# spcl/gms

Hardware: AMD Instinct MI355X
Metric: edges-intersected/sec + achieved HBM GB/s, RMAT-26 triangle count @1/2/4/8 GPU (higher is better)
Workload: dtype int32 ids / uint64 counts

## Files before the change

gms_amd/capi.py:

```python
import ctypes as C
import os

import numpy as np

_HERE = os.path.dirname(os.path.abspath(__file__))
LIB_PATH = os.environ.get("GMSX_LIB") or os.path.join(_HERE, "lib", "libgmsx.so")

_i64p = np.ctypeslib.ndpointer(np.int64, flags="C_CONTIGUOUS")
_i32p = np.ctypeslib.ndpointer(np.int32, flags="C_CONTIGUOUS")
_u32p = np.ctypeslib.ndpointer(np.uint32, flags="C_CONTIGUOUS")

GEN_KRONECKER, GEN_UNIFORM = 0, 1
RELABEL_NEVER, RELABEL_AUTO, RELABEL_ALWAYS = 0, 1, 2
TC_AUTO, TC_ORIENTED, TC_FULL = 0, 1, 2
UPLOAD_DEFAULT, UPLOAD_TRUSTED, UPLOAD_FOR_TC = 0, 1, 2
PREPARE_TC = 1
SETOP_INTERSECT, SETOP_DIFFERENCE = 0, 1
OK, ERR_INVALID, ERR_NOMEM, ERR_IO, ERR_FORMAT, ERR_DIRECTED, ERR_NO_DEVICE = 0, -1, -2, -3, -4, -5, -6
ERR_DEVICE_MEM, ERR_NOT_CANONICAL, ERR_OVERFLOW, ERR_UNSUPPORTED, ERR_KERNEL, ERR_COMM, ERR_TIMEOUT = -7, -8, -9, -10, -11, -12, -13
COMM_ID_BYTES = 128

SYMBOLS = [
    "gmsx_strerror", "gmsx_version",
    "gmsx_csr_generate", "gmsx_csr_generate_rmat", "gmsx_csr_from_edges", "gmsx_csr_load", "gmsx_csr_save_sg", "gmsx_csr_save_sgx", "gmsx_csr_is_mapped", "gmsx_csr_from_arrays",
# ... 248 lines not shown
    def save_sg(self, path):
        _check(lib().gmsx_csr_save_sg(self._h, os.fsencode(path)), "gmsx_csr_save_sg")

    def save_sgx(self, path):
        _check(lib().gmsx_csr_save_sgx(self._h, os.fsencode(path)), "gmsx_csr_save_sgx")

    @property
    def is_mapped(self):
        return bool(lib().gmsx_csr_is_mapped(self._h))

    def relabel_by_degree(self):
        h = C.c_void_p()
        _check(lib().gmsx_csr_relabel_by_degree(self._h, C.byref(h)), "gmsx_csr_relabel_by_degree")
        return HostCSR(h)

    def worth_relabelling(self):
        return bool(lib().gmsx_csr_worth_relabelling(self._h))

    @property
    def num_nodes(self):
        return lib().gmsx_csr_num_nodes(self._h)

    @property
    def num_edges(self):
        return lib().gmsx_csr_num_edges(self._h)

    @property
    def nnz(self):
        return lib().gmsx_csr_num_edges_directed(self._h)

    def offsets(self):
        return np.ctypeslib.as_array(lib().gmsx_csr_offsets(self._h), shape=(self.num_nodes + 1,))

    def neighbors(self):
        nnz = self.nnz
        if nnz == 0:
            return np.zeros(0, dtype=np.int32)
        return np.ctypeslib.as_array(lib().gmsx_csr_neighbors(self._h), shape=(nnz,))

    def merge_elements(self):
        return int(lib().gmsx_csr_merge_elements(self._h))

    def fingerprint(self):
        return int(lib().gmsx_csr_fingerprint(self._h, 0)), int(lib().gmsx_csr_fingerprint(self._h, 1))

    def __del__(self):
        if getattr(self, "_h", None):
            lib().gmsx_csr_free(self._h)
            self._h = None


def set_host_threads(n=0):
    return int(lib().gmsx_set_host_threads(int(n)))


def set_option(name, value):
    _check(lib().gmsx_set_option(name.encode(), None if value is None else str(value).encode()), f"gmsx_set_option({name})")


def reset_options():
    lib().gmsx_reset_options()


def option_names():
    out, i, p = [], 0, C.c_char_p()
    while lib().gmsx_option_name(i, C.byref(p)) == 0:
        out.append(p.value.decode())
        i += 1
    return out


class options:

    def __init__(self, **kw):
        self.kw = kw

    def __enter__(self):
        for k, v in self.kw.items():
            set_option(k, v)
        return self

    def __exit__(self, *exc):
        for k in self.kw:
            set_option(k, None)
        return False


def init(device=-1):
    _check(lib().gmsx_init(device), "gmsx_init")


def set_stream(stream_ptr):
    _check(lib().gmsx_set_stream(C.c_void_p(stream_ptr)), "gmsx_set_stream")


def hbm_read_probe(nbytes=4 << 30, iterations=20):
    v = C.c_double(0)
    _check(lib().gmsx_hbm_read_probe(int(nbytes), int(iterations), C.byref(v)), "gmsx_hbm_read_probe")
    return v.value


def device_info():
    name = C.create_string_buffer(256)
    cu, mem = C.c_int(0), C.c_int64(0)
    _check(lib().gmsx_device_info(name, 256, C.byref(cu), C.byref(mem)), "gmsx_device_info")
    return {"name": name.value.decode(), "compute_units": cu.value, "hbm_bytes": mem.value}


class DeviceGraph:

    def __init__(self, handle):
        self._h = handle

    @classmethod
    def upload(cls, off, neigh, flags=UPLOAD_DEFAULT):
        off = np.ascontiguousarray(off, dtype=np.int64)
        neigh = np.ascontiguousarray(neigh, dtype=np.int32)
        h = C.c_void_p()
        _check(lib().gmsx_graph_upload(off.size - 1, off, neigh if neigh.size else np.zeros(1, np.int32), flags, C.byref(h)),
               "gmsx_graph_upload")
        return cls(h)

    @classmethod
    def from_csr(cls, csr, flags=UPLOAD_DEFAULT, shard=None):
        h = C.c_void_p()
        if shard is None:
            _check(lib().gmsx_graph_upload_csr(csr._h, flags, C.byref(h)), "gmsx_graph_upload_csr")
        else:
            _check(lib().gmsx_graph_upload_csr_shard(csr._h, flags, int(shard[0]), int(shard[1]), C.byref(h)), "gmsx_graph_upload_csr_shard")
        return cls(h)

    num_nodes = property(lambda self: lib().gmsx_graph_num_nodes(self._h))
    num_edges = property(lambda self: lib().gmsx_graph_num_edges(self._h))
    device_bytes = property(lambda self: lib().gmsx_graph_device_bytes(self._h))
    max_out_degree = property(lambda self: lib().gmsx_graph_max_out_degree(self._h))
    tc_passes = property(lambda self: lib().gmsx_graph_tc_passes(self._h))

    def prepare(self, what=PREPARE_TC):
        _check(lib().gmsx_graph_prepare(self._h, what), "gmsx_graph_prepare")

    def tc_total(self, algo=TC_AUTO, stats=False):
        out, st = C.c_uint64(0), Stats()
        _check(lib().gmsx_tc_total(self._h, algo, C.byref(out), C.byref(st)), "gmsx_tc_total")
        return (int(out.value), st.as_dict()) if stats else int(out.value)

    def tc_partial(self, part, nparts, algo=TC_AUTO, stats=False):
        out, st = C.c_uint64(0), Stats()
        _check(lib().gmsx_tc_partial(self._h, algo, part, nparts, C.byref(out), C.byref(st)), "gmsx_tc_partial")
        return (int(out.value), st.as_dict()) if stats else int(out.value)

    BREAKDOWN = ["hub_rows_list", "hub_rows_bitset", "hub_rows_delta", "tail_rows_list", "tail_rows_delta", "entries", "pivot_containers",
                 "of_which_inline_rows", "light_streamed_hub_rows", "light_streamed_tail_rows", "light_pivot_lists_and_descriptors",
                 "count_entries", "count_inline_entries", "count_work_items", "count_light_streamed_members",
                 "reserved15", "reserved16", "reserved17", "reserved18", "reserved19", "reserved20"]
    BREAKDOWN_BYTES = ("hub_rows_list", "hub_rows_bitset", "hub_rows_delta", "tail_rows_list", "tail_rows_delta", "entries", "pivot_containers",
                       "light_streamed_hub_rows", "light_streamed_tail_rows", "light_pivot_lists_and_descriptors")

    def tc_stream_breakdown(self):
        out = np.zeros(21, dtype=np.uint64)
        _check(lib().gmsx_tc_stream_breakdown(self._h, out), "gmsx_tc_stream_breakdown")
        return dict(zip(self.BREAKDOWN, (int(x) for x in out)))

    def tc_row_histogram(self):
        out = np.zeros(256, dtype=np.uint64)
        _check(lib().gmsx_tc_row_histogram(self._h, out), "gmsx_tc_row_histogram")
        return out[:240].reshape(5, 24, 2).astype(np.int64), out[240:].astype(np.int64)

    def tc_comembership(self, batch):
        out = np.zeros(8, dtype=np.uint64)
        _check(lib().gmsx_tc_comembership(self._h, int(batch), out), "gmsx_tc_comembership")
        return dict(entries=int(out[0]), units=int(out[1]), distinct_rows=int(out[2]), batched_units=int(out[3]), items=int(out[4]))

    def tc_vertex_count2(self, stats=False):
        c, st = np.zeros(self.num_nodes, dtype=np.int64), Stats()
        _check(lib().gmsx_tc_vertex_count2(self._h, c, C.byref(st)), "gmsx_tc_vertex_count2")
        return (c, st.as_dict()) if stats else c

    def intersect_count_batch(self, u, v, stats=False):
        u = np.ascontiguousarray(u, dtype=np.int32)
        v = np.ascontiguousarray(v, dtype=np.int32)
        out, st = np.zeros(max(u.size, 1), dtype=np.uint32), Stats()
        _check(lib().gmsx_intersect_count_batch(self._h, u.size, u if u.size else np.zeros(1, np.int32),
                                                v if v.size else np.zeros(1, np.int32), out, C.byref(st)),
               "gmsx_intersect_count_batch")
        out = out[:u.size]
        return (out, st.as_dict()) if stats else out

    def set_op_batch(self, op, u, v, stats=False):
        code = {"intersect": SETOP_INTERSECT, "difference": SETOP_DIFFERENCE}[op]
        u = np.ascontiguousarray(u, dtype=np.int32)
        v = np.ascontiguousarray(v, dtype=np.int32)
        uu, vv = (u if u.size else np.zeros(1, np.int32)), (v if v.size else np.zeros(1, np.int32))
        off, st = np.zeros(u.size + 1, dtype=np.int64), Stats()
        _check(lib().gmsx_set_op_batch(self._h, code, u.size, uu, vv, off, None, 0, C.byref(st)), "gmsx_set_op_batch (sizing)")
        ids = np.zeros(max(int(off[-1]), 1), dtype=np.int32)
        _check(lib().gmsx_set_op_batch(self._h, code, u.size, uu, vv, off, ids.ctypes.data_as(C.c_void_p), int(off[-1]), C.byref(st)), "gmsx_set_op_batch")
        ids = ids[:int(off[-1])]
        return (off, ids, st.as_dict()) if stats else (off, ids)

    SIM = {"jaccard": 0, "overlap": 1, "adamic_adar": 2, "resource": 3, "common_neighbors": 4, "total_neighbors": 5, "pref_attachment": 6}

    def vertex_similarity_batch(self, metric, u, v, stats=False):
        u = np.ascontiguousarray(u, dtype=np.int32)
        v = np.ascontiguousarray(v, dtype=np.int32)
        out, st = np.zeros(max(u.size, 1), dtype=np.float64), Stats()
        m = self.SIM[metric] if isinstance(metric, str) else int(metric)
        _check(lib().gmsx_vertex_similarity_batch(self._h, m, u.size, u if u.size else np.zeros(1, np.int32),
                                                  v if v.size else np.zeros(1, np.int32), out, C.byref(st)), "gmsx_vertex_similarity_batch")
        out = out[:u.size]
        return (out, st.as_dict()) if stats else out

    def kclique_count(self, k, stats=False):
        ordered, cliques, st = C.c_uint64(0), C.c_uint64(0), Stats()
        _check(lib().gmsx_kclique_count(self._h, k, C.byref(ordered), C.byref(cliques), C.byref(st)), "gmsx_kclique_count")
        r = (int(ordered.value), int(cliques.value))
        return (r + (st.as_dict(),)) if stats else r

    def kclique_star_count(self, k, members=True, stats=False):
        stars, mem, st = C.c_uint64(0), C.c_uint64(0), Stats()
        _check(lib().gmsx_kclique_star_count(self._h, k, C.byref(stars), C.byref(mem) if members else None, C.byref(st)), "gmsx_kclique_star_count")
        r = (int(stars.value), int(mem.value) if members else None)
        return (r + (st.as_dict(),)) if stats else r

    def kclique_star_list_info(self, k, cliques_only=False, part=0, nparts=1):
        info = KcliqueStarListInfo()
        flags = KCSTAR_CLIQUES_ONLY if cliques_only else KCSTAR_DEFAULT
        _check(lib().gmsx_kclique_star_list(self._h, k, flags, part, nparts, None, None, None, 0, 0, C.byref(info), None),
               "gmsx_kclique_star_list (sizing)")
        return info.as_dict()

    def kclique_star_list(self, k, cliques_only=False, part=0, nparts=1, stats=False):
        info, st = KcliqueStarListInfo(), Stats()
        flags = KCSTAR_CLIQUES_ONLY if cliques_only else KCSTAR_DEFAULT
        _check(lib().gmsx_kclique_star_list(self._h, k, flags, part, nparts, None, None, None, 0, 0, C.byref(info), C.byref(st)),
               "gmsx_kclique_star_list (sizing)")
        sizing = st.as_dict()
        nc, nm = int(info.cliques), int(info.star_members)
        cl = np.zeros(max(nc * k, 1), dtype=np.int32)
        soff = mem = None
        if not cliques_only:
            soff = np.zeros(nc + 1, dtype=np.int64)
            mem = np.zeros(max(nm, 1), dtype=np.int32)
        _check(lib().gmsx_kclique_star_list(self._h, k, flags, part, nparts, cl.ctypes.data_as(C.c_void_p),
                                            None if cliques_only else soff.ctypes.data_as(C.c_void_p),
                                            None if cliques_only else mem.ctypes.data_as(C.c_void_p), nc, nm, C.byref(info), C.byref(st)),
               "gmsx_kclique_star_list")
        cl = cl[:nc * k].reshape(nc, k)
        if mem is not None:
            mem = mem[:nm]
        if stats:
            return cl, soff, mem, {"sizing": sizing, "fill": st.as_dict(), "info": info.as_dict()}
        return cl, soff, mem

    def kclique_partial(self, k, part, nparts, stats=False):
        out, st = C.c_uint64(0), Stats()
        _check(lib().gmsx_kclique_partial(self._h, k, part, nparts, C.byref(out), C.byref(st)), "gmsx_kclique_partial")
        return (int(out.value), st.as_dict()) if stats else int(out.value)

    def bk_count(self, rank=None, stats=False):
        out, st = C.c_uint64(0), Stats()
        rp = None
        if rank is not None:
            rank = np.ascontiguousarray(rank, dtype=np.int32)
            rp = rank.ctypes.data_as(C.c_void_p)
        _check(lib().gmsx_bk_count(self._h, rp, C.byref(out), C.byref(st)), "gmsx_bk_count")
        return (int(out.value), st.as_dict()) if stats else int(out.value)

    def bk_partial(self, part, nparts, rank=None, stats=False):
        out, st = C.c_uint64(0), Stats()
        rp = None
        if rank is not None:
            rank = np.ascontiguousarray(rank, dtype=np.int32)
            rp = rank.ctypes.data_as(C.c_void_p)
        _check(lib().gmsx_bk_partial(self._h, rp, part, nparts, C.byref(out), C.byref(st)), "gmsx_bk_partial")
        return (int(out.value), st.as_dict()) if stats else int(out.value)

    def bk_list_info(self, rank=None, part=0, nparts=1):
        info = BkListInfo()
        rp = None
        if rank is not None:
            rank = np.ascontiguousarray(rank, dtype=np.int32)
            rp = rank.ctypes.data_as(C.c_void_p)
        _check(lib().gmsx_bk_list(self._h, rp, part, nparts, None, None, 0, 0, C.byref(info), None), "gmsx_bk_list (sizing)")
        return info.as_dict()

    def bk_list(self, rank=None, part=0, nparts=1, stats=False):
        info, st = BkListInfo(), Stats()
        rp = None
        if rank is not None:
            rank = np.ascontiguousarray(rank, dtype=np.int32)
            rp = rank.ctypes.data_as(C.c_void_p)
        _check(lib().gmsx_bk_list(self._h, rp, part, nparts, None, None, 0, 0, C.byref(info), C.byref(st)), "gmsx_bk_list (sizing)")
        sizing = st.as_dict()
        off = np.zeros(int(info.cliques) + 1, dtype=np.int64)
        mem = np.zeros(max(int(info.members), 1), dtype=np.int32)
        _check(lib().gmsx_bk_list(self._h, rp, part, nparts, off.ctypes.data_as(C.c_void_p), mem.ctypes.data_as(C.c_void_p), off.size,
                                  int(info.members), C.byref(info), C.byref(st)), "gmsx_bk_list")
        mem = mem[:int(info.members)]
        if stats:
            return off, mem, {"sizing": sizing, "fill": st.as_dict(), "info": info.as_dict()}
        return off, mem

    def adg_rank(self, epsilon=0.001, rank_format=True, stats=False):
        out, rounds, st = np.zeros(max(self.num_nodes, 1), dtype=np.int32), C.c_int32(0), Stats()
        _check(lib().gmsx_adg_rank(self._h, float(epsilon), int(bool(rank_format)), out, C.byref(rounds), C.byref(st)), "gmsx_adg_rank")
        r = (out[:self.num_nodes], int(rounds.value))
        return (r + (st.as_dict(),)) if stats else r

    def tc_ordering(self, stats=False):
# ... 143 lines not shown
```

gms_amd/csrc/hip/device_graph.hip:

```cpp
#include "device_graph.hpp"

#include <algorithm>
#include <mutex>
#include <array>
#include <chrono>
#include <cstdio>
#include <cstdlib>
#include <cstring>
#include <memory>
#include <new>
#include <random>

#include <rocprim/device/device_radix_sort.hpp>
#include <rocprim/device/device_scan.hpp>
#include <rocprim/device/device_segmented_radix_sort.hpp>
#include <rocprim/iterator/transform_iterator.hpp>

#include "../host/gmsx_internal.hpp"

namespace gmsx {

Ctx &ctx() {
    static Ctx c;
    return c;
}

int ensure_init() { return ctx().device >= 0 ? GMSX_OK : gmsx_init(-1); }


__device__ __forceinline__ unsigned long long arc_mix(unsigned long long x) {
    x ^= x >> 30;
    x *= 0xbf58476d1ce4e5b9ull;
    x ^= x >> 27;
    x *= 0x94d049bb133111ebull;
    x ^= x >> 31;
    return x;
}
__global__ __launch_bounds__(256) void k_validate(int64_t n, const int64_t *__restrict__ off,
                                                  const int32_t *__restrict__ adj, int check_symmetry, unsigned long long key0,
                                                  unsigned long long key1,
                                                  unsigned long long *__restrict__ acc ) {
    const int lane = threadIdx.x & 63;
    const int64_t wave0 = (int64_t(blockIdx.x) * blockDim.x + threadIdx.x) >> 6;
    const int64_t nwaves = (int64_t(gridDim.x) * blockDim.x) >> 6;
    unsigned flags = 0;
    unsigned long long elems = 0;
    unsigned long long maxdeg = 0;
    unsigned long long f0 = 0, r0 = 0, f1 = 0, r1 = 0;
    for (int64_t u = wave0; u < n; u += nwaves) {
        const int64_t b = off[u], e = off[u + 1];
        const unsigned long long du = (unsigned long long)(e - b);
        if (du > maxdeg) maxdeg = du;
        if (lane == 0) elems += du * du;
        for (int64_t j = b + lane; j < e; j += 64) {
            const int32_t v = adj[j];
            if (v < 0 || v >= n) { flags |= 2; continue; }
            if (v == u) flags |= 4;
            if (j + 1 < e && adj[j + 1] <= v) flags |= 1;
            if (check_symmetry) {
                const unsigned long long uv = ((unsigned long long)uint32_t(u) << 32) | uint32_t(v), vu = ((unsigned long long)uint32_t(v) << 32) | uint32_t(u);
                f0 += arc_mix(uv ^ key0);
                r0 += arc_mix(vu ^ key0);
                f1 += arc_mix(uv * 0x9e3779b97f4a7c15ull + key1);
                r1 += arc_mix(vu * 0x9e3779b97f4a7c15ull + key1);
            }
        }
    }
    for (int s = 32; s > 0; s >>= 1) {
        elems += __shfl_down(elems, s);
        flags |= __shfl_down(flags, s);
        const unsigned long long o = __shfl_down(maxdeg, s);
        maxdeg = o > maxdeg ? o : maxdeg;
        f0 += __shfl_down(f0, s);
        r0 += __shfl_down(r0, s);
        f1 += __shfl_down(f1, s);
        r1 += __shfl_down(r1, s);
    }
    if (lane == 0) {
        if (flags) atomicOr(&acc[0], (unsigned long long)flags);
        if (elems) atomicAdd(&acc[1], elems);
        atomicMax(&acc[2], maxdeg);
        if (check_symmetry) {
            atomicAdd(&acc[3], f0);
            atomicAdd(&acc[4], r0);
            atomicAdd(&acc[5], f1);
            atomicAdd(&acc[6], r1);
        }
    }
}

__global__ void k_rank_keys(int64_t n, const int64_t *__restrict__ off, unsigned long long *__restrict__ keys) {
    const int64_t u = int64_t(blockIdx.x) * blockDim.x + threadIdx.x;
    if (u < n) keys[u] = ((unsigned long long)(off[u + 1] - off[u]) << 32) | (unsigned long long)u;
}
__global__ void k_assign_ids(int64_t n, const unsigned long long *__restrict__ sorted_keys, int32_t *__restrict__ oldid,
                             int32_t *__restrict__ newid) {
    const int64_t i = int64_t(blockIdx.x) * blockDim.x + threadIdx.x;
    if (i < n) {
        const int32_t o = int32_t(sorted_keys[i] & 0xffffffffull);
        oldid[i] = o;
        newid[o] = int32_t(i);
    }
}

__global__ __launch_bounds__(256) void k_count_parts(int64_t n, const int64_t *__restrict__ off, const int32_t *__restrict__ adj,
                                                     const int32_t *__restrict__ newid, int hub_limit, int64_t *__restrict__ hcnt,
                                                     int64_t *__restrict__ tcnt, int32_t *__restrict__ dplus) {
    const int lane = threadIdx.x & 63;
    const int64_t wave0 = (int64_t(blockIdx.x) * blockDim.x + threadIdx.x) >> 6;
    const int64_t nwaves = (int64_t(gridDim.x) * blockDim.x) >> 6;
    for (int64_t u = wave0; u < n; u += nwaves) {
        const int64_t b = off[u], e = off[u + 1];
        const int32_t nu = newid[u];
        int ch = 0, ct = 0;
        for (int64_t j = b + lane; j < e; j += 64) {
            const int32_t nv = newid[adj[j]];
            if (nv < nu) {
                if (nv < hub_limit) ch++; else ct++;
            }
        }
        for (int s = 32; s > 0; s >>= 1) {
            ch += __shfl_down(ch, s);
            ct += __shfl_down(ct, s);
        }
        if (lane == 0) {
            hcnt[nu] = (ch + 1) & ~1;
            tcnt[nu] = ct;
            dplus[nu] = ch + ct;
        }
    }
}

__global__ __launch_bounds__(256) void k_fill_parts(int64_t n, const int64_t *__restrict__ off, const int32_t *__restrict__ adj,
                                                    const int32_t *__restrict__ newid, int hub_limit, const int64_t *__restrict__ hoff,
                                                    const int64_t *__restrict__ toff, uint16_t *__restrict__ hadj,
                                                    int32_t *__restrict__ tadj) {
    const int lane = threadIdx.x & 63;
    const int64_t wave0 = (int64_t(blockIdx.x) * blockDim.x + threadIdx.x) >> 6;
    const int64_t nwaves = (int64_t(gridDim.x) * blockDim.x) >> 6;
    for (int64_t u = wave0; u < n; u += nwaves) {
        const int64_t b = off[u], e = off[u + 1];
        const int32_t nu = newid[u];
        int64_t ho = hoff[nu], to = toff[nu];
        const int64_t hend = hoff[nu + 1];
        for (int64_t base = b; base < e; base += 64) {
            const int64_t j = base + lane;
            bool kh = false, kt = false;
            int32_t nv = 0;
            if (j < e) {
                nv = newid[adj[j]];
                kh = nv < nu && nv < hub_limit;
                kt = nv < nu && nv >= hub_limit;
            }
            const unsigned long long mh = __ballot(kh), mt = __ballot(kt);
            const unsigned long long below = (1ull << lane) - 1ull;
            if (kh) hadj[ho + __popcll(mh & below)] = uint16_t(nv);
            if (kt) tadj[to + __popcll(mt & below)] = nv;
            ho += __popcll(mh);
            to += __popcll(mt);
        }
        if (lane == 0 && ho < hend) hadj[ho] = 0xFFFF;
    }
}

__device__ inline uint32_t delta_encode(const uint16_t *__restrict__ row, int len, uint32_t *__restrict__ emit) {
    uint32_t units = 0;
    int i = 0;
    while (i < len && row[i] != 0xFFFFu) {
        uint32_t w[4] = {row[i], 0u, 0u, 0u};
        uint32_t cur = row[i];
        int slot = 3;
// ... 86 lines not shown
            int rf = kFormList;
            if (rl >= 24 && delta_mode > 0) {
                const uint32_t d = delta_encode(hadj + b + k, rl, nullptr);
                if (d * 100u <= r * uint32_t(delta_pct)) { r = d; rf = kFormDelta; }
            }
            const uint32_t cand = uint32_t(B / 128) + r;
            if (cand < tot && (hybrid_mode == 2 || cand * 100u <= best * 90u)) {
                tot = cand;
                ks = k;
                best2 = r;
                form2 = rf;
            }
        }
        if (ks > 0) {
            best = tot - best2;
            form = kFormBitset;
        }
    }
    ksplit[v] = ks;
    const uint32_t u2[2] = {best, best2};
    const int f2[2] = {form, form2};
    for (int sl = 0; sl < 2; ++sl) {
        const bool big = u2[sl] >= 8u;
        units_out[2 * v + sl] = big ? int64_t((u2[sl] + 7u) & ~7u) : 0;
        small_out[2 * v + sl] = big ? 0 : int64_t(u2[sl]);
        real_out[2 * v + sl] = u2[sl];
        form_out[2 * v + sl] = (unsigned char)f2[sl];
    }
}
__global__ void k_srow_fill(int64_t n, const int64_t *__restrict__ hoff, const uint16_t *__restrict__ hadj, const int64_t *__restrict__ bmoff,
                            const uint32_t *__restrict__ bmpool, const int64_t *__restrict__ uoff, const int64_t *__restrict__ soff,
                            const uint32_t *__restrict__ real, const unsigned char *__restrict__ form, const int32_t *__restrict__ ksplit,
                            unsigned long long *__restrict__ srow, unsigned long long *__restrict__ srow2, uint32_t *__restrict__ spool) {
    const int64_t v = int64_t(blockIdx.x) * blockDim.x + threadIdx.x;
    if (v >= n) return;
    const int64_t b = hoff[v];
    const int len = int(hoff[v + 1] - b);
    const int ks = ksplit[v];
    for (int sl = 0; sl < 2; ++sl) {
        const int64_t units = int64_t(real[2 * v + sl]);
        const int64_t u0 = units >= 8 ? uoff[2 * v + sl] : uoff[2 * n] + soff[2 * v + sl];
        const int fm = form[2 * v + sl];
        const unsigned long long d = units ? ((unsigned long long)u0 << 24) | ((unsigned long long)fm << 22) | (unsigned long long)units : 0ull;
        if (sl == 0) srow[v] = units ? d : ((unsigned long long)u0 << 24) | ((unsigned long long)fm << 22);
        else srow2[v] = d;
        if (units == 0) continue;
        uint32_t *dst = spool + u0 * 4;
        const uint16_t *row = hadj + b + (sl ? ks : 0);
        const int rl = sl ? len - ks : len;
        if (sl == 0 && ks > 0) {
            for (int64_t w = 0; w < units * 4; ++w) dst[w] = 0;
            for (int i = 0; i < ks; ++i) dst[row[i] >> 5] |= 1u << (row[i] & 31u);
        } else if (fm == kFormDelta) {
            delta_encode(row, rl, dst);
        } else if (fm == kFormGap12) {
            gap12_encode(row, rl, dst);
        } else if (fm == kFormBitset) {
            const uint32_t *src = bmpool + bmoff[v];
            for (int64_t w = 0; w < units * 4; ++w) dst[w] = src[w];
        } else {
            for (int64_t w = 0; w < units * 4; ++w) {
                const int i = int(w) * 2;
                const uint32_t lo = i < rl ? row[i] : 0xFFFFu, hi = i + 1 < rl ? row[i + 1] : 0xFFFFu;
                dst[w] = lo | (hi << 16);
            }
        }
    }
}

__device__ inline uint32_t tail_delta_encode(const int32_t *__restrict__ row, int len, uint32_t *__restrict__ emit) {
    uint32_t units = 0;
    int i = 0;
    while (i < len) {
        uint32_t w[4] = {uint32_t(row[i]), 0u, 0u, 0u};
        uint32_t cur = uint32_t(row[i]);
        int slot = 1;
        ++i;
        while (i < len && slot < 6) {
            const uint32_t gap = uint32_t(row[i]) - cur;
            if (gap > 65535u) break;
            w[1 + (slot >> 1)] |= gap << ((slot & 1) * 16);
            ++slot;
            cur = uint32_t(row[i]);
            ++i;
        }
        w[1] |= uint32_t(slot);
        if (emit) {
            emit[units * 4 + 0] = w[0]; emit[units * 4 + 1] = w[1]; emit[units * 4 + 2] = w[2]; emit[units * 4 + 3] = w[3];
        }
        ++units;
    }
    return units;
}
__global__ void k_trow_sizes(int64_t n, const int64_t *__restrict__ toff, const int32_t *__restrict__ tadj, int delta_mode,
                             int64_t *__restrict__ units_out, int64_t *__restrict__ small_out, uint32_t *__restrict__ real_out, unsigned char *__restrict__ form_out) {
    const int64_t v = int64_t(blockIdx.x) * blockDim.x + threadIdx.x;
    if (v > n) return;
    if (v == n) { units_out[n] = 0; small_out[n] = 0; return; }
    const int64_t b = toff[v];
    const int len = int(toff[v + 1] - b);
    uint32_t best = uint32_t((len + 3) / 4);
    int form = kFormList;
    if (len >= 8 && delta_mode > 0) {
        const uint32_t d = tail_delta_encode(tadj + b, len, nullptr);
        if (delta_mode == 2 || d * 100u <= best * 85u) { best = d; form = kFormDelta; }
    }
    const bool big = best >= 8u;
    units_out[v] = big ? int64_t((best + 7u) & ~7u) : 0;
    small_out[v] = big ? 0 : int64_t(best);
    real_out[v] = best;
    form_out[v] = (unsigned char)form;
}
__global__ void k_trow_fill(int64_t n, const int64_t *__restrict__ toff, const int32_t *__restrict__ tadj, const int64_t *__restrict__ uoff,
                            const int64_t *__restrict__ soff, const uint32_t *__restrict__ real, const unsigned char *__restrict__ form,
                            unsigned long long *__restrict__ trow, uint32_t *__restrict__ tpool) {
    const int64_t v = int64_t(blockIdx.x) * blockDim.x + threadIdx.x;
    if (v >= n) return;
    const int64_t units = int64_t(real[v]);
    const int64_t u0 = units >= 8 ? uoff[v] : uoff[n] + soff[v];
    trow[v] = ((unsigned long long)u0 << 24) | ((unsigned long long)form[v] << 22) | (unsigned long long)units;
    if (units == 0) return;
    uint32_t *dst = tpool + u0 * 4;
    const int64_t b = toff[v];
    const int64_t len = toff[v + 1] - b;
    if (form[v] == kFormDelta) tail_delta_encode(tadj + b, int(len), dst);
    else
        for (int64_t w = 0; w < units * 4; ++w) dst[w] = w < len ? uint32_t(tadj[b + w]) : 0xfffffffeu;
}

__global__ void k_dense_sizes(int32_t limit, const int32_t *__restrict__ dplus, int64_t *__restrict__ sizes) {
    const int32_t v = int32_t(blockIdx.x * blockDim.x + threadIdx.x);
    if (v < limit) sizes[v] = bitset_words(v);
    if (v == limit) sizes[v] = 0;
}
__global__ __launch_bounds__(256) void k_dense_fill(int32_t limit, const int64_t *__restrict__ hoff, const uint16_t *__restrict__ hadj,
                                                    const int64_t *__restrict__ toff, const int32_t *__restrict__ tadj,
                                                    const int64_t *__restrict__ bmoff, uint32_t *__restrict__ pool) {
    const int lane = threadIdx.x & 63;
    const int32_t wave0 = int32_t((int64_t(blockIdx.x) * blockDim.x + threadIdx.x) >> 6);
    const int32_t nwaves = int32_t((int64_t(gridDim.x) * blockDim.x) >> 6);
    for (int32_t v = wave0; v < limit; v += nwaves) {
        const int64_t b = bmoff[v];
        if (bmoff[v + 1] == b) continue;
        for (int64_t j = hoff[v] + lane; j < hoff[v + 1]; j += 64) {
            const uint32_t id = hadj[j];
            if (id != 0xFFFFu) atomicOr(&pool[b + (id >> 5)], 1u << (id & 31u));
        }
        for (int64_t j = toff[v] + lane; j < toff[v + 1]; j += 64) {
            const uint32_t id = uint32_t(tadj[j]);
            atomicOr(&pool[b + (id >> 5)], 1u << (id & 31u));
        }
    }
}
__global__ __launch_bounds__(256) void k_tail_split(int64_t n, const int64_t *__restrict__ toff, const int32_t *__restrict__ tadj, int32_t limit,
                                                    int32_t *__restrict__ tsplit) {
    const int lane = threadIdx.x & 63;
    const int64_t wave0 = (int64_t(blockIdx.x) * blockDim.x + threadIdx.x) >> 6;
    const int64_t nwaves = (int64_t(gridDim.x) * blockDim.x) >> 6;
    for (int64_t u = wave0; u < n; u += nwaves) {
        int c = 0;
        for (int64_t j = toff[u] + lane; j < toff[u + 1]; j += 64) c += tadj[j] < limit;
        for (int s = 32; s > 0; s >>= 1) c += __shfl_down(c, s);
        if (lane == 0) tsplit[u] = c;
    }
}

__global__ void k_order_keys(int64_t n, const int32_t *__restrict__ dplus, int32_t *__restrict__ keys, int32_t *__restrict__ vals) {
    const int64_t i = int64_t(blockIdx.x) * blockDim.x + threadIdx.x;
    if (i < n) {
        keys[i] = dplus[i];
        vals[i] = int32_t(i);
    }
}

__global__ void k_warm(unsigned long long *p) {
    if (p) p[0] = 0;
}
__global__ void k_count_ge(int64_t n, const int32_t *__restrict__ order, const int32_t *__restrict__ dplus, int32_t thr, int64_t *__restrict__ out) {
    int64_t lo = 0, hi = n;
    while (lo < hi) {
        const int64_t mid = (lo + hi) >> 1;
        if (dplus[order[mid]] >= thr) lo = mid + 1; else hi = mid;
    }
    out[0] = lo;
}
__global__ void k_task_limits(int64_t n, const unsigned long long *__restrict__ srow, const unsigned long long *__restrict__ srow2,
                              const unsigned long long *__restrict__ trow, uint32_t hub_max, uint32_t tail_max, unsigned long long *__restrict__ out) {
    const int64_t v = int64_t(blockIdx.x) * blockDim.x + threadIdx.x;
    if (v >= n) return;
    if ((srow[v] & 0x3fffffull) > hub_max || (srow2[v] & 0x3fffffull) > hub_max || (trow[v] & 0x3fffffull) > tail_max) atomicOr(out, 1ull);
}

static constexpr int kInlineChunk = 64;
static constexpr int kDefaultInlineFirst = 28;
static constexpr int kInlineFirstMax = 64;
__device__ __forceinline__ bool takes_inline(int32_t v, int32_t inline_limit, const int32_t *__restrict__ dplus) {
    return v < inline_limit || dplus[v] >= kHeavy;
}
template <bool FILL>
__global__ __launch_bounds__(256) void k_inline_rows(int64_t first, int64_t end, const int32_t *__restrict__ order, const int64_t *__restrict__ hoff,
                                                     const uint16_t *__restrict__ hadj, const int64_t *__restrict__ toff, const int32_t *__restrict__ tadj,
                                                     const int32_t *__restrict__ dplus, int32_t inline_limit, int inline_first, const int32_t *__restrict__ opos, int nparts, int part,
                                                     unsigned long long *__restrict__ cnt_h,
                                                     unsigned long long *__restrict__ cnt_t, const int64_t *__restrict__ ihoff,
                                                     const int64_t *__restrict__ itoff, int64_t base_h, uint16_t *__restrict__ pool_h, int64_t base_t,
                                                     int32_t *__restrict__ pool_t) {
    const int lane = threadIdx.x & 63;
    const int64_t wave0 = (int64_t(blockIdx.x) * blockDim.x + threadIdx.x) >> 6;
    const int64_t nwaves = (int64_t(gridDim.x) * blockDim.x) >> 6;
    for (int64_t pos = first + wave0; pos < end; pos += nwaves) {
        const int32_t u = order[pos];
        const int64_t hb = hoff[u], tb = toff[u];
        const int first_u = dplus[u] >= kHeavy ? inline_first : kInlineFirstMax;
        const int hl = min(int(hoff[u + 1] - hb), first_u), tl = min(int(toff[u + 1] - tb), first_u - hl);
        int32_t mv = 0x7fffffff;
        if (lane < hl) {
            const uint32_t x = hadj[hb + lane];
            if (x != 0xFFFFu) mv = int32_t(x);
        } else if (lane - hl < tl) {
            mv = tadj[tb + (lane - hl)];
        }
        const bool valid = mv != 0x7fffffff, is_tail = valid && lane >= hl;
        const unsigned long long vmask = __ballot(valid);
        const int nhub = __popcll(__ballot(valid && lane < hl));
        const int below = __popcll(vmask & ((1ull << lane) - 1ull));
        const bool give = valid && below > 0 && takes_inline(mv, inline_limit, dplus);
        const bool mine = give && (nparts <= 1 || shard_of(opos[mv], nparts) == part);
        const int nh = mine ? (is_tail ? nhub : below) : 0;
        const int nt = mine && is_tail ? lane - hl : 0;
        if (!FILL) {
            if (nh) atomicAdd(&cnt_h[mv], (unsigned long long)nh);
            if (nt) atomicAdd(&cnt_t[mv], (unsigned long long)nt);
        } else {
            int64_t at_h = 0, at_t = 0;
            if (nh) at_h = (base_h + ihoff[mv]) * 8 + int64_t(atomicAdd(&cnt_h[mv], (unsigned long long)nh));
            if (nt) at_t = (base_t + itoff[mv]) * 4 + int64_t(atomicAdd(&cnt_t[mv], (unsigned long long)nt));
            for (int k = 0; k < nhub; ++k) {
                const int32_t x = __shfl(mv, k);
                if (k < nh) pool_h[at_h + k] = uint16_t(x);
            }
            for (int k = 0; k < tl; ++k) {
                const int32_t x = __shfl(mv, hl + k);
                if (k < nt) pool_t[at_t + k] = x;
            }
        }
    }
}
__global__ void k_inline_units(int64_t n, const unsigned long long *__restrict__ ids_h, const unsigned long long *__restrict__ ids_t,
                               int64_t *__restrict__ units_h, int64_t *__restrict__ units_t) {
    const int64_t v = int64_t(blockIdx.x) * blockDim.x + threadIdx.x;
    if (v > n) return;
    units_h[v] = v < n ? int64_t((ids_h[v] + 7) / 8) : 0;
    units_t[v] = v < n ? int64_t((ids_t[v] + 3) / 4) : 0;
}
static constexpr int kDefaultHotWindows = 0, kDefaultHotKB = 2048, kDefaultHotMin = 16;
__device__ __forceinline__ int64_t receiver_of(int32_t w, const int32_t *__restrict__ dplus, const int32_t *__restrict__ opos, const int64_t *__restrict__ lidx,
                                               int64_t n_heavy) {
    return dplus[w] >= kHeavy ? int64_t(opos[w]) : n_heavy + lidx[w];
}
__global__ void k_opos(int64_t n, const int32_t *__restrict__ order, int32_t *__restrict__ opos) {
    const int64_t p = int64_t(blockIdx.x) * blockDim.x + threadIdx.x;
    if (p < n) opos[order[p]] = int32_t(p);
}
__global__ void k_light_flags(int64_t limit, const int32_t *__restrict__ dplus, int64_t *__restrict__ flags) {
    const int64_t w = int64_t(blockIdx.x) * blockDim.x + threadIdx.x;
    if (w <= limit) flags[w] = (w < limit && dplus[w] < kHeavy) ? 1 : 0;
}
__global__ void k_recv_vertices(int64_t n_heavy, int64_t limit, const int32_t *__restrict__ order, const int32_t *__restrict__ dplus, const int64_t *__restrict__ lidx,
                                int32_t *__restrict__ recv_v) {
    const int64_t i = int64_t(blockIdx.x) * blockDim.x + threadIdx.x;
    if (i < n_heavy) recv_v[i] = order[i];
    if (i < limit && dplus[i] < kHeavy) recv_v[n_heavy + lidx[i]] = int32_t(i);
}
template <bool FILL>
__global__ void k_inline_entries(int64_t n, const int32_t *__restrict__ dplus, const int32_t *__restrict__ opos, const int64_t *__restrict__ lidx, int64_t n_heavy,
                                 int32_t inline_limit, const int64_t *__restrict__ ihoff, const int64_t *__restrict__ itoff, int64_t base_h, int64_t base_t,
                                 uint32_t *__restrict__ cnt, uint32_t *__restrict__ cur, const int64_t *__restrict__ hbeg, const int64_t *__restrict__ tbeg,
                                 TaskList htask, TaskList ttask, unsigned long long *__restrict__ totals, TcClasses cc) {
    const int kClasses = cc.count();
    const int64_t v = int64_t(blockIdx.x) * blockDim.x + threadIdx.x;
    if (v >= n) return;
    const int64_t uh = ihoff[v + 1] - ihoff[v], ut = itoff[v + 1] - itoff[v];
    if (uh == 0 && ut == 0) return;
    if (dplus[v] < kHeavy && v >= inline_limit) return;
    const int64_t p = receiver_of(int32_t(v), dplus, opos, lidx, n_heavy);
    uint32_t *c = cnt + p * kClasses;
    for (int64_t o = 0; o < uh; o += kInlineChunk) {
        const unsigned long long units = (unsigned long long)min(int64_t(kInlineChunk), uh - o);
        const unsigned long long d = ((unsigned long long)(base_h + ihoff[v] + o) << 24) | ((unsigned long long)kFormList << 22) | units;
        const int cls = hub_class(cc, d);
        if (!FILL) atomicAdd(&c[cls], 1u);
        else htask.put(hbeg[p] + c[cls] + atomicAdd(&cur[p * kClasses + cls], 1u), d);
    }
    for (int64_t o = 0; o < ut; o += kInlineChunk) {
        const unsigned long long units = (unsigned long long)min(int64_t(kInlineChunk), ut - o);
        const unsigned long long d = ((unsigned long long)(base_t + itoff[v] + o) << 24) | ((unsigned long long)kFormList << 22) | units;
        const int cls = tail_class(cc, d);
        if (!FILL) atomicAdd(&c[cls], 1u);
        else ttask.put(tbeg[p] + c[cls] + atomicAdd(&cur[p * kClasses + cls], 1u), d);
    }
    if (!FILL) {
        atomicAdd(&totals[0], (unsigned long long)((uh + kInlineChunk - 1) / kInlineChunk));
        atomicAdd(&totals[1], (unsigned long long)((ut + kInlineChunk - 1) / kInlineChunk));
    }
}
__global__ void k_list_sizes(int64_t n_recv, uint32_t *__restrict__ cnt, int64_t *__restrict__ hcnt, int64_t *__restrict__ tcnt, TcClasses cc) {
    const int kClasses = cc.count(), hub_end = cc.tail_base();
    const int64_t p = int64_t(blockIdx.x) * blockDim.x + threadIdx.x;
    if (p > n_recv) return;
    if (p == n_recv) { hcnt[p] = 0; tcnt[p] = 0; return; }
    uint32_t *c = cnt + p * kClasses;
    uint32_t run = 0;
    for (int k = 0; k < hub_end; ++k) { const uint32_t x = c[k]; c[k] = run; run += x; }
    hcnt[p] = run;
    run = 0;
    for (int k = hub_end; k < kClasses; ++k) { const uint32_t x = c[k]; c[k] = run; run += x; }
    tcnt[p] = run;
}

__global__ void k_ledge_count(int64_t first, int64_t end, const int32_t *__restrict__ order, const int64_t *__restrict__ toff, const int32_t *__restrict__ tadj,
                              const int32_t *__restrict__ tsplit, const int32_t *__restrict__ dplus, int64_t *__restrict__ cnt) {
    const int64_t pos = first + int64_t(blockIdx.x) * blockDim.x + threadIdx.x;
    if (pos > end) return;
    int64_t c = 0;
    if (pos < end) {
        const int32_t u = order[pos];
        const int64_t tb = toff[u];
        const int tl = int(toff[u + 1] - tb);
        for (int i = tsplit[u]; i < tl; ++i) c += dplus[tadj[tb + i]] < kHeavy ? 1 : 0;
    }
    cnt[pos - first] = c;
}
__global__ void k_ledge_fill(int64_t first, int64_t end, const int32_t *__restrict__ order, const int64_t *__restrict__ hoff, const int64_t *__restrict__ toff,
                             const int32_t *__restrict__ tadj, const int32_t *__restrict__ tsplit, const int32_t *__restrict__ dplus,
                             const int64_t *__restrict__ ebeg, int nparts, int part, uint4 *__restrict__ ledge) {
    const int64_t pos = first + int64_t(blockIdx.x) * blockDim.x + threadIdx.x;
    if (pos >= end) return;
    const int32_t u = order[pos];
    const int64_t hb = hoff[u], tb = toff[u];
    const int tl = int(toff[u + 1] - tb);
    const unsigned long long hu = (unsigned long long)hb | ((unsigned long long)(hoff[u + 1] - hb) << 40);
    int64_t e = ebeg[pos - first];
    for (int i = tsplit[u]; i < tl; ++i) {
        const int32_t v = tadj[tb + i];
        if (dplus[v] >= kHeavy) continue;
        if (nparts <= 1 || shard_of(e, nparts) == part) {
            const unsigned long long tu = (unsigned long long)tb | ((unsigned long long)i << 40);
            const unsigned long long hv = (unsigned long long)hoff[v] | ((unsigned long long)(hoff[v + 1] - hoff[v]) << 40);
            const unsigned long long tv = (unsigned long long)toff[v] | ((unsigned long long)(toff[v + 1] - toff[v]) << 40);
            const int64_t slot = nparts <= 1 ? e : e / nparts;
            ledge[2 * slot] = make_uint4(uint32_t(hu), uint32_t(hu >> 32), uint32_t(tu), uint32_t(tu >> 32));
            ledge[2 * slot + 1] = make_uint4(uint32_t(hv), uint32_t(hv >> 32), uint32_t(tv), uint32_t(tv >> 32));
        }
        ++e;
    }
}

__device__ __forceinline__ uint32_t cut_hub_units(const uint32_t *__restrict__ spool, unsigned long long d, int below, int32_t v) {
    const uint32_t units = uint32_t(d) & 0x3fffffu, form = (uint32_t(d) >> 22) & 3u;
    if (form == kFormList) return min(units, uint32_t(below + 7) / 8u);
    if (form == kFormBitset) return min(units, uint32_t(v + 127) / 128u);
    const uint4 *row = reinterpret_cast<const uint4 *>(spool) + (d >> 24);
    uint32_t lo = 0, hi = units;
    while (lo < hi) {
        const uint32_t mid = (lo + hi) >> 1;
        if (int32_t(row[mid].x & 0xffffu) < v) lo = mid + 1; else hi = mid;
    }
    return lo;
}
__device__ __forceinline__ uint32_t cut_tail_units(const uint32_t *__restrict__ tpool, unsigned long long d, int below, int32_t v) {
    const uint32_t units = uint32_t(d) & 0x3fffffu, form = (uint32_t(d) >> 22) & 3u;
    if (form != kFormDelta) return min(units, uint32_t(below + 3) / 4u);
    const uint4 *row = reinterpret_cast<const uint4 *>(tpool) + (d >> 24);
    uint32_t lo = 0, hi = units;
    while (lo < hi) {
        const uint32_t mid = (lo + hi) >> 1;
        if (int32_t(row[mid].x) < v) lo = mid + 1; else hi = mid;
    }
    return lo;
}
__device__ __forceinline__ uint32_t claim_by_class(uint32_t *ctr, int cls, bool active, int lane) {
    uint32_t mine = 0;
    unsigned long long todo = __ballot(active);
    while (todo) {
        const int leader = __ffsll((long long)todo) - 1;
        const int c = __builtin_amdgcn_readlane(cls, leader);
        const unsigned long long same = __ballot(active && cls == c);
        uint32_t base = 0;
        if (lane == leader) base = atomicAdd(&ctr[c], uint32_t(__popcll(same)));
        base = uint32_t(__builtin_amdgcn_readlane(int(base), leader));
        if (active && cls == c) mine = base + uint32_t(__popcll(same & ((1ull << lane) - 1ull)));
        todo &= ~same;
    }
    return mine;
}
template <bool FILL>
__global__ __launch_bounds__(256) void k_task_lists(int64_t n_heavy, const int32_t *__restrict__ order, const int64_t *__restrict__ hoff,
                                                    const uint16_t *__restrict__ hadj, const int64_t *__restrict__ toff, const int32_t *__restrict__ tadj,
                                                    const int32_t *__restrict__ dplus, const unsigned long long *__restrict__ srow,
                                                    const unsigned long long *__restrict__ srow2, const int32_t *__restrict__ ksplit,
                                                    const unsigned long long *__restrict__ trow, int two_sided, const int32_t *__restrict__ opos,
                                                    uint32_t *__restrict__ cnt, uint32_t *__restrict__ cur, const int64_t *__restrict__ hbeg,
                                                    const int64_t *__restrict__ tbeg, TaskList htask, TaskList ttask,
                                                    int32_t *__restrict__ tunits, unsigned long long *__restrict__ reversed, const uint32_t *__restrict__ spool,
                                                    const uint32_t *__restrict__ tpool, int32_t inline_limit, int inline_first, int nparts, int part, TcClasses cc) {
    const int kClasses = cc.count();
    const int lane = threadIdx.x & 63;
    const int64_t wave0 = (int64_t(blockIdx.x) * blockDim.x + threadIdx.x) >> 6;
    const int64_t nwaves = (int64_t(gridDim.x) * blockDim.x) >> 6;
    unsigned long long rev = 0;
    for (int64_t pos = wave0; pos < n_heavy; pos += nwaves) {
        const int32_t u = order[pos];
        const int64_t hb = hoff[u], tb = toff[u];
        const int hl = int(hoff[u + 1] - hb), tl = int(toff[u + 1] - tb);
        const unsigned long long du_s = srow[u], du_s2 = srow2[u], du_t = trow[u];
        const int ks_u = ksplit[u];
        uint32_t *cu = cnt + pos * kClasses, *ru = cur + pos * kClasses;
        const bool own_u = nparts <= 1 || shard_of(pos, nparts) == part;
        int kept = 0;
        for (int base = 0; base < hl + tl; base += 64) {
            const int i = base + lane;
            int32_t v = -1;
            if (i < hl) {
                const uint32_t x = hadj[hb + i];
                if (x != 0xFFFFu) v = int32_t(x);
            } else if (i < hl + tl) v = tadj[tb + i - hl];
            if (v >= 0 && i > 0 && i < inline_first && takes_inline(v, inline_limit, dplus)) v = -1;
            bool reverse = false;
            uint32_t ch = 0, ch2 = 0, ct = 0;
            if (v >= 0 && i > 0 && two_sided && dplus[v] >= kHeavy) {
                if (i < hl) {
                    ch = cut_hub_units(spool, du_s, i, v);
                    if (du_s2 && i > ks_u) ch2 = cut_hub_units(spool, du_s2, i - ks_u, v);
                } else {
                    ch = uint32_t(du_s) & 0x3fffffu;
                    ch2 = uint32_t(du_s2) & 0x3fffffu;
                }
                ct = (i < hl || toff[v + 1] == toff[v]) ? 0u : cut_tail_units(tpool, du_t, i - hl, v);
                const uint32_t keep = uint32_t(srow[v] & 0x3fffffull) + uint32_t(srow2[v] & 0x3fffffull) + (i > hl ? uint32_t(trow[v] & 0x3fffffull) : 0u);
                reverse = ch + ch2 + ct < keep;
            }
            const bool fwd = v >= 0 && !reverse && own_u;
            if (reverse && nparts > 1 && shard_of(opos[v], nparts) != part) v = -1;
            const unsigned long long fh = (fwd && i > 0) ? srow[v] : 0ull, fh2 = (fwd && i > 0) ? srow2[v] : 0ull, ft = (fwd && i > hl) ? trow[v] : 0ull;
            const bool fh_on = (fh & 0x3fffffull) != 0, fh2_on = (fh2 & 0x3fffffull) != 0, ft_on = (ft & 0x3fffffull) != 0;
            const uint32_t sh = claim_by_class(FILL ? ru : cu, hub_class(cc, fh), fh_on, lane);
            const uint32_t sh2 = claim_by_class(FILL ? ru : cu, hub_class(cc, fh2), fh2_on, lane);
            const uint32_t st = claim_by_class(FILL ? ru : cu, tail_class(cc, ft), ft_on, lane);
            if (FILL) {
                if (fh_on) htask.put(hbeg[pos] + cu[hub_class(cc, fh)] + sh, fh);
                if (fh2_on) htask.put(hbeg[pos] + cu[hub_class(cc, fh2)] + sh2, fh2);
                if (ft_on) ttask.put(tbeg[pos] + cu[tail_class(cc, ft)] + st, ft);
            }
            kept += __popcll(__ballot(fwd));
            if (v >= 0 && reverse) {
                const int64_t pv = opos[v];
                const unsigned long long rh = ch ? (du_s & ~0x3fffffull) | ch : 0ull, rh2 = ch2 ? (du_s2 & ~0x3fffffull) | ch2 : 0ull,
                                         rt = ct ? (du_t & ~0x3fffffull) | ct : 0ull;
                uint32_t *cv = cnt + pv * kClasses;
                if (!FILL) {
                    if (rh) atomicAdd(&cv[hub_class(cc, rh)], 1u);
                    if (rh2) atomicAdd(&cv[hub_class(cc, rh2)], 1u);
                    if (rt) atomicAdd(&cv[tail_class(cc, rt)], 1u);
                    atomicAdd(&tunits[pv], 1);
                    ++rev;
                } else {
                    uint32_t *rv = cur + pv * kClasses;
                    if (rh) htask.put(hbeg[pv] + cv[hub_class(cc, rh)] + atomicAdd(&rv[hub_class(cc, rh)], 1u), rh);
                    if (rh2) htask.put(hbeg[pv] + cv[hub_class(cc, rh2)] + atomicAdd(&rv[hub_class(cc, rh2)], 1u), rh2);
                    if (rt) ttask.put(tbeg[pv] + cv[tail_class(cc, rt)] + atomicAdd(&rv[tail_class(cc, rt)], 1u), rt);
                }
            }
        }
        if (!FILL && lane == 0 && kept) atomicAdd(&tunits[pos], kept);
    }
    if (!FILL) {
        for (int s = 32; s > 0; s >>= 1) rev += __shfl_down(rev, s);
        if (lane == 0 && rev) atomicAdd(reversed, rev);
    }
}
__global__ void k_item_counts(int64_t n_recv, const int64_t *__restrict__ lbeg, const uint32_t *__restrict__ cnt, TcClasses cc, int phases, int64_t *__restrict__ items) {
    const int64_t p = int64_t(blockIdx.x) * blockDim.x + threadIdx.x;
    if (p > n_recv) return;
    if (p == n_recv) { items[int64_t(phases) * n_recv] = 0; return; }
    for (int ph = 0; ph < phases; ++ph) {
        int64_t b = 0, e = lbeg[p + 1] - lbeg[p];
        if (phases > 1) hub_phase_range(cc, cnt + p * cc.count(), e, ph, &b, &e);
        items[int64_t(ph) * n_recv + p] = (e - b + kTaskChunk - 1) / kTaskChunk;
    }
}
__global__ void k_item_fill(int64_t n_recv, const int32_t *__restrict__ recv_v, const int32_t *__restrict__ opos, const int64_t *__restrict__ lbeg,
                            const int64_t *__restrict__ ioff, TaskList task, const int64_t *__restrict__ coff, int kind,
                            const uint32_t *__restrict__ cnt, TcClasses cc, int phases, gmsx_tc_item *__restrict__ items) {
    const int64_t p = int64_t(blockIdx.x) * blockDim.x + threadIdx.x;
    if (p >= n_recv) return;
    const int32_t w = recv_v[p];
    const uint64_t cont = uint64_t(coff[w]) | (uint64_t(coff[w + 1] - coff[w]) << 40);
    for (int ph = 0; ph < phases; ++ph) {
    int64_t b = 0, e = lbeg[p + 1] - lbeg[p];
    if (phases > 1) hub_phase_range(cc, cnt + p * cc.count(), e, ph, &b, &e);
    b += lbeg[p];
    e += lbeg[p];
    int64_t k = ioff[int64_t(ph) * n_recv + p];
    for (int64_t x = b; x < e; x += kTaskChunk, ++k) {
        const int ne = int(min(int64_t(kTaskChunk), e - x));
        gmsx_tc_item it{};
        it.bc = uint64_t(x) | (uint64_t(ne) << 40);
        it.cont = cont;
        it.pivot = w;
        it.pos = opos[w];
        it.kind = uint32_t(kind);
        for (int f = 0; f < 4; ++f) {
            int lo = 0, hi = ne;
            while (lo < hi) {
                const int mid = (lo + hi) >> 1;
                if (int((uint32_t(task.get(x + mid)) >> 22) & 3u) < f) lo = mid + 1; else hi = mid;
            }
            it.fbeg[f] = uint16_t(lo);
        }
        items[k] = it;
    }
    }
}

static int grid_for_waves(int64_t rows) {
    const int64_t want = (rows + 3) / 4;
    const int64_t cap = int64_t(ctx().compute_units > 0 ? ctx().compute_units : 256) * 32;
    return int(want < 1 ? 1 : (want > cap ? cap : want));
}

template <class T>
static int dmalloc(T **p, int64_t count, gmsx_graph *g, int line = __builtin_LINE()) {
    const size_t bytes = size_t(count > 0 ? count : 1) * sizeof(T);
    const bool trace = opt("MEM_TRACE") != nullptr;
    if (trace && g && bytes >= (1u << 20)) std::fprintf(stderr, "gmsx mem: device_graph.hip:%d %.3f GB (elements of %zu B)\n", line, double(bytes) * 1e-9, sizeof(T));
    if (g && g->tc_building && g->tc_limit_bytes > 0 && g->device_bytes + int64_t(bytes) - g->tc_base_bytes > g->tc_limit_bytes) {
        *p = nullptr;
        return GMSX_ERR_DEVICE_MEM;
    }
    if (hipMalloc(reinterpret_cast<void **>(p), bytes) != hipSuccess) {
        (void)hipGetLastError();
        *p = nullptr;
        return GMSX_ERR_DEVICE_MEM;
    }
    if (g) g->device_bytes += int64_t(bytes);
    return GMSX_OK;
}

struct DevGuard {
    void *p;
    ~DevGuard() { (void)hipFree(p); }
};

static void free_tc(gmsx_graph *g) {
    auto drop = [](auto *&p) {
        (void)hipFree(p);
        p = nullptr;
    };
    drop(g->tsplit); drop(g->srow); drop(g->srow2); drop(g->ksplit); drop(g->spool); drop(g->trow); drop(g->htask.lo); drop(g->htask.hi); drop(g->ttask.lo); drop(g->ttask.hi); drop(g->hitem); drop(g->titem); drop(g->tunits);
    drop(g->ledge); drop(g->tpool); drop(g->shard_hitem); drop(g->shard_titem);
    g->shard_idx_part = g->shard_idx_nparts = -1;
    g->device_bytes -= g->tc_bytes;
    g->tc_bytes = 0;
    g->tc_ready = false;
    g->htask_entries = g->ttask_entries = g->hitems = g->titems = g->inline_hentries = g->inline_tentries = 0;
    g->n_ledge = g->ledge_total = 0;
    g->task_reverse = g->inline_units = g->spool_units = g->tpool_units = 0;
    g->stats_part = g->stats_nparts = -1;
}

static void free_graph(gmsx_graph *g) {
    if (!g) return;
    (void)hipFree(g->off);
    (void)hipFree(g->adj);
    (void)hipFree(g->newid);
    (void)hipFree(g->oldid);
    (void)hipFree(g->hoff);
    (void)hipFree(g->hadj);
    (void)hipFree(g->toff);
    (void)hipFree(g->tadj);
    (void)hipFree(g->bmoff);
    (void)hipFree(g->bmpool);
    (void)hipFree(g->tsplit);
    (void)hipFree(g->srow);
    (void)hipFree(g->srow2);
    (void)hipFree(g->ksplit);
    (void)hipFree(g->spool);
    (void)hipFree(g->trow);
    (void)hipFree(g->htask.lo);
    (void)hipFree(g->htask.hi);
    (void)hipFree(g->ttask.lo);
    (void)hipFree(g->ttask.hi);
    (void)hipFree(g->hitem);
    (void)hipFree(g->titem);
    (void)hipFree(g->tunits);
    (void)hipFree(g->shard_hitem);
    (void)hipFree(g->shard_titem);
    (void)hipFree(g->ledge);
    (void)hipFree(g->tpool);
    (void)hipFree(g->dplus);
    (void)hipFree(g->order);
    (void)hipFree(g->kc_rel);
    (void)hipFree(g->kc_aoff);
    (void)hipFree(g->kc_arena);
    (void)hipFree(g->kc_rec);
    (void)hipFree(g->kc_item);
    (void)hipFree(g->kc_relt);
    (void)hipFree(g->kc_rect);
    (void)hipFree(g->kc_itemt);
    (void)hipFree(g->scratch);
    (void)hipFree(g->acc);
    delete g;
}

int exclusive_scan_i64(const int64_t *in, int64_t *out, int64_t count, hipStream_t s) {
    size_t tmp_bytes = 0;
    GMSX_HIP(rocprim::exclusive_scan(nullptr, tmp_bytes, in, out, int64_t(0), size_t(count), rocprim::plus<int64_t>(), s));
    void *tmp = nullptr;
    GMSX_HIP(hipMalloc(&tmp, tmp_bytes ? tmp_bytes : 8));
    DevGuard g_tmp{tmp};
    GMSX_HIP(rocprim::exclusive_scan(tmp, tmp_bytes, in, out, int64_t(0), size_t(count), rocprim::plus<int64_t>(), s));
    GMSX_HIP(hipStreamSynchronize(s));
    return GMSX_OK;
}

struct OffsetMinus {
    int64_t base;
    __host__ __device__ int64_t operator()(int64_t x) const { return x - base; }
};
__global__ void k_lower_bound_i64(int64_t count, const int64_t *__restrict__ a, int64_t target, int64_t *__restrict__ out) {
    int64_t lo = 0, hi = count;
    while (lo < hi) {
        const int64_t mid = (lo + hi) >> 1;
        if (a[mid] < target) lo = mid + 1; else hi = mid;
    }
    out[0] = lo;
}
template <class K>
static int sort_rows(K *keys, int64_t entries, int64_t n, const int64_t *d_off, int end_bit, hipStream_t s) {
    if (n <= 0 || entries <= 0) return GMSX_OK;
    int64_t chunk = int64_t(1) << 31;
    if (const char *e = opt("SORT_CHUNK")) {
        const long long v = std::atoll(e);
        if (v > 0) chunk = v;
    }
    int64_t *d_v = nullptr;
    GMSX_HIP(hipMalloc(reinterpret_cast<void **>(&d_v), sizeof(int64_t)));
    DevGuard g_v{d_v};
    GMSX_HIP(hipStreamSynchronize(s));
    int64_t v0 = 0, base = 0;
    while (v0 < n) {
        int64_t v1 = n;
        if (entries - base > chunk) {
            hipLaunchKernelGGL(k_lower_bound_i64, dim3(1), dim3(1), 0, s, n + 1, d_off, base + chunk + 1, d_v);
            GMSX_HIP(hipStreamSynchronize(s));
            GMSX_HIP(hipMemcpy(&v1, d_v, sizeof(int64_t), hipMemcpyDeviceToHost));
            v1 = std::max(v0 + 1, std::min(n, v1 - 1));
        }
        int64_t end = 0;
        GMSX_HIP(hipMemcpy(&end, d_off + v1, sizeof(int64_t), hipMemcpyDeviceToHost));
        const int64_t cnt = end - base;
        if (cnt >= (int64_t(1) << 32)) return GMSX_ERR_UNSUPPORTED;
        if (cnt > 0) {
            K *sorted = nullptr;
            GMSX_HIP(hipMalloc(reinterpret_cast<void **>(&sorted), size_t(cnt) * sizeof(K)));
            DevGuard g_sorted{sorted};
            auto begin = rocprim::make_transform_iterator(d_off + v0, OffsetMinus{base});
            auto endit = rocprim::make_transform_iterator(d_off + v0 + 1, OffsetMinus{base});
            size_t tmp_bytes = 0;
            GMSX_HIP(rocprim::segmented_radix_sort_keys(nullptr, tmp_bytes, keys + base, sorted, unsigned(cnt), unsigned(v1 - v0), begin, endit, 0, end_bit, s));
            void *tmp = nullptr;
            GMSX_HIP(hipMalloc(&tmp, tmp_bytes ? tmp_bytes : 8));
            DevGuard g_tmp{tmp};
            GMSX_HIP(rocprim::segmented_radix_sort_keys(tmp, tmp_bytes, keys + base, sorted, unsigned(cnt), unsigned(v1 - v0), begin, endit, 0, end_bit, s));
            GMSX_HIP(hipMemcpyAsync(keys + base, sorted, size_t(cnt) * sizeof(K), hipMemcpyDeviceToDevice, s));
            GMSX_HIP(hipStreamSynchronize(s));
        }
        v0 = v1;
        base = end;
    }
    return GMSX_OK;
}

template <class K, class V>
static int sort_segment_pairs(K *keys, V *vals, int64_t entries, int64_t n, const int64_t *d_off, int end_bit, hipStream_t s) {
    if (n <= 0 || entries <= 0) return GMSX_OK;
    int64_t chunk = int64_t(1) << 31;
    if (const char *e = opt("SORT_CHUNK")) {
        const long long v = std::atoll(e);
        if (v > 0) chunk = v;
    }
    int64_t *d_v = nullptr;
    GMSX_HIP(hipMalloc(reinterpret_cast<void **>(&d_v), sizeof(int64_t)));
    DevGuard g_v{d_v};
    GMSX_HIP(hipStreamSynchronize(s));
    int64_t v0 = 0, base = 0;
    while (v0 < n) {
        int64_t v1 = n;
        if (entries - base > chunk) {
            hipLaunchKernelGGL(k_lower_bound_i64, dim3(1), dim3(1), 0, s, n + 1, d_off, base + chunk + 1, d_v);
            GMSX_HIP(hipStreamSynchronize(s));
            GMSX_HIP(hipMemcpy(&v1, d_v, sizeof(int64_t), hipMemcpyDeviceToHost));
            v1 = std::max(v0 + 1, std::min(n, v1 - 1));
        }
        int64_t end = 0;
        GMSX_HIP(hipMemcpy(&end, d_off + v1, sizeof(int64_t), hipMemcpyDeviceToHost));
        const int64_t cnt = end - base;
        if (cnt >= (int64_t(1) << 32)) return GMSX_ERR_UNSUPPORTED;
        if (cnt > 0) {
            K *k_out = nullptr;
            V *v_out = nullptr;
            GMSX_HIP(hipMalloc(reinterpret_cast<void **>(&k_out), size_t(cnt) * sizeof(K)));
            DevGuard g_ko{k_out};
            GMSX_HIP(hipMalloc(reinterpret_cast<void **>(&v_out), size_t(cnt) * sizeof(V)));
            DevGuard g_vo{v_out};
            auto begin = rocprim::make_transform_iterator(d_off + v0, OffsetMinus{base});
            auto endit = rocprim::make_transform_iterator(d_off + v0 + 1, OffsetMinus{base});
            size_t tmp_bytes = 0;
            GMSX_HIP(rocprim::segmented_radix_sort_pairs(nullptr, tmp_bytes, keys + base, k_out, vals + base, v_out, unsigned(cnt), unsigned(v1 - v0), begin, endit, 0,
                                                         end_bit, s));
            void *tmp = nullptr;
            GMSX_HIP(hipMalloc(&tmp, tmp_bytes ? tmp_bytes : 8));
            DevGuard g_tmp{tmp};
            GMSX_HIP(rocprim::segmented_radix_sort_pairs(tmp, tmp_bytes, keys + base, k_out, vals + base, v_out, unsigned(cnt), unsigned(v1 - v0), begin, endit, 0,
                                                         end_bit, s));
            GMSX_HIP(hipMemcpyAsync(vals + base, v_out, size_t(cnt) * sizeof(V), hipMemcpyDeviceToDevice, s));
            GMSX_HIP(hipStreamSynchronize(s));
        }
        v0 = v1;
        base = end;
    }
    return GMSX_OK;
}

struct PhaseTimer {
    hipStream_t s;
    bool on;
    std::chrono::steady_clock::time_point t0;
    const char *what;
    PhaseTimer(hipStream_t st, const char *w) : s(st), on(opt("TIMING") != nullptr), t0(std::chrono::steady_clock::now()), what(w) {}
    void mark(const char *phase) {
        if (!on) return;
        (void)hipStreamSynchronize(s);
        const auto t1 = std::chrono::steady_clock::now();
        std::fprintf(stderr, "[gmsx %s] %-28s %8.1f ms\n", what, phase, std::chrono::duration<double, std::milli>(t1 - t0).count());
        t0 = t1;
    }
};

static constexpr size_t kH2dChunk = size_t(64) << 20;
struct H2dStage {
// ... 41 lines not shown
        parallel_memcpy(to, static_cast<const char *>(src) + at, n);
        GMSX_HIP(hipMemcpyAsync(static_cast<char *>(dst) + at, to, n, hipMemcpyHostToDevice, s));
        GMSX_HIP(hipEventRecord(st.ev[b], s));
        used[b] = true;
    }
    return GMSX_OK;
}

static int build_device_sets(gmsx_graph *g, uint32_t flags) {
    hipStream_t s = ctx().stream;
    PhaseTimer pt(s, "base build");
    const int64_t n = g->n;
    if (int rc = dmalloc(&g->scratch, 16, g)) return rc;
    if (int rc = dmalloc(&g->acc, kAccWords, g)) return rc;
    GMSX_HIP(hipMemsetAsync(g->scratch, 0, 16 * sizeof(unsigned long long), s));

    const int check_sym = (flags & GMSX_UPLOAD_TRUSTED) ? 0 : 1;
    static const std::array<unsigned long long, 2> sym_keys = []() noexcept {
        try {
            std::random_device rd;
            return std::array<unsigned long long, 2>{((unsigned long long)rd() << 32) | rd(), ((unsigned long long)rd() << 32) | rd()};
        } catch (...) {
            const unsigned long long t = (unsigned long long)std::chrono::steady_clock::now().time_since_epoch().count();
            const unsigned long long a = (unsigned long long)reinterpret_cast<uintptr_t>(&t);
            return std::array<unsigned long long, 2>{t * 0x9E3779B97F4A7C15ull ^ a, (a * 0xC2B2AE3D27D4EB4Full) ^ (t << 17)};
        }
    }();
    if (n > 0)
        hipLaunchKernelGGL(k_validate, dim3(grid_for_waves(n)), dim3(256), 0, s, n, g->off, g->adj, check_sym, sym_keys[0], sym_keys[1], g->scratch);
    unsigned long long acc[7] = {0, 0, 0, 0, 0, 0, 0};
    GMSX_HIP(hipMemcpyAsync(acc, g->scratch, sizeof(acc), hipMemcpyDeviceToHost, s));
    GMSX_HIP(hipStreamSynchronize(s));
    if (check_sym && (acc[3] != acc[4] || acc[5] != acc[6])) acc[0] |= 8;
    if (!(flags & GMSX_UPLOAD_TRUSTED) && acc[0] != 0) return GMSX_ERR_NOT_CANONICAL;
    if ((flags & GMSX_UPLOAD_TRUSTED) && (acc[0] & 2)) return GMSX_ERR_NOT_CANONICAL;
    if (!(flags & GMSX_UPLOAD_TRUSTED) && (g->nnz & 1)) return GMSX_ERR_NOT_CANONICAL;
    g->alg_elements = acc[1];
    g->max_deg = int32_t(acc[2]);
    g->m = g->nnz / 2;

    pt.mark("validate");
    const unsigned tb = unsigned((n + 255) / 256);
    if (int rc = dmalloc(&g->newid, n, g)) return rc;
    if (int rc = dmalloc(&g->oldid, n, g)) return rc;
    if (n > 0) {
        unsigned long long *k_in = nullptr, *k_out = nullptr;
        if (int rc = dmalloc(&k_in, n, nullptr)) return rc;
        DevGuard g1{k_in};
        if (int rc = dmalloc(&k_out, n, nullptr)) return rc;
        DevGuard g2{k_out};
        hipLaunchKernelGGL(k_rank_keys, dim3(tb), dim3(256), 0, s, n, g->off, k_in);
        size_t tmp_bytes = 0;
        GMSX_HIP(rocprim::radix_sort_keys_desc(nullptr, tmp_bytes, k_in, k_out, size_t(n), 0, 64, s));
        void *tmp = nullptr;
        GMSX_HIP(hipMalloc(&tmp, tmp_bytes ? tmp_bytes : 8));
        DevGuard g3{tmp};
        GMSX_HIP(rocprim::radix_sort_keys_desc(tmp, tmp_bytes, k_in, k_out, size_t(n), 0, 64, s));
        hipLaunchKernelGGL(k_assign_ids, dim3(tb), dim3(256), 0, s, n, k_out, g->oldid, g->newid);
        GMSX_HIP(hipStreamSynchronize(s));
    }

    pt.mark("rank ids");
    int hub_limit = int((flags >> 8) & 0xffffu);
    if (hub_limit == 0 || hub_limit > kHub) hub_limit = kHub;
    int64_t *hcnt = nullptr, *tcnt = nullptr;
    if (int rc = dmalloc(&hcnt, n + 1, nullptr)) return rc;
    DevGuard g_h{hcnt};
    if (int rc = dmalloc(&tcnt, n + 1, nullptr)) return rc;
    DevGuard g_t{tcnt};
    GMSX_HIP(hipMemsetAsync(hcnt, 0, size_t(n + 1) * sizeof(int64_t), s));
    GMSX_HIP(hipMemsetAsync(tcnt, 0, size_t(n + 1) * sizeof(int64_t), s));
    if (int rc = dmalloc(&g->dplus, n, g)) return rc;
    if (n > 0)
        hipLaunchKernelGGL(k_count_parts, dim3(grid_for_waves(n)), dim3(256), 0, s, n, g->off, g->adj, g->newid, hub_limit, hcnt, tcnt, g->dplus);
    if (int rc = dmalloc(&g->hoff, n + 1, g)) return rc;
    if (int rc = dmalloc(&g->toff, n + 1, g)) return rc;
    if (int rc = exclusive_scan_i64(hcnt, g->hoff, n + 1, s)) return rc;
    if (int rc = exclusive_scan_i64(tcnt, g->toff, n + 1, s)) return rc;
    GMSX_HIP(hipMemcpy(&g->hub_entries, g->hoff + n, sizeof(int64_t), hipMemcpyDeviceToHost));
    GMSX_HIP(hipMemcpy(&g->tail_entries, g->toff + n, sizeof(int64_t), hipMemcpyDeviceToHost));

    if (int rc = dmalloc(&g->hadj, g->hub_entries + 8, g)) return rc;
    if (int rc = dmalloc(&g->tadj, g->tail_entries + 4, g)) return rc;
    GMSX_HIP(hipMemsetAsync(g->hadj + g->hub_entries, 0xff, 8 * sizeof(uint16_t), s));
    GMSX_HIP(hipMemsetAsync(g->tadj + g->tail_entries, 0xff, 4 * sizeof(int32_t), s));
    if (n > 0)
        hipLaunchKernelGGL(k_fill_parts, dim3(grid_for_waves(n)), dim3(256), 0, s, n, g->off, g->adj, g->newid, hub_limit, g->hoff, g->toff,
                           g->hadj, g->tadj);

    pt.mark("containers count+fill");
    if (int rc = sort_rows(g->hadj, g->hub_entries, n, g->hoff, 16, s)) return rc;
    if (int rc = sort_rows(g->tadj, g->tail_entries, n, g->toff, 32, s)) return rc;
    g->rows_sorted = true;

    pt.mark("row sorts");
    g->dense_limit = int32_t(std::min<int64_t>(n, hub_limit));
    g->bitset_limit = g->dense_limit;
    {
        const int32_t K = g->bitset_limit;
        int64_t *sizes = nullptr;
        if (int rc = dmalloc(&sizes, int64_t(K) + 1, nullptr)) return rc;
        DevGuard g_sz{sizes};
        if (int rc = dmalloc(&g->bmoff, int64_t(K) + 1, g)) return rc;
        hipLaunchKernelGGL(k_dense_sizes, dim3(unsigned(K / 256 + 1)), dim3(256), 0, s, K, g->dplus, sizes);
        if (int rc = exclusive_scan_i64(sizes, g->bmoff, int64_t(K) + 1, s)) return rc;
        GMSX_HIP(hipMemcpy(&g->bmpool_words, g->bmoff + K, sizeof(int64_t), hipMemcpyDeviceToHost));
        if (int rc = dmalloc(&g->bmpool, g->bmpool_words + 4, g)) return rc;
        GMSX_HIP(hipMemsetAsync(g->bmpool, 0, size_t(g->bmpool_words + 4) * sizeof(uint32_t), s));
        if (K > 0 && g->bmpool_words > 0)
            hipLaunchKernelGGL(k_dense_fill, dim3(grid_for_waves(K)), dim3(256), 0, s, K, g->hoff, g->hadj, g->toff, g->tadj, g->bmoff, g->bmpool);
    }
    pt.mark("bitsets");
    if (int rc = dmalloc(&g->order, n, g)) return rc;
    if (n > 0) {
        int32_t *keys_in = nullptr, *vals_in = nullptr, *keys_out = nullptr;
        if (int rc = dmalloc(&keys_out, n, nullptr)) return rc;
        DevGuard g_ko{keys_out};
        if (int rc = dmalloc(&keys_in, n, nullptr)) return rc;
        DevGuard g_ki{keys_in};
        if (int rc = dmalloc(&vals_in, n, nullptr)) return rc;
        DevGuard g_vi{vals_in};
        hipLaunchKernelGGL(k_order_keys, dim3(tb), dim3(256), 0, s, n, g->dplus, keys_in, vals_in);
        size_t tmp_bytes = 0;
        GMSX_HIP(rocprim::radix_sort_pairs_desc(nullptr, tmp_bytes, keys_in, keys_out, vals_in, g->order, size_t(n), 0, 32, s));
        void *tmp = nullptr;
        GMSX_HIP(hipMalloc(&tmp, tmp_bytes ? tmp_bytes : 8));
        DevGuard g_tmp{tmp};
        GMSX_HIP(rocprim::radix_sort_pairs_desc(tmp, tmp_bytes, keys_in, keys_out, vals_in, g->order, size_t(n), 0, 32, s));
        int32_t top = 0;
        GMSX_HIP(hipMemcpyAsync(&top, keys_out, sizeof(int32_t), hipMemcpyDeviceToHost, s));
        GMSX_HIP(hipStreamSynchronize(s));
        g->max_dplus = top;
    }

    pt.mark("d+ order");
    GMSX_HIP(hipStreamSynchronize(s));
    GMSX_HIP(hipGetLastError());
    g->hub_limit = hub_limit;
    g->upload_flags = flags;
    return GMSX_OK;
}

static int build_tc_sets(gmsx_graph *g) {
    hipStream_t s = ctx().stream;
    PhaseTimer pt(s, "tc build");
    const int64_t n = g->n;
    const uint32_t flags = g->upload_flags;
    const int hub_limit = g->hub_limit;
    const unsigned tb = unsigned((n + 255) / 256);
    int32_t *opos = nullptr;
    if (int rc = dmalloc(&opos, n + 1, nullptr)) return rc;
    DevGuard g_opos{opos};
    if (n > 0) hipLaunchKernelGGL(k_opos, dim3(tb), dim3(256), 0, s, n, g->order, opos);
    {
        int64_t want = std::min<int64_t>(524288, n / 256);
        bool forced = false;
        if (const char *e = opt("INLINE_LIMIT")) {
            const long long v = std::atoll(e);
            if (v >= 0 && v <= (1ll << 31) - 1) { want = v; forced = true; }
        }
        if (!forced && ((flags >> 8) & 0xffffu)) want = int64_t(4) * hub_limit;
        g->inline_limit = int32_t(std::min<int64_t>(n, std::max<int64_t>(want, g->dense_limit)));
        g->inline_first = kDefaultInlineFirst;
        if (const char *e = opt("TC_INLINE_FIRST")) g->inline_first = std::max(1, std::min(kInlineFirstMax, std::atoi(e)));
        if (int rc = dmalloc(&g->tsplit, n, g)) return rc;
        if (n > 0) hipLaunchKernelGGL(k_tail_split, dim3(grid_for_waves(n)), dim3(256), 0, s, n, g->toff, g->tadj, g->inline_limit, g->tsplit);
    }

    pt.mark("tail split");
    int64_t n_heavy = 0, n_work = 0;
    unsigned long long *inl_h = nullptr, *inl_t = nullptr;
    int64_t *ihoff = nullptr, *itoff = nullptr;
    if (int rc = dmalloc(&inl_h, n + 1, nullptr)) return rc;
    DevGuard g_inl_h{inl_h};
    if (int rc = dmalloc(&inl_t, n + 1, nullptr)) return rc;
    DevGuard g_inl_t{inl_t};
    if (int rc = dmalloc(&ihoff, n + 1, nullptr)) return rc;
    DevGuard g_ihoff{ihoff};
    if (int rc = dmalloc(&itoff, n + 1, nullptr)) return rc;
    DevGuard g_itoff{itoff};
    int64_t inline_h_units = 0, inline_t_units = 0;
    {
        if (n > 0) {
            int64_t *d_cnt = nullptr;
            if (int rc = dmalloc(&d_cnt, 2, nullptr)) return rc;
            DevGuard g_c{d_cnt};
            hipLaunchKernelGGL(k_count_ge, dim3(1), dim3(1), 0, s, n, g->order, g->dplus, int32_t(kHeavy), d_cnt);
            hipLaunchKernelGGL(k_count_ge, dim3(1), dim3(1), 0, s, n, g->order, g->dplus, int32_t(2), d_cnt + 1);
            GMSX_HIP(hipStreamSynchronize(s));
            int64_t h[2] = {0, 0};
            GMSX_HIP(hipMemcpy(h, d_cnt, sizeof(h), hipMemcpyDeviceToHost));
            n_heavy = h[0];
            n_work = h[1];
        }
        GMSX_HIP(hipMemsetAsync(inl_h, 0, size_t(n + 1) * sizeof(unsigned long long), s));
        GMSX_HIP(hipMemsetAsync(inl_t, 0, size_t(n + 1) * sizeof(unsigned long long), s));
        if (n_work > 0)
            hipLaunchKernelGGL(k_inline_rows<false>, dim3(grid_for_waves(n_work)), dim3(256), 0, s, int64_t(0), n_work, g->order, g->hoff, g->hadj,
                               g->toff, g->tadj, g->dplus, g->inline_limit, g->inline_first, opos, g->shard_nparts, g->shard_part, inl_h, inl_t, ihoff, itoff, int64_t(0), static_cast<uint16_t *>(nullptr),
                               int64_t(0), static_cast<int32_t *>(nullptr));
        int64_t *uh = nullptr, *ut = nullptr;
        if (int rc = dmalloc(&uh, n + 1, nullptr)) return rc;
        DevGuard g_uh{uh};
        if (int rc = dmalloc(&ut, n + 1, nullptr)) return rc;
        DevGuard g_ut{ut};
        hipLaunchKernelGGL(k_inline_units, dim3(unsigned(n / 256 + 1)), dim3(256), 0, s, n, inl_h, inl_t, uh, ut);
        if (int rc = exclusive_scan_i64(uh, ihoff, n + 1, s)) return rc;
        if (int rc = exclusive_scan_i64(ut, itoff, n + 1, s)) return rc;
        GMSX_HIP(hipMemcpy(&inline_h_units, ihoff + n, sizeof(int64_t), hipMemcpyDeviceToHost));
        GMSX_HIP(hipMemcpy(&inline_t_units, itoff + n, sizeof(int64_t), hipMemcpyDeviceToHost));
        g->inline_units = inline_h_units + inline_t_units;
    }

    pt.mark("inline row sizes");
    int64_t inline_h_base = 0, inline_t_base = 0;
    {
        int delta_mode = g->rows_sorted ? 1 : 0;
        if (const char *e = opt("TC_DELTA")) {
            const int v = std::atoi(e);
            if (v >= 0 && v <= 2 && g->rows_sorted) delta_mode = v;
        }
        int delta_pct = 85;
        if (const char *e = opt("TC_DELTA_PCT")) {
            const int v = std::atoi(e);
            if (v >= 10 && v <= 100) delta_pct = v;
        }
        int gap12_mode = 0;
        if (const char *e = opt("TC_GAP12")) {
            const int v = std::atoi(e);
            if (v >= 0 && v <= 2 && g->rows_sorted) gap12_mode = v;
        }
        int hybrid_mode = 0;
        if (const char *e = opt("TC_HYBRID")) {
            const int v = std::atoi(e);
            if (v >= 0 && v <= 2 && g->rows_sorted) hybrid_mode = v;
        }
        int64_t *units = nullptr, *uoff = nullptr, *small = nullptr, *soff = nullptr;
        uint32_t *real = nullptr;
        unsigned char *form = nullptr;
        const int64_t n2 = 2 * n;
        if (int rc = dmalloc(&units, n2 + 1, nullptr)) return rc;
        DevGuard g_u{units};
        if (int rc = dmalloc(&uoff, n2 + 1, nullptr)) return rc;
        DevGuard g_o{uoff};
        if (int rc = dmalloc(&small, n2 + 1, nullptr)) return rc;
        DevGuard g_s{small};
        if (int rc = dmalloc(&soff, n2 + 1, nullptr)) return rc;
        DevGuard g_so{soff};
        if (int rc = dmalloc(&real, n2 + 1, nullptr)) return rc;
        DevGuard g_r{real};
        if (int rc = dmalloc(&form, n2 + 1, nullptr)) return rc;
        DevGuard g_f{form};
        if (int rc = dmalloc(&g->ksplit, n + 1, g)) return rc;
        hipLaunchKernelGGL(k_srow_sizes, dim3(unsigned(n / 256 + 1)), dim3(256), 0, s, n, g->hoff, g->hadj, g->dplus, g->dense_limit, delta_mode, delta_pct, gap12_mode,
                           hybrid_mode, units, small, real, form, g->ksplit);
        if (int rc = exclusive_scan_i64(units, uoff, n2 + 1, s)) return rc;
        if (int rc = exclusive_scan_i64(small, soff, n2 + 1, s)) return rc;
        int64_t big_units = 0, small_units = 0;
        GMSX_HIP(hipMemcpy(&big_units, uoff + n2, sizeof(int64_t), hipMemcpyDeviceToHost));
        GMSX_HIP(hipMemcpy(&small_units, soff + n2, sizeof(int64_t), hipMemcpyDeviceToHost));
        g->spool_units = big_units + small_units + inline_h_units;
        inline_h_base = big_units + small_units;
        if (g->spool_units >= (int64_t(1) << 40)) return GMSX_ERR_DEVICE_MEM;
        if (int rc = dmalloc(&g->srow, n, g)) return rc;
        if (int rc = dmalloc(&g->srow2, n, g)) return rc;
        if (int rc = dmalloc(&g->spool, (g->spool_units + kPoolSlack) * 4, g)) return rc;
        GMSX_HIP(hipMemsetAsync(g->spool, 0, size_t((g->spool_units + kPoolSlack) * 4) * sizeof(uint32_t), s));
        if (inline_h_units > 0) GMSX_HIP(hipMemsetAsync(g->spool + inline_h_base * 4, 0xff, size_t(inline_h_units) * 16, s));
        if (n > 0)
            hipLaunchKernelGGL(k_srow_fill, dim3(unsigned((n + 255) / 256)), dim3(256), 0, s, n, g->hoff, g->hadj, g->bmoff, g->bmpool, uoff, soff, real, form,
                               g->ksplit, g->srow, g->srow2, g->spool);
        GMSX_HIP(hipStreamSynchronize(s));
    }
    {
        int delta_mode = g->rows_sorted ? 1 : 0;
        if (const char *e = opt("TC_TAIL_DELTA")) {
            const int v = std::atoi(e);
            if (v >= 0 && v <= 2 && g->rows_sorted) delta_mode = v;
        }
        int64_t *units = nullptr, *uoff = nullptr, *small = nullptr, *soff = nullptr;
        uint32_t *real = nullptr;
        unsigned char *form = nullptr;
        if (int rc = dmalloc(&units, n + 1, nullptr)) return rc;
        DevGuard g_u{units};
        if (int rc = dmalloc(&uoff, n + 1, nullptr)) return rc;
        DevGuard g_o{uoff};
        if (int rc = dmalloc(&small, n + 1, nullptr)) return rc;
        DevGuard g_s{small};
        if (int rc = dmalloc(&soff, n + 1, nullptr)) return rc;
        DevGuard g_so{soff};
        if (int rc = dmalloc(&real, n + 1, nullptr)) return rc;
        DevGuard g_r{real};
        if (int rc = dmalloc(&form, n + 1, nullptr)) return rc;
        DevGuard g_f{form};
        hipLaunchKernelGGL(k_trow_sizes, dim3(unsigned(n / 256 + 1)), dim3(256), 0, s, n, g->toff, g->tadj, delta_mode, units, small, real, form);
        if (int rc = exclusive_scan_i64(units, uoff, n + 1, s)) return rc;
        if (int rc = exclusive_scan_i64(small, soff, n + 1, s)) return rc;
        int64_t big_units = 0, small_units = 0;
        GMSX_HIP(hipMemcpy(&big_units, uoff + n, sizeof(int64_t), hipMemcpyDeviceToHost));
        GMSX_HIP(hipMemcpy(&small_units, soff + n, sizeof(int64_t), hipMemcpyDeviceToHost));
        inline_t_base = big_units + small_units;
        g->tpool_units = inline_t_base + inline_t_units;
        if (g->tpool_units >= (int64_t(1) << 40)) return GMSX_ERR_DEVICE_MEM;
        if (int rc = dmalloc(&g->trow, n, g)) return rc;
        if (int rc = dmalloc(&g->tpool, (g->tpool_units + kPoolSlack) * 4, g)) return rc;
        GMSX_HIP(hipMemsetD32Async(reinterpret_cast<hipDeviceptr_t>(g->tpool), int(0xFFFFFFFEu), size_t(g->tpool_units + kPoolSlack) * 4, s));
        if (n > 0)
            hipLaunchKernelGGL(k_trow_fill, dim3(unsigned((n + 255) / 256)), dim3(256), 0, s, n, g->toff, g->tadj, uoff, soff, real, form, g->trow, g->tpool);
        GMSX_HIP(hipStreamSynchronize(s));
    }

    pt.mark("tail stream rows");
    if (n_work > 0) {
        GMSX_HIP(hipMemsetAsync(inl_h, 0, size_t(n + 1) * sizeof(unsigned long long), s));
        GMSX_HIP(hipMemsetAsync(inl_t, 0, size_t(n + 1) * sizeof(unsigned long long), s));
        hipLaunchKernelGGL(k_inline_rows<true>, dim3(grid_for_waves(n_work)), dim3(256), 0, s, int64_t(0), n_work, g->order, g->hoff, g->hadj, g->toff,
                           g->tadj, g->dplus, g->inline_limit, g->inline_first, opos, g->shard_nparts, g->shard_part, inl_h, inl_t, ihoff, itoff, inline_h_base, reinterpret_cast<uint16_t *>(g->spool),
                           inline_t_base, reinterpret_cast<int32_t *>(g->tpool));
    }
    pt.mark("inline rows fill");
    {
        const int64_t nl = n_work - n_heavy;
        g->n_ledge = g->ledge_total = 0;
        if (nl > 0) {
            int64_t *ecnt = nullptr, *ebeg = nullptr;
            if (int rc = dmalloc(&ecnt, nl + 1, nullptr)) return rc;
            DevGuard g_ec{ecnt};
            if (int rc = dmalloc(&ebeg, nl + 1, nullptr)) return rc;
            DevGuard g_eb{ebeg};
            hipLaunchKernelGGL(k_ledge_count, dim3(unsigned(nl / 256 + 1)), dim3(256), 0, s, n_heavy, n_work, g->order, g->toff, g->tadj, g->tsplit, g->dplus, ecnt);
            if (int rc = exclusive_scan_i64(ecnt, ebeg, nl + 1, s)) return rc;
            GMSX_HIP(hipMemcpy(&g->ledge_total, ebeg + nl, sizeof(int64_t), hipMemcpyDeviceToHost));
            const int np = g->shard_nparts > 1 ? g->shard_nparts : 1, pp = g->shard_nparts > 1 ? g->shard_part : 0;
            {
                const int64_t full = g->ledge_total / np, rem = g->ledge_total % np;
                g->n_ledge = np <= 1 ? g->ledge_total : full + (((full & 1) ? np - 1 - pp : pp) < rem ? 1 : 0);
            }
            if (int rc = dmalloc(&g->ledge, 2 * g->n_ledge + 2, g)) return rc;
            hipLaunchKernelGGL(k_ledge_fill, dim3(unsigned(nl / 256 + 1)), dim3(256), 0, s, n_heavy, n_work, g->order, g->hoff, g->toff, g->tadj, g->tsplit, g->dplus, ebeg,
                               np, pp, g->ledge);
            GMSX_HIP(hipStreamSynchronize(s));
        }
    }
    pt.mark("light pivot list");
    {
        int two_sided = 1;
        if (const char *e = opt("TC_TWO_SIDED")) two_sided = std::atoi(e) != 0;
        const unsigned vb = unsigned(n / 256 + 1);
        const int64_t L = g->inline_limit;
        int64_t *lflag = nullptr, *lidx = nullptr;
        if (int rc = dmalloc(&lflag, L + 1, nullptr)) return rc;
        DevGuard g_lf{lflag};
        if (int rc = dmalloc(&lidx, L + 1, nullptr)) return rc;
        DevGuard g_li{lidx};
        hipLaunchKernelGGL(k_light_flags, dim3(unsigned(L / 256 + 1)), dim3(256), 0, s, L, g->dplus, lflag);
        if (int rc = exclusive_scan_i64(lflag, lidx, L + 1, s)) return rc;
        int64_t n_light_recv = 0;
        GMSX_HIP(hipMemcpy(&n_light_recv, lidx + L, sizeof(int64_t), hipMemcpyDeviceToHost));
        const int64_t n_recv = n_heavy + n_light_recv;
        int32_t *recv_v = nullptr;
        if (int rc = dmalloc(&recv_v, n_recv + 1, nullptr)) return rc;
        DevGuard g_rv{recv_v};
        if (std::max<int64_t>(n_heavy, L) > 0)
            hipLaunchKernelGGL(k_recv_vertices, dim3(unsigned(std::max<int64_t>(n_heavy, L) / 256 + 1)), dim3(256), 0, s, n_heavy, L, g->order, g->dplus, lidx, recv_v);
        {
            auto env_int = [](const char *name, int dflt) { return int(opt_int(name, dflt)); };
            g->tc_hot_windows = std::max(0, std::min(kMaxHotWindows, env_int("TC_HOT_WINDOWS", kDefaultHotWindows)));
            g->tc_window_units = uint32_t(std::max(1, env_int("TC_HOT_KB", kDefaultHotKB))) * 64u;
            g->tc_hot_min = std::max(1, env_int("TC_HOT_MIN", kDefaultHotMin));
        }
        const TcClasses cc{g->tc_hot_windows, g->tc_window_units, g->tc_hot_min};
        const int kClasses = cc.count();
        uint32_t *cnt = nullptr, *cur = nullptr;
        if (int rc = dmalloc(&cnt, n_recv * kClasses + 1, nullptr)) return rc;
        DevGuard g_cnt{cnt};
        if (int rc = dmalloc(&cur, n_recv * kClasses + 1, nullptr)) return rc;
        DevGuard g_cur{cur};
        GMSX_HIP(hipMemsetAsync(cnt, 0, size_t(n_recv * kClasses + 1) * sizeof(uint32_t), s));
        GMSX_HIP(hipMemsetAsync(cur, 0, size_t(n_recv * kClasses + 1) * sizeof(uint32_t), s));
        if (int rc = dmalloc(&g->tunits, n_heavy + 1, g)) return rc;
        GMSX_HIP(hipMemsetAsync(g->tunits, 0, size_t(n_heavy + 1) * sizeof(int32_t), s));
        unsigned long long *totals = nullptr;
        if (int rc = dmalloc(&totals, 4, nullptr)) return rc;
        DevGuard g_tot{totals};
        GMSX_HIP(hipMemsetAsync(totals, 0, 4 * sizeof(unsigned long long), s));
        int64_t *hcnt = nullptr, *tcnt = nullptr, *hbeg = nullptr, *tbeg = nullptr;
        if (int rc = dmalloc(&hcnt, n_recv + 1, nullptr)) return rc;
        DevGuard g_hc{hcnt};
        if (int rc = dmalloc(&tcnt, n_recv + 1, nullptr)) return rc;
        DevGuard g_tc{tcnt};
        if (int rc = dmalloc(&hbeg, n_recv + 1, nullptr)) return rc;
        DevGuard g_hb{hbeg};
        if (int rc = dmalloc(&tbeg, n_recv + 1, nullptr)) return rc;
        DevGuard g_tb{tbeg};
        const int grid = grid_for_waves(n_heavy);
        if (g->spool_units + kPoolSlack >= (int64_t(1) << 32) || g->tpool_units + kPoolSlack >= (int64_t(1) << 32)) return GMSX_ERR_DEVICE_MEM;
        {
            uint32_t hub_max = kTaskHubUnitsMax, tail_max = kTaskTailUnitsMax;
            if (const char *e = opt("TC_TEST_MAX_UNITS")) hub_max = tail_max = uint32_t(std::max(1, std::atoi(e)));
            if (n > 0) hipLaunchKernelGGL(k_task_limits, dim3(vb), dim3(256), 0, s, n, g->srow, g->srow2, g->trow, hub_max, tail_max, totals + 3);
        }
        if (n > 0)
            hipLaunchKernelGGL(k_inline_entries<false>, dim3(vb), dim3(256), 0, s, n, g->dplus, opos, lidx, n_heavy, g->inline_limit, ihoff, itoff, inline_h_base,
                               inline_t_base, cnt, cur, hbeg, tbeg, TaskList{}, TaskList{}, totals, cc);
        if (n_heavy > 0)
            hipLaunchKernelGGL(k_task_lists<false>, dim3(grid), dim3(256), 0, s, n_heavy, g->order, g->hoff, g->hadj, g->toff, g->tadj, g->dplus, g->srow, g->srow2, g->ksplit, g->trow,
                               two_sided, opos, cnt, cur, hbeg, tbeg, TaskList{}, TaskList{}, g->tunits,
                               totals + 2, g->spool, g->tpool, g->inline_limit, g->inline_first, g->shard_nparts, g->shard_part, cc);
        pt.mark("task lists count");
        hipLaunchKernelGGL(k_list_sizes, dim3(unsigned(n_recv / 256 + 1)), dim3(256), 0, s, n_recv, cnt, hcnt, tcnt, cc);
        if (int rc = exclusive_scan_i64(hcnt, hbeg, n_recv + 1, s)) return rc;
        if (int rc = exclusive_scan_i64(tcnt, tbeg, n_recv + 1, s)) return rc;
        unsigned long long tot[4] = {0, 0, 0, 0};
        GMSX_HIP(hipMemcpy(&g->htask_entries, hbeg + n_recv, sizeof(int64_t), hipMemcpyDeviceToHost));
        GMSX_HIP(hipMemcpy(&g->ttask_entries, tbeg + n_recv, sizeof(int64_t), hipMemcpyDeviceToHost));
        GMSX_HIP(hipMemcpy(tot, totals, sizeof(tot), hipMemcpyDeviceToHost));
        if (tot[3]) return GMSX_ERR_UNSUPPORTED;
        g->inline_hentries = int64_t(tot[0]);
        g->inline_tentries = int64_t(tot[1]);
        g->task_reverse = int64_t(tot[2]);
        if (g->htask_entries >= (int64_t(1) << 40) || g->ttask_entries >= (int64_t(1) << 40)) return GMSX_ERR_DEVICE_MEM;
        if (int rc = dmalloc(&g->htask.lo, g->htask_entries + 2, g)) return rc;
        if (int rc = dmalloc(&g->htask.hi, g->htask_entries + 2, g)) return rc;
        if (int rc = dmalloc(&g->ttask.lo, g->ttask_entries + 2, g)) return rc;
        if (int rc = dmalloc(&g->ttask.hi, g->ttask_entries + 2, g)) return rc;
        if (n > 0)
            hipLaunchKernelGGL(k_inline_entries<true>, dim3(vb), dim3(256), 0, s, n, g->dplus, opos, lidx, n_heavy, g->inline_limit, ihoff, itoff, inline_h_base,
                               inline_t_base, cnt, cur, hbeg, tbeg, g->htask, g->ttask, totals, cc);
        if (n_heavy > 0)
            hipLaunchKernelGGL(k_task_lists<true>, dim3(grid), dim3(256), 0, s, n_heavy, g->order, g->hoff, g->hadj, g->toff, g->tadj, g->dplus, g->srow, g->srow2, g->ksplit, g->trow,
                               two_sided, opos, cnt, cur, hbeg, tbeg, g->htask, g->ttask, g->tunits, totals + 2, g->spool, g->tpool, g->inline_limit, g->inline_first, g->shard_nparts, g->shard_part, cc);
        pt.mark("task lists fill");
        const int hub_phases = cc.hub_phases();
        const int64_t slots = int64_t(hub_phases) * n_recv;
        int64_t *icnt = nullptr, *ioff = nullptr;
        if (int rc = dmalloc(&icnt, slots + 1, nullptr)) return rc;
        DevGuard g_ic{icnt};
        if (int rc = dmalloc(&ioff, slots + 1, nullptr)) return rc;
        DevGuard g_io{ioff};
        const unsigned rb = unsigned(n_recv / 256 + 1);
        hipLaunchKernelGGL(k_item_counts, dim3(rb), dim3(256), 0, s, n_recv, hbeg, cnt, cc, hub_phases, icnt);
        if (int rc = exclusive_scan_i64(icnt, ioff, slots + 1, s)) return rc;
        GMSX_HIP(hipMemcpy(&g->hitems, ioff + slots, sizeof(int64_t), hipMemcpyDeviceToHost));
        if (int rc = dmalloc(&g->hitem, g->hitems + 1, g)) return rc;
        if (n_recv > 0) hipLaunchKernelGGL(k_item_fill, dim3(rb), dim3(256), 0, s, n_recv, recv_v, opos, hbeg, ioff, g->htask, g->hoff, 0, cnt, cc, hub_phases, g->hitem);
        hipLaunchKernelGGL(k_item_counts, dim3(rb), dim3(256), 0, s, n_recv, tbeg, cnt, cc, 1, icnt);
        if (int rc = exclusive_scan_i64(icnt, ioff, n_recv + 1, s)) return rc;
        GMSX_HIP(hipMemcpy(&g->titems, ioff + n_recv, sizeof(int64_t), hipMemcpyDeviceToHost));
        if (int rc = dmalloc(&g->titem, g->titems + 1, g)) return rc;
        if (n_recv > 0) hipLaunchKernelGGL(k_item_fill, dim3(rb), dim3(256), 0, s, n_recv, recv_v, opos, tbeg, ioff, g->ttask, g->toff, 1, cnt, cc, 1, g->titem);
        if (g->hitems >= (int64_t(1) << 31) || g->titems >= (int64_t(1) << 31)) return GMSX_ERR_DEVICE_MEM;
        GMSX_HIP(hipStreamSynchronize(s));
    }
    pt.mark("work items");
    GMSX_HIP(hipStreamSynchronize(s));
    GMSX_HIP(hipGetLastError());
    {
        auto drop = [&](auto *&p, size_t bytes) {
            if (!p) return;
            (void)hipFree(p);
            p = nullptr;
            g->device_bytes -= int64_t(bytes);
        };
        const size_t nn = size_t(n > 0 ? n : 1);
        drop(g->tsplit, nn * sizeof(int32_t));
        drop(g->srow2, nn * sizeof(unsigned long long));
        const char *keep = opt("TC_KEEP_ROWS");
        if (!(keep && std::atoi(keep) != 0)) {
            drop(g->srow, nn * sizeof(unsigned long long));
            drop(g->trow, nn * sizeof(unsigned long long));
        }
        drop(g->ksplit, size_t(n + 1) * sizeof(int32_t));
    }
    return GMSX_OK;
}

static int build_tc_once(gmsx_graph *g) {
    g->tc_base_bytes = g->device_bytes;
    g->tc_building = true;
    const int rc = build_tc_sets(g);
    g->tc_building = false;
    g->tc_bytes = g->device_bytes - g->tc_base_bytes;
    if (rc) {
        free_tc(g);
        return rc;
    }
    g->tc_ready = true;
    return GMSX_OK;
}

int ensure_tc(const gmsx_graph *cg) {
    gmsx_graph *g = const_cast<gmsx_graph *>(cg);
    if (g->tc_ready) return GMSX_OK;
    if (const char *e = opt("TC_MEM_LIMIT_MB")) {
        const long long v = std::atoll(e);
        g->tc_limit_bytes = v > 0 ? int64_t(v) << 20 : 0;
    }
    int rc = build_tc_once(g);
    if (rc == GMSX_ERR_DEVICE_MEM && g->shard_nparts == 1) {
        (void)hipGetLastError();
        for (int k = 2; k <= 4096 && rc == GMSX_ERR_DEVICE_MEM; k *= 2) {
            g->shard_part = 0;
            g->shard_nparts = k;
            rc = build_tc_once(g);
            if (rc == GMSX_OK) g->tc_passes = k;
        }
        if (rc) {
            g->shard_part = 0;
            g->shard_nparts = 1;
        }
    }
    return rc;
}

__global__ void k_shard_flags(int64_t n_items, const gmsx_tc_item *__restrict__ items, int nparts, int part, int64_t *__restrict__ flags) {
    const int64_t i = int64_t(blockIdx.x) * blockDim.x + threadIdx.x;
    if (i <= n_items) flags[i] = (i < n_items && shard_of(items[i].pos, nparts) == part) ? 1 : 0;
}
__global__ void k_shard_scatter(int64_t n_items, const int64_t *__restrict__ flags, const int64_t *__restrict__ slot, const gmsx_tc_item *__restrict__ items,
                                gmsx_tc_item *__restrict__ out) {
    const int64_t i = int64_t(blockIdx.x) * blockDim.x + threadIdx.x;
    if (i < n_items && flags[i]) out[slot[i]] = items[i];
}
int tc_shard_items(const gmsx_graph *g, int part, int nparts) {
    if (g->shard_idx_part == part && g->shard_idx_nparts == nparts) return GMSX_OK;
    hipStream_t s = ctx().stream;
    (void)hipFree(g->shard_hitem);
    (void)hipFree(g->shard_titem);
    g->shard_hitem = g->shard_titem = nullptr;
    g->shard_idx_part = g->shard_idx_nparts = -1;
    auto one = [&](const gmsx_tc_item *items, int64_t n_items, gmsx_tc_item **idx, int64_t *count) -> int {
        *count = 0;
        if (n_items == 0) return GMSX_OK;
        int64_t *flags = nullptr, *slot = nullptr;
        if (int rc = dmalloc(&flags, n_items + 1, nullptr)) return rc;
        DevGuard g_f{flags};
        if (int rc = dmalloc(&slot, n_items + 1, nullptr)) return rc;
        DevGuard g_s{slot};
        hipLaunchKernelGGL(k_shard_flags, dim3(unsigned(n_items / 256 + 1)), dim3(256), 0, s, n_items, items, nparts, part, flags);
        if (int rc = exclusive_scan_i64(flags, slot, n_items + 1, s)) return rc;
        GMSX_HIP(hipMemcpy(count, slot + n_items, sizeof(int64_t), hipMemcpyDeviceToHost));
        if (int rc = dmalloc(idx, *count + 1, nullptr)) return rc;
        hipLaunchKernelGGL(k_shard_scatter, dim3(unsigned(n_items / 256 + 1)), dim3(256), 0, s, n_items, flags, slot, items, *idx);
        GMSX_HIP(hipStreamSynchronize(s));
        return GMSX_OK;
    };
    if (int rc = one(g->hitem, g->hitems, &g->shard_hitem, &g->shard_hitems)) return rc;
    if (int rc = one(g->titem, g->titems, &g->shard_titem, &g->shard_titems)) return rc;
    g->shard_idx_part = part;
    g->shard_idx_nparts = nparts;
    return GMSX_OK;
}

int ensure_tc_shard(const gmsx_graph *cg, int part, int nparts) {
    gmsx_graph *g = const_cast<gmsx_graph *>(cg);
    if (g->tc_ready && g->shard_part == part && g->shard_nparts == nparts) return GMSX_OK;
    free_tc(g);
    g->shard_part = part;
    g->shard_nparts = nparts;
    return build_tc_once(g);
}

int count_dplus_ge(const gmsx_graph *g, int32_t threshold, int64_t *out) {
    if (g->n == 0) {
        *out = 0;
        return GMSX_OK;
    }
    for (int i = 0; i < g->ge_used; ++i)
        if (g->ge_thr[i] == threshold) {
            *out = g->ge_cnt[i];
            return GMSX_OK;
        }
    hipStream_t s = ctx().stream;
    hipLaunchKernelGGL(k_count_ge, dim3(1), dim3(1), 0, s, g->n, g->order, g->dplus, threshold, reinterpret_cast<int64_t *>(g->scratch + 8));
    GMSX_HIP(hipMemcpyAsync(out, g->scratch + 8, sizeof(int64_t), hipMemcpyDeviceToHost, s));
    GMSX_HIP(hipStreamSynchronize(s));
    if (g->ge_used < 40) {
        g->ge_thr[g->ge_used] = threshold;
        g->ge_cnt[g->ge_used] = *out;
        ++g->ge_used;
    }
    return GMSX_OK;
}

// ... 167 lines not shown
```

gms_amd/csrc/hip/device_graph.hpp:

```cpp
#pragma once
#include <hip/hip_runtime.h>

#include <cstdint>

#include "gmsx.h"
#include "gmsx_internal.hpp"

#if !defined(GMSX_DEV_HOOKS) &&                                                                                                               \
    (defined(GMSX_KC_NO_PROBE) || defined(GMSX_KC_NO_HITS) || defined(GMSX_KC_NO_TAIL) || defined(GMSX_KC_NO_INNER) || defined(GMSX_KC_CELLS_ONLY) ||   \
     defined(GMSX_KC_NO_ROWS) || defined(GMSX_KC_BUILD_ONLY) || defined(GMSX_KC_NO_SLAB_CALL) || defined(GMSX_KC_NO_PAIRS) || defined(GMSX_KC_SLAB_ROW_SCAN) || \
     defined(GMSX_BK_AB) || defined(GMSX_BK_NO_HIT_ATOMICS) || defined(GMSX_BK_STATS) || defined(GMSX_TC_NO_PROBE) || defined(GMSX_TC_STAGING_ONLY))
#error "A/B switches need -DGMSX_DEV_HOOKS (tools/ab_lib.sh sets it); the default build of libgmsx.so carries none of them"
#endif

struct __attribute__((aligned(64))) gmsx_tc_item {
    uint64_t bc;
    uint64_t cont;
    int32_t pivot;
    int32_t pos;
    uint32_t kind;
    uint16_t fbeg[4];
    uint32_t reserved[7];
};
static_assert(sizeof(gmsx_tc_item) == 64, "work item record = one 64-byte line");
constexpr uint32_t kTaskHubUnitsMax = (1u << 14) - 1, kTaskTailUnitsMax = (1u << 15) - 1;
struct TaskList {
    uint32_t *lo = nullptr;
    uint16_t *hi = nullptr;
    bool tail = false;
    __host__ __device__ TaskList at(int64_t first) const { return TaskList{lo + first, hi + first, tail}; }
    __device__ __forceinline__ unsigned long long get(int64_t i) const {
        const uint32_t l = lo[i], h = hi[i];
        const unsigned long long first = ((unsigned long long)h << 16) | (l >> 16);
        const uint32_t form = tail ? ((l >> 15) & 1u) << 1 : (l >> 14) & 3u, units = tail ? l & kTaskTailUnitsMax : l & kTaskHubUnitsMax;
        return (first << 24) | ((unsigned long long)form << 22) | units;
    }
    __device__ __forceinline__ void put(int64_t i, unsigned long long d) const {
        const uint32_t first = uint32_t(d >> 24), form = (uint32_t(d) >> 22) & 3u, units = uint32_t(d) & 0x3fffffu;
        lo[i] = (first << 16) | (tail ? (form >> 1) << 15 : form << 14) | units;
        hi[i] = uint16_t(first >> 16);
    }
};
struct gmsx_graph {
    int64_t n = 0, nnz = 0, m = 0;
    int64_t *off = nullptr;
    int32_t *adj = nullptr;
    int32_t *newid = nullptr;
    int32_t *oldid = nullptr;
    int64_t *hoff = nullptr;
    uint16_t *hadj = nullptr;
    int64_t *toff = nullptr;
    int32_t *tadj = nullptr;
    int64_t *bmoff = nullptr;
    uint32_t *bmpool = nullptr;
    int32_t dense_limit = 0;
    int32_t bitset_limit = 0;
    unsigned long long *srow = nullptr;
    unsigned long long *srow2 = nullptr;
    int32_t *ksplit = nullptr;
    uint32_t *spool = nullptr;
    int64_t spool_units = 0;
    TaskList htask{nullptr, nullptr, false};
    TaskList ttask{nullptr, nullptr, true};
    int64_t htask_entries = 0, ttask_entries = 0;
    struct gmsx_tc_item *hitem = nullptr, *titem = nullptr;
    int64_t hitems = 0, titems = 0;
    int64_t inline_hentries = 0, inline_tentries = 0;
    mutable struct gmsx_tc_item *shard_hitem = nullptr, *shard_titem = nullptr;
    mutable int64_t shard_hitems = 0, shard_titems = 0;
    mutable int shard_idx_part = -1, shard_idx_nparts = -1;
    int32_t *tunits = nullptr;
    int64_t task_reverse = 0;
    uint4 *ledge = nullptr;
    int64_t n_ledge = 0, ledge_total = 0;
    int tc_hot_windows = 0;
    uint32_t tc_window_units = 1;
    int tc_hot_min = 0;
    int inline_first = 64;
    int32_t inline_limit = 0;
    int64_t inline_units = 0;
    unsigned long long *trow = nullptr;
    uint32_t *tpool = nullptr;
    int64_t tpool_units = 0;
    int32_t *tsplit = nullptr;
    int64_t dense_rows = 0, bmpool_words = 0;
    bool rows_sorted = false;
    int32_t *dplus = nullptr;
    int32_t *order = nullptr;
    int64_t hub_entries = 0, tail_entries = 0;
    int32_t max_dplus = 0;
    int32_t max_deg = 0;
    mutable bool kc_rev_tried = false;
    mutable uint32_t *kc_rel = nullptr;
    mutable int64_t *kc_aoff = nullptr;
    mutable uint32_t *kc_arena = nullptr;
    mutable ulonglong2 *kc_rec = nullptr;
    mutable uint4 *kc_item = nullptr;
    mutable uint32_t *kc_relt = nullptr;
    mutable ulonglong2 *kc_rect = nullptr;
    mutable uint4 *kc_itemt = nullptr;
    mutable int64_t kc_recst = 0, kc_itemst = 0;
    mutable int64_t kc_recs = 0, kc_items = 0, kc_arena_words = 0, kc_rev_bytes = 0;
    mutable double kc_rev_build_ms = 0.0;
    unsigned long long *scratch = nullptr;
    unsigned long long *acc = nullptr;
    mutable int32_t ge_thr[40] = {0};
    mutable int64_t ge_cnt[40] = {0};
    mutable int ge_used = 0;
    mutable int stats_part = -1, stats_nparts = -1;
    mutable uint64_t stats_units = 0, stats_probes = 0, stats_bytes = 0;
    int shard_part = 0, shard_nparts = 1;
    int tc_passes = 1;
    int64_t tc_limit_bytes = 0, tc_base_bytes = 0;
    bool tc_building = false;
    bool tc_ready = false;
    int64_t tc_bytes = 0;
    int hub_limit = 0;
    uint32_t upload_flags = 0;
    uint64_t alg_elements = 0;
    int64_t device_bytes = 0;
};

namespace gmsx {

static constexpr int kHub = 65535;
static constexpr int kBitmapWords = 2048;
static constexpr int kAccWords = 64 * 16 + 16;
static constexpr int kFormList = 0, kFormBitset = 1, kFormDelta = 2, kFormGap12 = 3;
static constexpr int kPoolSlack = 64;
static constexpr int kTaskChunk = 512;
static constexpr int kLenClasses = 12;
static constexpr int kHubClasses = 4 * kLenClasses, kTailClasses = 2 * kLenClasses;
static constexpr int kMaxHotWindows = 8;
struct TcClasses {
    int hot_windows;
    uint32_t window_units;
    int hot_min;
    __host__ __device__ int hub_phases() const { return hot_windows + 1; }
    __host__ __device__ int tail_base() const { return hub_phases() * kHubClasses; }
    __host__ __device__ int count() const { return tail_base() + kTailClasses; }
    __host__ __device__ int phase(unsigned long long d) const {
        if (hot_windows <= 0) return 0;
        const unsigned long long w = (d >> 24) / window_units;
        return w < (unsigned long long)hot_windows ? int(w) : hot_windows;
    }
};
__host__ __device__ inline int length_class(uint32_t u) {
    return u <= 16 ? (u <= 4 ? 0 : u <= 8 ? 1 : u <= 12 ? 2 : 3) : u <= 64 ? (u <= 24 ? 4 : u <= 32 ? 5 : u <= 48 ? 6 : 7) : (u <= 96 ? 8 : u <= 128 ? 9 : u <= 192 ? 10 : 11);
}
__host__ __device__ inline int hub_class(const TcClasses &cc, unsigned long long d) {
    return cc.phase(d) * kHubClasses + int((uint32_t(d) >> 22) & 3u) * kLenClasses + length_class(uint32_t(d) & 0x3fffffu);
}
__host__ __device__ inline int tail_class(const TcClasses &cc, unsigned long long d) {
    return cc.tail_base() + (((uint32_t(d) >> 22) & 3u) == 2u ? kLenClasses : 0) + length_class(uint32_t(d) & 0x3fffffu);
}
__host__ __device__ inline void hub_phase_range(const TcClasses &cc, const uint32_t *c, int64_t len, int ph, int64_t *b, int64_t *e) {
    int64_t start = 0;
    for (int q = 0;; ++q) {
        const int64_t end = q < cc.hot_windows ? int64_t(c[(q + 1) * kHubClasses]) : len;
        const bool own = q == cc.hot_windows || end - start >= cc.hot_min;
        if (q == ph) {
            *b = start;
            *e = own ? end : start;
            return;
        }
        if (own) start = end;
    }
}
__host__ __device__ inline int shard_of(int64_t pos, int nparts) {
    const int j = int(pos % nparts);
    return ((pos / nparts) & 1) ? nparts - 1 - j : j;
}
static constexpr int kHeavy = 64;
static constexpr int kDeltaIds = 14;

__host__ __device__ inline int64_t bitset_words(int32_t v) { return ((int64_t(v) + 31) / 32 + 3) & ~int64_t(3); }

struct Ctx {
    int device = -1;
    hipStream_t stream = nullptr;
    hipStream_t own_stream = nullptr;
    hipEvent_t ev[4] = {nullptr, nullptr, nullptr, nullptr};
    hipStream_t side[2] = {nullptr, nullptr};
    hipEvent_t ev_fork = nullptr, ev_join[2] = {nullptr, nullptr};
    int compute_units = 0;
};
Ctx &ctx();
int ensure_init();
int kclique_vertex_counts(const gmsx_graph *g, unsigned long long *d_counts, gmsx_stats *st);
int count_dplus_ge(const gmsx_graph *g, int32_t threshold, int64_t *out);
int exclusive_scan_i64(const int64_t *in, int64_t *out, int64_t count, hipStream_t s);
int ensure_tc(const gmsx_graph *g);
int ensure_tc_shard(const gmsx_graph *g, int part, int nparts);
int tc_shard_items(const gmsx_graph *g, int part, int nparts);
int tc_vertex_counts_device(const gmsx_graph *g, unsigned long long *d_counts, gmsx_stats *st);
int tc_full_partial(const gmsx_graph *g, int part, int nparts, uint64_t *partial, gmsx_stats *st);

__device__ __forceinline__ int uni32(int x) { return __builtin_amdgcn_readfirstlane(x); }
__device__ __forceinline__ uint32_t uni32(uint32_t x) { return uint32_t(__builtin_amdgcn_readfirstlane(int(x))); }
__device__ __forceinline__ int64_t uni64(int64_t x) {
    const uint32_t lo = uint32_t(__builtin_amdgcn_readfirstlane(int(uint32_t(uint64_t(x)))));
    const uint32_t hi = uint32_t(__builtin_amdgcn_readfirstlane(int(uint32_t(uint64_t(x) >> 32))));
    return int64_t((uint64_t(hi) << 32) | lo);
}
__device__ __forceinline__ unsigned long long uni64(unsigned long long x) { return (unsigned long long)uni64(int64_t(x)); }

#define GMSX_HIP(call)                                                    \
    do {                                                                  \
        hipError_t e_ = (call);                                           \
        if (e_ != hipSuccess) {                                           \
            (void)hipGetLastError();                                      \
            return e_ == hipErrorOutOfMemory ? GMSX_ERR_DEVICE_MEM : GMSX_ERR_KERNEL; \
        }                                                                 \
    } while (0)

}
```

gms_amd/csrc/hip/tc.hip:

```cpp
#include "device_graph.hpp"

#include <algorithm>
#include <type_traits>
#include <rocprim/device/device_radix_sort.hpp>
#include <rocprim/device/device_reduce.hpp>
#include <rocprim/device/device_reduce_by_key.hpp>
#include <cstdio>
#include <cstdlib>
#include <cstring>

namespace gmsx {

static constexpr int kAccSlots = 64;
static constexpr int kAccStride = 16;

struct __attribute__((packed, aligned(4))) u4u { uint32_t x, y, z, w; };

__device__ __forceinline__ int64_t readlane64(int64_t x, int l) {
    const uint32_t lo = __builtin_amdgcn_readlane(uint32_t(uint64_t(x)), l);
    const uint32_t hi = __builtin_amdgcn_readlane(uint32_t(uint64_t(x) >> 32), l);
    return int64_t((uint64_t(hi) << 32) | lo);
}

__device__ __forceinline__ uint32_t bit_lo(const uint32_t *bm, uint32_t p) {
    const uint32_t word = bm[(p >> 5) & 0x7ffu];
    return __builtin_amdgcn_ubfe(word, p, 1u);
}
__device__ __forceinline__ uint32_t bit_hi(const uint32_t *bm, uint32_t p) {
    const uint32_t q = p >> 16;
    const uint32_t word = bm[q >> 5];
    return __builtin_amdgcn_ubfe(word, q & 31u, 1u);
}
__device__ __forceinline__ uint32_t hub_hits8(const uint32_t *bm, u4u p) {
    return bit_lo(bm, p.x) + bit_hi(bm, p.x) + bit_lo(bm, p.y) + bit_hi(bm, p.y) + bit_lo(bm, p.z) + bit_hi(bm, p.z) +
           bit_lo(bm, p.w) + bit_hi(bm, p.w);
}

__device__ __forceinline__ uint32_t delta_unit_hits(const uint32_t *bm, uint4 p) {
    uint32_t id[14];
    id[0] = p.x & 0xffffu;
    id[1] = id[0] + (p.x >> 24);
    id[2] = id[1] + (p.y & 0xffu);
    id[3] = id[2] + ((p.y >> 8) & 0xffu);
    id[4] = id[3] + ((p.y >> 16) & 0xffu);
    id[5] = id[4] + (p.y >> 24);
    id[6] = id[5] + (p.z & 0xffu);
    id[7] = id[6] + ((p.z >> 8) & 0xffu);
    id[8] = id[7] + ((p.z >> 16) & 0xffu);
    id[9] = id[8] + (p.z >> 24);
    id[10] = id[9] + (p.w & 0xffu);
    id[11] = id[10] + ((p.w >> 8) & 0xffu);
    id[12] = id[11] + ((p.w >> 16) & 0xffu);
    id[13] = id[12] + (p.w >> 24);
    uint32_t w[14];
#pragma unroll
    for (int k = 0; k < 14; ++k) w[k] = bm[id[k] >> 5];
    uint32_t hits = 0;
#pragma unroll
    for (int k = 0; k < 14; ++k) hits |= __builtin_amdgcn_ubfe(w[k], id[k], 1u) << k;
    const uint32_t n = (p.x >> 16) & 0xffu;
    return uint32_t(__popc(hits & ((1u << n) - 1u)));
}

__device__ __forceinline__ uint32_t gap12_unit_hits(const uint32_t *bm, uint4 p) {
    uint32_t id[10];
    id[0] = p.x & 0xffffu;
    id[1] = id[0] + (p.x >> 20);
    id[2] = id[1] + (p.y & 0xfffu);
    id[3] = id[2] + __builtin_amdgcn_ubfe(p.y, 12u, 12u);
    id[4] = id[3] + (__builtin_amdgcn_alignbit(p.z, p.y, 24u) & 0xfffu);
    id[5] = id[4] + __builtin_amdgcn_ubfe(p.z, 4u, 12u);
    id[6] = id[5] + __builtin_amdgcn_ubfe(p.z, 16u, 12u);
    id[7] = id[6] + (__builtin_amdgcn_alignbit(p.w, p.z, 28u) & 0xfffu);
    id[8] = id[7] + __builtin_amdgcn_ubfe(p.w, 8u, 12u);
    id[9] = id[8] + (p.w >> 20);
    uint32_t w[10];
#pragma unroll
    for (int k = 0; k < 10; ++k) w[k] = bm[id[k] >> 5];
    uint32_t hits = 0;
#pragma unroll
    for (int k = 0; k < 10; ++k) hits |= __builtin_amdgcn_ubfe(w[k], id[k], 1u) << k;
    const uint32_t n = (p.x >> 16) & 0xfu;
    return uint32_t(__popc(hits & ((1u << n) - 1u)));
}

__device__ __forceinline__ uint32_t hash_slot(int32_t w, int shift) { return (uint32_t(w) * 0x9E3779B1u) >> shift; }

__device__ __forceinline__ void set_insert(int32_t *tbl, uint32_t mask, int shift, int32_t w) {
    uint32_t h = hash_slot(w, shift);
    while (atomicCAS(&tbl[h], -1, w) != -1) h = (h + 1) & mask;
}
__device__ __forceinline__ uint32_t set_contains(const int32_t *tbl, uint32_t mask, int shift, int32_t w) {
    uint32_t h = hash_slot(w, shift), found = 0u;
    bool go;
    do {
        const int32_t x = tbl[h];
        found |= x == w ? 1u : 0u;
        go = x != w && x != -1;
        h = (h + 1) & mask;
    } while (go);
    return found;
}
static constexpr int kFilterWords = 1024;
__device__ __forceinline__ uint32_t flt_word(const uint32_t *flt, uint32_t id) { return flt[(id >> 5) & uint32_t(kFilterWords - 1)] >> (id & 31u); }
__device__ __forceinline__ uint32_t pick(uint32_t c, uint32_t x, uint32_t y) { return x ^ ((x ^ y) & (0u - c)); }
__device__ __forceinline__ uint32_t probe_set_bits(const int32_t *tbl, uint32_t mask, int shift, uint32_t m, const uint32_t (&id)[6]) {
    uint32_t c = 0;
    while (m) {
        const uint32_t k = uint32_t(__ffs(int(m)) - 1);
        m &= m - 1u;
        const uint32_t b0 = k & 1u, b1 = (k >> 1) & 1u, b2 = k >> 2;
        const uint32_t w = pick(b2, pick(b1, pick(b0, id[0], id[1]), pick(b0, id[2], id[3])), pick(b0, id[4], id[5]));
        c += set_contains(tbl, mask, shift, int32_t(w));
    }
    return c;
}
__device__ __forceinline__ uint32_t tail_unit_hits(const uint32_t *flt, const int32_t *tbl, uint32_t mask, int shift, uint4 p) {
    const uint32_t w0 = flt_word(flt, p.x), w1 = flt_word(flt, p.y), w2 = flt_word(flt, p.z), w3 = flt_word(flt, p.w);
    if (((w0 | w1 | w2 | w3) & 1u) == 0) return 0u;
    const uint32_t id[6] = {p.x, p.y, p.z, p.w, 0u, 0u};
    return probe_set_bits(tbl, mask, shift, (w0 & 1u) | ((w1 & 1u) << 1) | ((w2 & 1u) << 2) | ((w3 & 1u) << 3), id);
}
__device__ __forceinline__ uint32_t tail_delta_unit_hits(const uint32_t *flt, const int32_t *tbl, uint32_t mask, int shift, uint4 p) {
    const uint32_t id0 = p.x, id1 = id0 + (p.y >> 16), id2 = id1 + (p.z & 0xffffu), id3 = id2 + (p.z >> 16), id4 = id3 + (p.w & 0xffffu),
                   id5 = id4 + (p.w >> 16);
    const uint32_t w0 = flt_word(flt, id0), w1 = flt_word(flt, id1), w2 = flt_word(flt, id2), w3 = flt_word(flt, id3), w4 = flt_word(flt, id4),
                   w5 = flt_word(flt, id5);
    if (((w0 | w1 | w2 | w3 | w4 | w5) & 1u) == 0) return 0u;
    const uint32_t n = p.y & 0xffu;
    const uint32_t m = ((w0 & 1u) | ((w1 & 1u) << 1) | ((w2 & 1u) << 2) | ((w3 & 1u) << 3) | ((w4 & 1u) << 4) | ((w5 & 1u) << 5)) & ((1u << n) - 1u);
    const uint32_t id[6] = {id0, id1, id2, id3, id4, id5};
    return probe_set_bits(tbl, mask, shift, m, id);
}
static constexpr int kBlockLog = 10;
template <int FORM>
__device__ __forceinline__ uint32_t hub_unit_hits(const uint32_t *bm, uint4 p, int j) {
    if (FORM == kFormBitset) {
        const uint4 q = *reinterpret_cast<const uint4 *>(bm + 4 * j);
        return uint32_t(__popc(p.x & q.x) + __popc(p.y & q.y) + __popc(p.z & q.z) + __popc(p.w & q.w));
    }
    if (FORM == kFormDelta) return delta_unit_hits(bm, p);
    if (FORM == kFormGap12) return gap12_unit_hits(bm, p);
    return hub_hits8(bm, u4u{p.x, p.y, p.z, p.w});
}
template <int FORM>
__device__ __forceinline__ uint32_t tail_unit_hits_f(const uint32_t *flt, const int32_t *tbl, uint32_t mask, int shift, uint4 p) {
    return FORM == kFormDelta ? tail_delta_unit_hits(flt, tbl, mask, shift, p) : tail_unit_hits(flt, tbl, mask, shift, p);
}
#ifndef GMSX_TC_TAIL_DEPTH
#define GMSX_TC_TAIL_DEPTH 1
#endif
#ifndef GMSX_TC_HUB_GROUP
#define GMSX_TC_HUB_GROUP 16
// ... 353 lines not shown
                if (neA > nl) {
                    st.start(sd, oddA, pool, nl, neA, tid);
                    c += st.run([=](uint4 p, int, int) { return tail_delta_unit_hits(flt, tbl, mask, shift, p); });
                }
#endif
            }
            if (!staged) {
                __syncthreads();
                if (vB) stage(L.rec[rb], buf ^ 1, lane, wave);
                if (fetch) L.chunk[1] = pend < unsigned(n_items) ? int(pend) : -1;
            }
        }
        total += c;
        ra = rb;
        vA = vB;
        vB = vC;
        buf ^= 1;
    }
}

#ifndef GMSX_TC_HUB_MIN_WAVES
#define GMSX_TC_HUB_MIN_WAVES 8
#endif
#ifndef GMSX_TC_TAIL_MIN_WAVES
#define GMSX_TC_TAIL_MIN_WAVES 8
#endif
template <bool TAIL>
__global__ __launch_bounds__(256) __attribute__((amdgpu_waves_per_eu(TAIL ? GMSX_TC_TAIL_MIN_WAVES : GMSX_TC_HUB_MIN_WAVES, 8))) void k_tc_items(
    const uint16_t *__restrict__ hadj, const int32_t *__restrict__ tadj, const uint32_t *__restrict__ pool, const TaskList task,
    const gmsx_tc_item *__restrict__ items, int n_items, unsigned int *__restrict__ qhead, unsigned long long *__restrict__ acc) {
    __shared__ __attribute__((aligned(16))) ItemLds L;
    const int tid = threadIdx.x;
    unsigned long long total = 0;
    item_loop<TAIL>(L, hadj, tadj, pool, task, items, n_items, qhead, total);
    block_add(total, L.red, tid & 63, tid >> 6, tid, acc);
}

template <int K>
__device__ __forceinline__ uint32_t ror_in_row(uint32_t x) {
    if constexpr (K == 0) return x;
    else return uint32_t(__builtin_amdgcn_mov_dpp(int(x), 0x120 + K, 0xf, 0xf, false));
}
__device__ __forceinline__ bool row_has(uint32_t a, uint32_t x) {
    bool m = false;
#define GMSX_ROT(K) m |= a == ror_in_row<K>(x);
    GMSX_ROT(0) GMSX_ROT(1) GMSX_ROT(2) GMSX_ROT(3) GMSX_ROT(4) GMSX_ROT(5) GMSX_ROT(6) GMSX_ROT(7)
    GMSX_ROT(8) GMSX_ROT(9) GMSX_ROT(10) GMSX_ROT(11) GMSX_ROT(12) GMSX_ROT(13) GMSX_ROT(14) GMSX_ROT(15)
#undef GMSX_ROT
    return m;
}
struct LightRows {
    uint32_t ah[4], at[4], bh[4], bt[4];
};
struct LightRec {
    uint4 r0, r1;
};
__global__ __launch_bounds__(256) void k_tc_light(const uint16_t *__restrict__ hadj, const int32_t *__restrict__ tadj, const uint4 *__restrict__ ledge, int nparts,
                                                  int part, int64_t count, unsigned long long *__restrict__ acc) {
    __shared__ unsigned long long red[4];
    const int tid = threadIdx.x, lane = tid & 63, wave = tid >> 6, sub = lane & 15;
    const int64_t ngroups = int64_t(gridDim.x) * 16, g0 = int64_t(blockIdx.x) * 16 + (tid >> 4);
    const int64_t trips = (count + ngroups - 1) / ngroups;
    auto load_rec = [&](int64_t t) -> LightRec {
        const int64_t k = g0 + t * ngroups;
        const int64_t kk = k < count ? k : 0;
        const int64_t e = nparts <= 1 ? kk : kk * nparts + ((kk & 1) ? nparts - 1 - part : part);
        LightRec r;
        r.r0 = ledge[2 * e];
        r.r1 = ledge[2 * e + 1];
        if (k >= count) {
            r.r0.y &= 0xffu;
            r.r0.w &= 0xffu;
            r.r1.y &= 0xffu;
            r.r1.w &= 0xffu;
        }
        return r;
    };
    auto wave_max = [](int x) {
        return max(max(__builtin_amdgcn_readlane(x, 0), __builtin_amdgcn_readlane(x, 16)), max(__builtin_amdgcn_readlane(x, 32), __builtin_amdgcn_readlane(x, 48)));
    };
    auto load_rows = [&](const LightRec &r) -> LightRows {
        const int64_t hu = int64_t((uint64_t(r.r0.y & 0xffu) << 32) | r.r0.x), tu = int64_t((uint64_t(r.r0.w & 0xffu) << 32) | r.r0.z);
        const int64_t hv = int64_t((uint64_t(r.r1.y & 0xffu) << 32) | r.r1.x), tv = int64_t((uint64_t(r.r1.w & 0xffu) << 32) | r.r1.z);
        const int hlu = int(r.r0.y >> 8), tlu = int(r.r0.w >> 8), hlv = int(r.r1.y >> 8), tlv = int(r.r1.w >> 8);
        const int more = wave_max((max(max(hlu, hlv), max(tlu, tlv)) + 15) >> 4);
        LightRows w;
        w.ah[0] = hadj[hlu ? hu + min(sub, hlu - 1) : 0];
        w.bh[0] = hadj[hlv ? hv + min(sub, hlv - 1) : 0];
        w.at[0] = uint32_t(tadj[tlu ? tu + min(sub, tlu - 1) : 0]);
        w.bt[0] = uint32_t(tadj[tlv ? tv + min(sub, tlv - 1) : 0]);
#pragma unroll
        for (int k = 1; k < 4; ++k) {
            w.ah[k] = w.bh[k] = w.at[k] = w.bt[k] = 0;
            if (k < more) {
                const int i = sub + 16 * k;
                w.ah[k] = hadj[hlu ? hu + min(i, hlu - 1) : 0];
                w.bh[k] = hadj[hlv ? hv + min(i, hlv - 1) : 0];
                w.at[k] = uint32_t(tadj[tlu ? tu + min(i, tlu - 1) : 0]);
                w.bt[k] = uint32_t(tadj[tlv ? tv + min(i, tlv - 1) : 0]);
            }
        }
        return w;
    };
    unsigned long long total = 0;
    if (trips > 0) {
        LightRec rec = load_rec(0);
        LightRows rows = load_rows(rec);
        LightRec rec_n = load_rec(1);
        for (int64_t t = 0; t < trips; ++t) {
            const LightRows rows_n = load_rows(rec_n);
            const LightRec rec_nn = load_rec(t + 2);
            const int hlu = int(rec.r0.y >> 8), tlu = int(rec.r0.w >> 8), hlv = int(rec.r1.y >> 8), tlv = int(rec.r1.w >> 8);
            const int nah = wave_max((hlu + 15) >> 4), nbh = wave_max((hlv + 15) >> 4), nat = wave_max((tlu + 15) >> 4), nbt = wave_max((tlv + 15) >> 4);
            uint32_t c = 0;
#pragma unroll
            for (int ka = 0; ka < 4; ++ka) {
                if (ka >= nah) break;
                const int ia = sub + 16 * ka;
                const uint32_t a = (ia < hlu && rows.ah[ka] != 0xFFFFu) ? rows.ah[ka] : 0xFFFFFFFFu;
                bool m = false;
#pragma unroll
                for (int kb = 0; kb < 4; ++kb) {
                    if (kb >= nbh) break;
                    const int ib = sub + 16 * kb;
                    const uint32_t x = (ib < hlv && rows.bh[kb] != 0xFFFFu) ? rows.bh[kb] : 0xFFFFFFFEu;
                    m |= row_has(a, x);
                }
                c += m ? 1u : 0u;
            }
#pragma unroll
            for (int ka = 0; ka < 4; ++ka) {
                if (ka >= nat) break;
                const int ia = sub + 16 * ka;
                const uint32_t a = ia < tlu ? rows.at[ka] : 0xFFFFFFFFu;
                bool m = false;
#pragma unroll
                for (int kb = 0; kb < 4; ++kb) {
                    if (kb >= nbt) break;
                    const int ib = sub + 16 * kb;
                    const uint32_t x = ib < tlv ? rows.bt[kb] : 0xFFFFFFFEu;
                    m |= row_has(a, x);
                }
                c += m ? 1u : 0u;
            }
            total += c;
            rec = rec_n;
            rows = rows_n;
            rec_n = rec_nn;
        }
    }
    block_add(total, red, lane, wave, tid, acc);
}

__global__ __launch_bounds__(256) void k_tc_stats(const int64_t *__restrict__ hoff, const uint16_t *__restrict__ hadj,
                                                  const int64_t *__restrict__ toff, const int32_t *__restrict__ tadj,
                                                  const int32_t *__restrict__ dplus, const int32_t *__restrict__ order,
                                                  const int32_t *__restrict__ tunits, int32_t inline_limit, int inline_first, int64_t end, int nparts, int part,
                                                  unsigned long long *__restrict__ out) {
    const int lane = threadIdx.x & 63;
    const int64_t wave0 = (int64_t(blockIdx.x) * blockDim.x + threadIdx.x) >> 6;
    const int64_t nwaves = (int64_t(gridDim.x) * blockDim.x) >> 6;
    unsigned long long units = 0, probes = 0, bytes = 0;
    for (int64_t pos = wave0; pos < end; pos += nwaves) {
        if (nparts > 1 && shard_of(pos, nparts) != part) continue;
        const int32_t u = order[pos];
        const int du = dplus[u];
        if (du >= kHeavy) {
            if (lane == 0) units += (unsigned long long)tunits[pos];
            const int hl = min(int(hoff[u + 1] - hoff[u]), inline_first), tl = min(int(toff[u + 1] - toff[u]), inline_first - hl);
            int32_t v = -1;
            if (lane < hl) {
                const uint32_t x = hadj[hoff[u] + lane];
                if (x != 0xFFFFu) v = int32_t(x);
            } else if (lane - hl < tl) v = tadj[toff[u] + lane - hl];
            if (v >= 0 && lane > 0 && (v < inline_limit || dplus[v] >= kHeavy)) ++units;
            continue;
        }
        const int hl = int(hoff[u + 1] - hoff[u]);
        if (lane == 0) units += (unsigned long long)du;
        if (du < 2) continue;
        for (int64_t j = toff[u] + lane; j < toff[u + 1]; j += 64) {
            const int32_t v = tadj[j];
            if (v < inline_limit || dplus[v] >= kHeavy) continue;
            const unsigned long long hv = (unsigned long long)(hoff[v + 1] - hoff[v]), tv = (unsigned long long)(toff[v + 1] - toff[v]);
            bytes += 32ull + 2ull * hl + 4ull * (unsigned long long)(j - toff[u]) + 2ull * hv + 4ull * tv;
            probes += hv + tv;
        }
    }
    for (int s = 32; s > 0; s >>= 1) {
        units += __shfl_down(units, s);
        probes += __shfl_down(probes, s);
        bytes += __shfl_down(bytes, s);
    }
    if (lane == 0) {
        if (units) atomicAdd(&out[0], units);
        if (probes) atomicAdd(&out[1], probes);
        if (bytes) atomicAdd(&out[2], bytes);
    }
}
__global__ __launch_bounds__(256) void k_tc_item_stats(const int64_t *__restrict__ coff, int bytes_per_id, int tail, const TaskList task,
                                                       const gmsx_tc_item *__restrict__ items, int64_t n_items, int nparts, int part,
                                                       unsigned long long *__restrict__ out) {
    const int lane = threadIdx.x & 63;
    const int64_t wave0 = (int64_t(blockIdx.x) * blockDim.x + threadIdx.x) >> 6;
    const int64_t nwaves = (int64_t(gridDim.x) * blockDim.x) >> 6;
    unsigned long long probes = 0, bytes = 0;
    auto slots = [tail](unsigned long long d) -> unsigned long long {
        const unsigned long long n = d & 0x3fffffull, f = (d >> 22) & 3ull;
        return n * (tail ? (f == kFormDelta ? 6ull : 4ull) : (f == kFormList ? 8ull : f == kFormDelta ? 14ull : f == kFormGap12 ? 10ull : 4ull));
    };
    for (int64_t q = wave0; q < n_items; q += nwaves) {
        const gmsx_tc_item &it = items[q];
        if (nparts > 1 && shard_of(it.pos, nparts) != part) continue;
        const int ne = int(it.bc >> 40);
        const int64_t b = int64_t(it.bc & 0xffffffffffull);
        if (lane == 0) bytes += (unsigned long long)bytes_per_id * (unsigned long long)(coff[it.pivot + 1] - coff[it.pivot]);
        for (int i = lane; i < ne; i += 64) {
            const unsigned long long d = task.get(b + i);
            bytes += 6ull + 16ull * (d & 0x3fffffull);
            probes += slots(d);
        }
    }
    for (int s = 32; s > 0; s >>= 1) {
        probes += __shfl_down(probes, s);
        bytes += __shfl_down(bytes, s);
    }
    if (lane == 0) {
        if (probes) atomicAdd(&out[1], probes);
        if (bytes) atomicAdd(&out[2], bytes);
    }
}

__global__ __launch_bounds__(256) void k_tc_breakdown(const int64_t *__restrict__ hoff, const int64_t *__restrict__ toff, const int32_t *__restrict__ tadj,
                                                      const int32_t *__restrict__ dplus, const int32_t *__restrict__ order,
                                                      const TaskList htask, const gmsx_tc_item *__restrict__ hitem, int64_t hitems,
                                                      const TaskList ttask, const gmsx_tc_item *__restrict__ titem, int64_t titems,
                                                      int32_t inline_limit, int64_t first_light, int64_t end_light,
                                                      unsigned long long *__restrict__ out) {
    const int lane = threadIdx.x & 63;
    const int64_t wave0 = (int64_t(blockIdx.x) * blockDim.x + threadIdx.x) >> 6;
    const int64_t nwaves = (int64_t(gridDim.x) * blockDim.x) >> 6;
    unsigned long long c[15] = {0, 0, 0, 0, 0, 0, 0, 0, 0, 0, 0, 0, 0, 0, 0};
    for (int64_t q = wave0; q < hitems + titems; q += nwaves) {
        const bool tail = q >= hitems;
        const gmsx_tc_item &it = tail ? titem[q - hitems] : hitem[q];
        const TaskList task = tail ? ttask : htask;
        const int ne = int(it.bc >> 40);
        const int64_t b0 = int64_t(it.bc & 0xffffffffffull);
        if (lane == 0) {
            c[6] += tail ? 4ull * (unsigned long long)(toff[it.pivot + 1] - toff[it.pivot]) : 2ull * (unsigned long long)(hoff[it.pivot + 1] - hoff[it.pivot]);
            c[11] += (unsigned long long)ne;
            c[13] += 1;
        }
        for (int i = lane; i < ne; i += 64) {
            const unsigned long long d = task.get(b0 + i);
            const unsigned long long db = 16ull * (d & 0x3fffffull);
            const int fd = int((d >> 22) & 3);
            if (tail) c[fd == kFormDelta ? 4 : 3] += db;
            else c[fd == kFormList ? 0 : fd == kFormBitset ? 1 : 2] += db;
            c[5] += 6;
        }
    }
    for (int64_t pos = first_light + wave0; pos < end_light; pos += nwaves) {
        const int32_t u = order[pos];
        const int64_t tb0 = toff[u], te = toff[u + 1];
        const unsigned long long hl = (unsigned long long)(hoff[u + 1] - hoff[u]);
        for (int64_t j = tb0 + lane; j < te; j += 64) {
            const int32_t v = tadj[j];
            if (v < inline_limit || dplus[v] >= kHeavy) continue;
            c[8] += 2ull * (unsigned long long)(hoff[v + 1] - hoff[v]);
            c[9] += 4ull * (unsigned long long)(toff[v + 1] - toff[v]);
            c[10] += 32ull + 2ull * hl + 4ull * (unsigned long long)(j - tb0);
            c[14] += 1;
        }
    }
    for (int k = 0; k < 15; ++k) {
        unsigned long long x = c[k];
        for (int s = 32; s > 0; s >>= 1) x += __shfl_down(x, s);
        if (lane == 0 && x) atomicAdd(&out[k], x);
    }
}

__device__ __forceinline__ int hist_bin(unsigned long long units) {
    if (units <= 16) return int(units) - 1;
    int b = 16;
    for (unsigned long long lim = 32; units > lim && b < 23; lim <<= 1) ++b;
    return b;
}
__global__ __launch_bounds__(256) void k_tc_comember_keys(const TaskList htask, const gmsx_tc_item *__restrict__ hitem, int64_t hitems, int batch,
                                                         unsigned long long *__restrict__ keys, uint32_t *__restrict__ vals, unsigned long long *__restrict__ sums) {
    unsigned long long ents = 0, units = 0;
    for (int64_t i = blockIdx.x; i < hitems; i += gridDim.x) {
        const gmsx_tc_item it = hitem[i];
        const unsigned long long first = it.bc & 0xffffffffffull;
        const int n = int(it.bc >> 40);
        const unsigned long long b = (unsigned long long)(it.pos / batch) << 40;
        for (int e = threadIdx.x; e < n; e += 256) {
            const unsigned long long d = htask.get(int64_t(first + e));
            keys[first + e] = b | (d >> 24);
            vals[first + e] = uint32_t(d & 0x3fffffull);
            ++ents;
            units += d & 0x3fffffull;
        }
    }
    for (int sft = 32; sft > 0; sft >>= 1) {
        ents += __shfl_xor(ents, sft);
        units += __shfl_xor(units, sft);
    }
    if ((threadIdx.x & 63) == 0) {
        atomicAdd(&sums[0], ents);
        atomicAdd(&sums[1], units);
    }
}
__global__ __launch_bounds__(256) void k_tc_sum_u32(const uint32_t *__restrict__ v, unsigned long long n, unsigned long long *__restrict__ out) {
    unsigned long long t = 0;
    for (unsigned long long i = (unsigned long long)blockIdx.x * 256 + threadIdx.x; i < n; i += (unsigned long long)gridDim.x * 256) t += v[i];
    for (int sft = 32; sft > 0; sft >>= 1) t += __shfl_xor(t, sft);
    if ((threadIdx.x & 63) == 0) atomicAdd(out, t);
}
__global__ __launch_bounds__(256) void k_tc_row_hist(const int64_t *__restrict__ hoff, const uint16_t *__restrict__ hadj,
                                                     const int64_t *__restrict__ toff, const int32_t *__restrict__ tadj,
                                                     const int32_t *__restrict__ dplus, const int32_t *__restrict__ order,
                                                     const unsigned long long *__restrict__ srow, const unsigned long long *__restrict__ trow,
                                                     const TaskList htask, const gmsx_tc_item *__restrict__ hitem, int64_t hitems,
                                                     const TaskList ttask, const gmsx_tc_item *__restrict__ titem, int64_t titems,
                                                     int64_t end, unsigned long long *__restrict__ out) {
    __shared__ unsigned long long h[256];
    for (int i = threadIdx.x; i < 256; i += 256) h[i] = 0;
    __syncthreads();
    const int lane = threadIdx.x & 63;
    const int64_t wave0 = (int64_t(blockIdx.x) * blockDim.x + threadIdx.x) >> 6;
    const int64_t nwaves = (int64_t(gridDim.x) * blockDim.x) >> 6;
    auto add = [&](int cls, unsigned long long units) {
        if (units == 0) return;
        const int b = (cls * 24 + hist_bin(units)) * 2;
        atomicAdd(&h[b], 1ull);
        atomicAdd(&h[b + 1], units);
    };
    for (int64_t q = wave0; q < hitems + titems; q += nwaves) {
        const bool tail = q >= hitems;
        const gmsx_tc_item &it = tail ? titem[q - hitems] : hitem[q];
        const TaskList task = tail ? ttask : htask;
        const int ne = int(it.bc >> 40);
        const int64_t b0 = int64_t(it.bc & 0xffffffffffull);
        if (lane == 0) {
            atomicAdd(&h[240], (unsigned long long)ne);
            atomicAdd(&h[242], 1ull);
            atomicAdd(&h[243], tail ? 4ull * (unsigned long long)(toff[it.pivot + 1] - toff[it.pivot]) : 2ull * (unsigned long long)(hoff[it.pivot + 1] - hoff[it.pivot]));
        }
        for (int i = lane; i < ne; i += 64) {
            const unsigned long long d = task.get(b0 + i);
            if (tail) add(((d >> 22) & 3) == kFormDelta ? 4 : 3, d & 0x3fffffull);
            else add(min(int((d >> 22) & 3), 2), d & 0x3fffffull);
        }
    }
    for (int64_t pos = wave0; pos < end; pos += nwaves) {
        if (!srow || !trow) break;
        const int32_t u = order[pos];
        const int du = dplus[u];
        if (du < 2) continue;
        const int64_t hb = hoff[u], tb = toff[u];
        const int hl = int(hoff[u + 1] - hb), tl = int(toff[u + 1] - tb);
        const unsigned long long su = (srow[u] & 0x3fffffull) + (trow[u] & 0x3fffffull);
        unsigned long long cur = 0, best = 0, cut = 0;
        for (int i = lane; i < hl + tl; i += 64) {
            int32_t v;
            if (i < hl) {
                const uint32_t x = hadj[hb + i];
                if (x == 0xFFFFu) continue;
                v = int32_t(x);
            } else v = tadj[tb + i - hl];
            const unsigned long long sv = (srow[v] & 0x3fffffull) + (trow[v] & 0x3fffffull);
            cur += sv;
            best += min(su, sv);
            cut += min(sv, dplus[v] >= kHeavy ? (su * (unsigned long long)i + du - 1) / (unsigned long long)du : ~0ull);
        }
        atomicAdd(&h[du >= kHeavy ? 248 : 250], cur);
        atomicAdd(&h[du >= kHeavy ? 249 : 251], best);
        if (du >= kHeavy) atomicAdd(&h[252], cut);
    }
    __syncthreads();
    for (int i = threadIdx.x; i < 256; i += 256)
        if (h[i]) atomicAdd(&out[i], h[i]);
}

static int tc_one(const gmsx_graph *g, int part, int nparts, uint64_t *partial, gmsx_stats *st);

static int tc_oriented(const gmsx_graph *g, int part, int nparts, uint64_t *partial, gmsx_stats *st) {
    if (int rc = ensure_tc(g)) return rc;
    if (g->tc_passes == 1) return tc_one(g, part, nparts, partial, st);
    if (nparts > 1) {
        auto restore = [&](int rc) {
            gmsx_graph *m = const_cast<gmsx_graph *>(g);
            if (m->tc_ready && m->shard_part == 0 && m->shard_nparts == m->tc_passes) return rc;
            (void)ensure_tc_shard(g, 0, g->tc_passes);
            return rc;
        };
        int J = nparts >= g->tc_passes ? 1 : (g->tc_passes + nparts - 1) / nparts;
        if (J > 1 && (J & 1)) ++J;
        for (;; J *= 2) {
            uint64_t total = 0;
            gmsx_stats sum{};
            int rc = GMSX_OK;
            for (int a = 0; a < J && rc == GMSX_OK; ++a) {
                const int sub = a * nparts + ((a & 1) ? nparts - 1 - part : part);
                rc = ensure_tc_shard(g, sub, nparts * J);
                if (rc) break;
                uint64_t pp = 0;
                gmsx_stats sp{};
                rc = tc_one(g, sub, nparts * J, &pp, st ? &sp : nullptr);
                total += pp;
                sum.kernel_ms += sp.kernel_ms;
                sum.setup_ms += sp.setup_ms;
                sum.units += sp.units;
                sum.probes += sp.probes;
                sum.stream_bytes += sp.stream_bytes;
                sum.launches += sp.launches;
            }
            if (rc == GMSX_ERR_DEVICE_MEM && nparts * J <= (1 << 20)) continue;
            if (rc) return restore(rc);
            *partial = total;
            if (st) *st = sum;
            return GMSX_OK;
        }
    }
    uint64_t total = 0;
    gmsx_stats sum{};
    for (int p = 0; p < g->tc_passes; ++p) {
        if (int rc = ensure_tc_shard(g, p, g->tc_passes)) return rc;
        uint64_t pp = 0;
        gmsx_stats sp{};
        if (int rc = tc_one(g, p, g->tc_passes, &pp, st ? &sp : nullptr)) return rc;
        total += pp;
        sum.kernel_ms += sp.kernel_ms;
        sum.setup_ms += sp.setup_ms;
        sum.units += sp.units;
        sum.probes += sp.probes;
        sum.stream_bytes += sp.stream_bytes;
        sum.launches += sp.launches;
    }
    *partial = total;
    if (st) {
        sum.alg_elements = g->alg_elements;
        *st = sum;
    }
    return GMSX_OK;
}

static int tc_one(const gmsx_graph *g, int part, int nparts, uint64_t *partial, gmsx_stats *st) {
    const bool use_idx = nparts > 1 && g->shard_nparts == 1;
    if (use_idx)
        if (int rc = tc_shard_items(g, part, nparts)) return rc;
    const gmsx_tc_item *hitem = use_idx ? g->shard_hitem : g->hitem, *titem = use_idx ? g->shard_titem : g->titem;
    int64_t n_hitems = use_idx ? g->shard_hitems : g->hitems, n_titems = use_idx ? g->shard_titems : g->titems;
#ifdef GMSX_DEV_HOOKS
    const char *only = std::getenv("GMSX_TC_ONLY");
    if (only) {
        if (std::strcmp(only, "hub") != 0) n_hitems = 0;
        if (std::strcmp(only, "tail") != 0) n_titems = 0;
    }
#else
    const char *only = nullptr;
#endif
    Ctx &c = ctx();
    hipStream_t s = c.stream;
    unsigned long long *acc = g->acc;
    static_assert(kAccSlots * kAccStride + 16 <= kAccWords, "gmsx_graph::acc too small");
    unsigned int *qhead = reinterpret_cast<unsigned int *>(acc + kAccSlots * kAccStride + 4);
    static_assert((kQueueStride + 1) * sizeof(unsigned int) <= 12 * sizeof(unsigned long long), "queue heads past gmsx_graph::acc");
    GMSX_HIP(hipEventRecord(c.ev[0], s));
    GMSX_HIP(hipMemsetAsync(acc, 0, sizeof(unsigned long long) * kAccWords, s));
    GMSX_HIP(hipEventRecord(c.ev[1], s));

    int launches = 0;
    const int cus = c.compute_units > 0 ? c.compute_units : 256;
    const int64_t cap_blocks = int64_t(cus) * 16;
    const bool run_light = !only || std::strcmp(only, "light") == 0;
    const bool strided = nparts > 1 && g->shard_nparts == 1;
    const int64_t cnt_light = [&]() -> int64_t {
        if (!run_light) return 0;
        if (!strided) return g->n_ledge;
        const int64_t full = g->n_ledge / nparts, rem = g->n_ledge % nparts;
        return full + (((full & 1) ? nparts - 1 - part : part) < rem ? 1 : 0);
    }();
    const int overlap = [] { const char *e = opt("TC_OVERLAP"); return e ? std::atoi(e) : 0; }();
    const int persist = [] { const char *e = opt("TC_PERSIST"); return e ? std::atoi(e) : 1; }();
    const bool sides = overlap && c.side[0] && c.side[1];
    struct Join {
        Ctx &c;
        hipStream_t s;
        bool armed[2] = {false, false};
        ~Join() {
            for (int i = 0; i < 2; ++i)
                if (armed[i] && hipEventRecord(c.ev_join[i], c.side[i]) == hipSuccess) (void)hipStreamWaitEvent(s, c.ev_join[i], 0);
        }
    } join{c, s};
    const bool side_light = sides && cnt_light > 0 && n_hitems + n_titems > 0;
    const bool side_tail = sides && !persist && n_hitems > 0 && n_titems > 0;
    if (side_light || side_tail) GMSX_HIP(hipEventRecord(c.ev_fork, s));
    if (side_tail) {
        GMSX_HIP(hipStreamWaitEvent(c.side[0], c.ev_fork, 0));
        join.armed[0] = true;
    }
    if (side_light) {
        GMSX_HIP(hipStreamWaitEvent(c.side[1], c.ev_fork, 0));
        join.armed[1] = true;
    }
    if (persist) {
        const int wgs_env = [] { const char *e = opt("TC_ITEM_WGS"); return e ? std::atoi(e) : 0; }();
        auto grid = [&](int64_t n, int wgs) {
            return unsigned(std::max<int64_t>(1, std::min<int64_t>((n + kGrab - 1) / kGrab, int64_t(cus) * (wgs_env > 0 ? wgs_env : wgs))));
        };
        if (n_hitems > 0) {
            hipLaunchKernelGGL(k_tc_items<false>, dim3(grid(n_hitems, GMSX_TC_HUB_MIN_WAVES)), dim3(256), 0, s, g->hadj, g->tadj, g->spool, g->htask, hitem, int(n_hitems), qhead, acc);
            ++launches;
        }
        if (n_titems > 0) {
            hipLaunchKernelGGL(k_tc_items<true>, dim3(grid(n_titems, GMSX_TC_TAIL_MIN_WAVES)), dim3(256), 0, s, g->hadj, g->tadj, g->tpool, g->ttask, titem, int(n_titems),
                               qhead + kQueueStride, acc);
            ++launches;
        }
    } else {
        if (n_hitems > 0) {
            hipLaunchKernelGGL(k_tc_block, dim3(unsigned(n_hitems)), dim3(256), 0, s, g->hoff, g->hadj, g->spool, g->htask, hitem, acc);
            ++launches;
        }
        if (n_titems > 0) {
            hipLaunchKernelGGL(k_tc_tail, dim3(unsigned(n_titems)), dim3(256), 0, side_tail ? c.side[0] : s, g->toff, g->tadj, g->tpool, g->ttask, titem, acc);
            ++launches;
        }
    }
    if (cnt_light > 0) {
        const int64_t blocks = std::min<int64_t>((cnt_light + 15) / 16, int64_t(cus) * 8);
        hipLaunchKernelGGL(k_tc_light, dim3(unsigned(blocks)), dim3(256), 0, side_light ? c.side[1] : s, g->hadj, g->tadj, g->ledge, strided ? nparts : 1,
                           strided ? part : 0, cnt_light, acc);
        ++launches;
    }
    for (int i = 0; i < 2; ++i)
        if (join.armed[i]) {
            join.armed[i] = false;
            GMSX_HIP(hipEventRecord(c.ev_join[i], c.side[i]));
            GMSX_HIP(hipStreamWaitEvent(s, c.ev_join[i], 0));
        }
    GMSX_HIP(hipEventRecord(c.ev[2], s));
    GMSX_HIP(hipGetLastError());

    const bool need_stats = st && !(g->stats_part == part && g->stats_nparts == nparts);
    if (need_stats) {
        if (g->n > 0) {
            const int64_t blocks = std::min<int64_t>((g->n + 3) / 4, cap_blocks);
            hipLaunchKernelGGL(k_tc_stats, dim3(unsigned(blocks)), dim3(256), 0, s, g->hoff, g->hadj, g->toff, g->tadj, g->dplus, g->order,
                               g->tunits, g->inline_limit, g->inline_first, g->n, nparts, part, acc + kAccSlots * kAccStride);
        }
        if (g->hitems > 0)
            hipLaunchKernelGGL(k_tc_item_stats, dim3(unsigned(std::min<int64_t>((g->hitems + 3) / 4, cap_blocks))), dim3(256), 0, s, g->hoff, 2, 0, g->htask, g->hitem,
                               g->hitems, nparts, part, acc + kAccSlots * kAccStride);
        if (g->titems > 0)
            hipLaunchKernelGGL(k_tc_item_stats, dim3(unsigned(std::min<int64_t>((g->titems + 3) / 4, cap_blocks))), dim3(256), 0, s, g->toff, 4, 1, g->ttask, g->titem,
                               g->titems, nparts, part, acc + kAccSlots * kAccStride);
    }
    unsigned long long host[kAccSlots * kAccStride + 3];
    GMSX_HIP(hipMemcpyAsync(host, acc, sizeof(host), hipMemcpyDeviceToHost, s));
    GMSX_HIP(hipStreamSynchronize(s));
    unsigned long long total = 0;
    for (int i = 0; i < kAccSlots; ++i) total += host[i * kAccStride];
    *partial = total;
    if (st) {
        float ms_setup = 0.f, ms_kernel = 0.f;
        GMSX_HIP(hipEventElapsedTime(&ms_setup, c.ev[0], c.ev[1]));
        GMSX_HIP(hipEventElapsedTime(&ms_kernel, c.ev[1], c.ev[2]));
        st->kernel_ms = ms_kernel;
        st->setup_ms = ms_setup;
        if (need_stats) {
            g->stats_part = part;
            g->stats_nparts = nparts;
            g->stats_units = host[kAccSlots * kAccStride];
            g->stats_probes = host[kAccSlots * kAccStride + 1];
            g->stats_bytes = host[kAccSlots * kAccStride + 2];
        }
        st->units = g->stats_units;
        st->probes = g->stats_probes;
        st->alg_elements = nparts == 1 ? g->alg_elements : 0;
        st->launches = launches;
        st->reserved = 0;
        st->stream_bytes = g->stats_bytes;
    }
    return GMSX_OK;
}

}

using namespace gmsx;

extern "C" {

int gmsx_tc_divisor(int algo) { return algo == GMSX_TC_FULL ? 3 : 1; }

int gmsx_tc_stream_breakdown(const gmsx_graph *g, uint64_t *out21) {
    return gmsx::guard([&]() -> int {
        if (!g || !out21) return GMSX_ERR_INVALID;
        if (int rc = ensure_init()) return rc;
        if (int rc = ensure_tc(g)) return rc;
        hipStream_t s = ctx().stream;
        std::memset(out21, 0, 21 * sizeof(uint64_t));
        if (g->n == 0) return GMSX_OK;
        int64_t n_block = 0, n_work = 0;
        if (int rc = count_dplus_ge(g, kHeavy, &n_block)) return rc;
        if (int rc = count_dplus_ge(g, 2, &n_work)) return rc;
        unsigned long long *acc = nullptr;
        GMSX_HIP(hipMalloc(reinterpret_cast<void **>(&acc), 21 * 8));
        struct Guard { void *p; ~Guard() { (void)hipFree(p); } } g1{acc};
        GMSX_HIP(hipMemsetAsync(acc, 0, 21 * 8, s));
        const int cus = ctx().compute_units > 0 ? ctx().compute_units : 256;
        hipLaunchKernelGGL(k_tc_breakdown, dim3(unsigned(cus * 16)), dim3(256), 0, s, g->hoff, g->toff, g->tadj, g->dplus, g->order, g->htask,
                           g->hitem, g->hitems, g->ttask, g->titem, g->titems, g->inline_limit, n_block, n_work, acc);
        GMSX_HIP(hipMemcpyAsync(out21, acc, 21 * 8, hipMemcpyDeviceToHost, s));
        GMSX_HIP(hipStreamSynchronize(s));
        GMSX_HIP(hipGetLastError());
        out21[7] = uint64_t(g->inline_units) * 16ull;
        out21[12] = uint64_t(g->inline_hentries + g->inline_tentries);
        return GMSX_OK;
    });
}

int gmsx_tc_row_histogram(const gmsx_graph *g, uint64_t *out256) {
    return gmsx::guard([&]() -> int {
        uint64_t *out248 = out256;
        if (!g || !out248) return GMSX_ERR_INVALID;
        if (int rc = ensure_init()) return rc;
        if (int rc = ensure_tc(g)) return rc;
        hipStream_t s = ctx().stream;
        std::memset(out248, 0, 256 * sizeof(uint64_t));
        if (g->n == 0) return GMSX_OK;
        unsigned long long *acc = nullptr;
        GMSX_HIP(hipMalloc(reinterpret_cast<void **>(&acc), 256 * 8));
        struct Guard { void *p; ~Guard() { (void)hipFree(p); } } g1{acc};
        GMSX_HIP(hipMemsetAsync(acc, 0, 256 * 8, s));
        const int cus = ctx().compute_units > 0 ? ctx().compute_units : 256;
        hipLaunchKernelGGL(k_tc_row_hist, dim3(unsigned(cus * 8)), dim3(256), 0, s, g->hoff, g->hadj, g->toff, g->tadj, g->dplus, g->order, g->srow, g->trow,
                           g->htask, g->hitem, g->hitems, g->ttask, g->titem, g->titems, g->n, acc);
        GMSX_HIP(hipGetLastError());
        GMSX_HIP(hipMemcpyAsync(out248, acc, 256 * 8, hipMemcpyDeviceToHost, s));
        GMSX_HIP(hipStreamSynchronize(s));
        GMSX_HIP(hipGetLastError());
        out248[241] = uint64_t(g->inline_hentries + g->inline_tentries);
        return GMSX_OK;
    });
}

int gmsx_tc_comembership(const gmsx_graph *g, int batch, uint64_t *out8) {
    return gmsx::guard([&]() -> int {
        if (!g || !out8 || batch < 1) return GMSX_ERR_INVALID;
        if (int rc = ensure_init()) return rc;
        if (int rc = ensure_tc(g)) return rc;
        hipStream_t s = ctx().stream;
        std::memset(out8, 0, 8 * sizeof(uint64_t));
        const int64_t ne = g->htask_entries;
        if (g->n == 0 || ne == 0 || g->hitems == 0) return GMSX_OK;
        struct Guard { void *p = nullptr; ~Guard() { (void)hipFree(p); } } gk0, gk1, gv0, gv1, gu, ga, gc, gt, gsum;
        unsigned long long *k0 = nullptr, *k1 = nullptr, *uk = nullptr, *cnt = nullptr, *sum = nullptr;
        uint32_t *v0 = nullptr, *v1 = nullptr, *agg = nullptr;
        GMSX_HIP(hipMalloc(reinterpret_cast<void **>(&k0), size_t(ne) * 8)); gk0.p = k0;
        GMSX_HIP(hipMalloc(reinterpret_cast<void **>(&k1), size_t(ne) * 8)); gk1.p = k1;
        GMSX_HIP(hipMalloc(reinterpret_cast<void **>(&v0), size_t(ne) * 4)); gv0.p = v0;
        GMSX_HIP(hipMalloc(reinterpret_cast<void **>(&v1), size_t(ne) * 4)); gv1.p = v1;
        GMSX_HIP(hipMalloc(reinterpret_cast<void **>(&sum), 4 * 8)); gsum.p = sum;
        GMSX_HIP(hipMemsetAsync(k0, 0xff, size_t(ne) * 8, s));
        GMSX_HIP(hipMemsetAsync(v0, 0, size_t(ne) * 4, s));
        GMSX_HIP(hipMemsetAsync(sum, 0, 4 * 8, s));
        hipLaunchKernelGGL(k_tc_comember_keys, dim3(unsigned(std::min<int64_t>(g->hitems, 1 << 20))), dim3(256), 0, s, g->htask, g->hitem, g->hitems, batch, k0, v0, sum);
        size_t tb = 0;
        GMSX_HIP(rocprim::radix_sort_pairs(nullptr, tb, k0, k1, v0, v1, size_t(ne), 0, 64, s));
        void *tmp = nullptr;
        GMSX_HIP(hipMalloc(&tmp, tb ? tb : 8)); gt.p = tmp;
        GMSX_HIP(rocprim::radix_sort_pairs(tmp, tb, k0, k1, v0, v1, size_t(ne), 0, 64, s));
        uk = k0;
        agg = v0;
        GMSX_HIP(hipMalloc(reinterpret_cast<void **>(&cnt), 8)); gc.p = cnt;
        size_t rb = 0;
        GMSX_HIP(rocprim::reduce_by_key(nullptr, rb, k1, v1, size_t(ne), uk, agg, cnt, rocprim::maximum<uint32_t>(), rocprim::equal_to<unsigned long long>(), s));
        void *tmp2 = nullptr;
        Guard g2;
        GMSX_HIP(hipMalloc(&tmp2, rb ? rb : 8)); g2.p = tmp2;
        GMSX_HIP(rocprim::reduce_by_key(tmp2, rb, k1, v1, size_t(ne), uk, agg, cnt, rocprim::maximum<uint32_t>(), rocprim::equal_to<unsigned long long>(), s));
        unsigned long long nuniq = 0;
        GMSX_HIP(hipMemcpyAsync(&nuniq, cnt, 8, hipMemcpyDeviceToHost, s));
        GMSX_HIP(hipStreamSynchronize(s));
        hipLaunchKernelGGL(k_tc_sum_u32, dim3(1024), dim3(256), 0, s, agg, (unsigned long long)nuniq, sum + 2);
        unsigned long long h[4] = {0, 0, 0, 0};
        GMSX_HIP(hipMemcpyAsync(h, sum, sizeof(h), hipMemcpyDeviceToHost, s));
        GMSX_HIP(hipStreamSynchronize(s));
        GMSX_HIP(hipGetLastError());
        out8[0] = uint64_t(h[0]);
        out8[1] = uint64_t(h[1]);
        out8[2] = uint64_t(nuniq);
        out8[3] = uint64_t(h[2]);
        out8[4] = uint64_t(g->hitems);
        return GMSX_OK;
    });
}

int gmsx_tc_partial(const gmsx_graph *g, int algo, int part, int nparts, uint64_t *partial, gmsx_stats *stats) {
    return gmsx::guard([&]() -> int {
        if (!g || !partial || nparts < 1 || part < 0 || part >= nparts) return GMSX_ERR_INVALID;
        if (algo != GMSX_TC_AUTO && algo != GMSX_TC_ORIENTED && algo != GMSX_TC_FULL) return GMSX_ERR_INVALID;
        if (int rc = ensure_init()) return rc;
        if (algo == GMSX_TC_FULL) return tc_full_partial(g, part, nparts, partial, stats);
        if (g->tc_passes == 1 && g->shard_nparts > 1 && (nparts != g->shard_nparts || part != g->shard_part)) return GMSX_ERR_INVALID;
        return tc_oriented(g, part, nparts, partial, stats);
    });
}

int gmsx_tc_total(const gmsx_graph *g, int algo, uint64_t *triangles, gmsx_stats *stats) {
    return gmsx::guard([&]() -> int {
        if (!triangles) return GMSX_ERR_INVALID;
        uint64_t partial = 0;
        if (int rc = gmsx_tc_partial(g, algo, 0, 1, &partial, stats)) return rc;
        const uint64_t div = uint64_t(gmsx_tc_divisor(algo));
        if (partial % div != 0) return GMSX_ERR_KERNEL;
        *triangles = partial / div;
        return GMSX_OK;
    });
}

}
```

gms_amd/csrc/host/loader.cpp:

```cpp
#include "gmsx_internal.hpp"

#include <fcntl.h>
#include <sys/mman.h>
#include <sys/stat.h>
#include <unistd.h>

#include <algorithm>
#ifdef _OPENMP
#include <parallel/algorithm>
#endif
#include <atomic>
#include <cerrno>
#include <cmath>
#include <cstdio>
#include <cstdlib>
#include <cstring>
#include <ctime>
#include <fstream>
#include <limits>
#include <memory>
#include <new>
#include <random>
#include <sstream>
#include <string>
// ... 501 lines not shown
        ++u;
    }
    return finish_el(us, vs, el);
}
static int read_mtx(const std::string &path, EdgeList &el) {
    std::ifstream in(path);
    if (!in.is_open()) return GMSX_ERR_IO;
    std::string start, object, format, field, symmetry, line;
    if (!(in >> start >> object >> format >> field >> symmetry)) return GMSX_ERR_FORMAT;
    if (start != "%%MatrixMarket" || object != "matrix" || format != "coordinate" || field == "complex") return GMSX_ERR_FORMAT;
    const bool weights = field == "real" || field == "double" || field == "integer";
    if (!weights && field != "pattern") return GMSX_ERR_FORMAT;
    if (symmetry != "symmetric" && symmetry != "general" && symmetry != "skew-symmetric") return GMSX_ERR_FORMAT;
    std::getline(in, line);
    long long rows = -1, cols = -1, nz = -1;
    while (std::getline(in, line)) {
        if (!line.empty() && line[0] == '%') continue;
        std::istringstream hs(line);
        if (!(hs >> rows >> cols >> nz)) return GMSX_ERR_FORMAT;
        break;
    }
    if (rows < 0 || rows != cols) return GMSX_ERR_FORMAT;
    std::vector<int32_t> us, vs;
    while (std::getline(in, line)) {
        std::istringstream ls(line);
        long long a, b;
        if (!(ls >> a >> b)) continue;
        if (int rc = push_edge(us, vs, a - 1, b - 1)) return rc;
        if (symmetry == "symmetric")
            if (int rc = push_edge(us, vs, b - 1, a - 1)) return rc;
    }
    return finish_el(us, vs, el);
}

static int validate_csr_arrays(const int64_t *off, const int32_t *ng, int64_t n, int64_t nnz);
static int read_sg(const std::string &path, Csr &g) {
    std::FILE *f = std::fopen(path.c_str(), "rb");
    if (!f) return GMSX_ERR_IO;
    struct Closer { std::FILE *f; ~Closer() { std::fclose(f); } } closer{f};
    unsigned char directed = 0;
    int64_t nnz = 0, n = 0;
    if (std::fread(&directed, 1, 1, f) != 1 || std::fread(&nnz, 8, 1, f) != 1 || std::fread(&n, 8, 1, f) != 1)
        return GMSX_ERR_FORMAT;
    if (n < 0 || nnz < 0 || n > std::numeric_limits<int32_t>::max()) return GMSX_ERR_FORMAT;
    if (int rc = alloc_csr(g, n, nnz)) return rc;
    if (std::fread(g.off.get(), 8, size_t(n + 1), f) != size_t(n + 1)) return GMSX_ERR_FORMAT;
    if (nnz && std::fread(g.neigh.get(), 4, size_t(nnz), f) != size_t(nnz)) return GMSX_ERR_FORMAT;
    if (int rc = validate_csr_arrays(g.off.get(), g.neigh.get(), n, nnz)) return rc;
    g.directed = directed != 0;
    return GMSX_OK;
}


static constexpr char kSgxMagic[8] = {'G', 'M', 'S', 'X', 'C', 'S', 'R', '1'};
static constexpr int64_t kSgxAlign = 64;
static int64_t sgx_neigh_offset(int64_t n) { return (kSgxAlign + (n + 1) * 8 + kSgxAlign - 1) / kSgxAlign * kSgxAlign; }

void ArrayFree::unmap(void *base, size_t bytes) { (void)munmap(base, bytes); }

static int write_sgx(const Csr &g, const char *path) {
    std::FILE *f = std::fopen(path, "wb");
    if (!f) return GMSX_ERR_IO;
    int64_t head[8] = {0, g.directed ? 1 : 0, g.n, g.nnz, 0, 0, 0, 0};
    std::memcpy(head, kSgxMagic, 8);
    const int64_t pad = sgx_neigh_offset(g.n) - (kSgxAlign + (g.n + 1) * 8);
    const char zeros[64] = {0};
    bool ok = std::fwrite(head, 8, 8, f) == 8 && std::fwrite(g.off.get(), 8, size_t(g.n + 1), f) == size_t(g.n + 1) &&
              (pad == 0 || std::fwrite(zeros, 1, size_t(pad), f) == size_t(pad)) &&
              (g.nnz == 0 || std::fwrite(g.neigh.get(), 4, size_t(g.nnz), f) == size_t(g.nnz));
    ok = (std::fclose(f) == 0) && ok;
    return ok ? GMSX_OK : GMSX_ERR_IO;
}

static int validate_csr_arrays(const int64_t *off, const int32_t *ng, int64_t n, int64_t nnz) {
    if (off[0] != 0 || off[n] != nnz) return GMSX_ERR_FORMAT;
    int bad = 0;
#pragma omp parallel for reduction(| : bad) schedule(static)
    for (int64_t u = 0; u < n; ++u) bad |= int(off[u + 1] < off[u]);
    if (bad) return GMSX_ERR_FORMAT;
#pragma omp parallel for reduction(| : bad) schedule(static)
    for (int64_t j = 0; j < nnz; ++j) bad |= int(ng[j] < 0 || int64_t(ng[j]) >= n);
    return bad ? GMSX_ERR_FORMAT : GMSX_OK;
}

static int read_sgx(const std::string &path, Csr &g) {
    const int fd = open(path.c_str(), O_RDONLY | O_CLOEXEC);
    if (fd < 0) return GMSX_ERR_IO;
    struct Closer { int fd; ~Closer() { close(fd); } } closer{fd};
    struct stat st;
    if (fstat(fd, &st) != 0) return GMSX_ERR_IO;
    int64_t head[8];
    if (pread(fd, head, sizeof(head), 0) != ssize_t(sizeof(head)) || std::memcmp(head, kSgxMagic, 8) != 0) return GMSX_ERR_FORMAT;
    const int64_t n = head[2], nnz = head[3];
    if (n < 0 || nnz < 0 || n > std::numeric_limits<int32_t>::max() || (head[1] != 0 && head[1] != 1)) return GMSX_ERR_FORMAT;
    const int64_t noff = sgx_neigh_offset(n);
    if (nnz > (std::numeric_limits<int64_t>::max() - noff) / 4 || int64_t(st.st_size) < noff + nnz * 4) return GMSX_ERR_FORMAT;
    const int64_t page = int64_t(sysconf(_SC_PAGESIZE));
    auto map_part = [&](int64_t at, int64_t bytes, void **base, size_t *len) -> void * {
        const int64_t lo = at / page * page;
        *len = size_t(at - lo + std::max<int64_t>(bytes, 1));
        *base = mmap(nullptr, *len, PROT_READ | PROT_WRITE, MAP_PRIVATE, fd, off_t(lo));
        if (*base == MAP_FAILED) return nullptr;
        (void)madvise(*base, *len, MADV_WILLNEED);
        return static_cast<char *>(*base) + (at - lo);
    };
    void *b0 = nullptr, *b1 = nullptr;
    size_t l0 = 0, l1 = 0;
    void *p_off = map_part(kSgxAlign, (n + 1) * 8, &b0, &l0);
    if (!p_off) return GMSX_ERR_NOMEM;
    g.off = std::unique_ptr<int64_t[], ArrayFree>(static_cast<int64_t *>(p_off), ArrayFree{b0, l0});
    void *p_ng = map_part(noff, nnz * 4, &b1, &l1);
    if (!p_ng) return GMSX_ERR_NOMEM;
    g.neigh = std::unique_ptr<int32_t[], ArrayFree>(static_cast<int32_t *>(p_ng), ArrayFree{b1, l1});
    g.n = n;
    g.nnz = nnz;
    g.directed = head[1] != 0;
    g.mapped = true;
    return validate_csr_arrays(g.off.get(), g.neigh.get(), n, nnz);
}

}

namespace gmsx {
int host_threads() {
#ifdef _OPENMP
    return omp_get_max_threads();
#else
    return 1;
#endif
}
void parallel_memcpy(void *dst, const void *src, size_t bytes) {
#ifdef _OPENMP
#pragma omp parallel
    {
        const size_t nt = size_t(omp_get_num_threads()), t = size_t(omp_get_thread_num());
        const size_t per = ((bytes + nt - 1) / nt + 4095) & ~size_t(4095), lo = std::min(bytes, per * t), hi = std::min(bytes, lo + per);
        if (hi > lo) std::memcpy(static_cast<char *>(dst) + lo, static_cast<const char *>(src) + lo, hi - lo);
    }
#else
    std::memcpy(dst, src, bytes);
#endif
}
namespace {
struct Option {
    const char *name;
    char value[32];
    bool set;
};
Option g_options[] = {
    {"TIMING", "", false}, {"MEM_TRACE", "", false}, {"BK_VERBOSE", "", false},
    {"INLINE_LIMIT", "", false}, {"TC_INLINE_FIRST", "", false}, {"TC_DELTA", "", false}, {"TC_DELTA_PCT", "", false}, {"TC_GAP12", "", false},
    {"TC_HYBRID", "", false}, {"TC_TAIL_DELTA", "", false}, {"TC_TWO_SIDED", "", false}, {"TC_HOT_WINDOWS", "", false}, {"TC_HOT_KB", "", false},
    {"TC_HOT_MIN", "", false}, {"TC_TEST_MAX_UNITS", "", false}, {"TC_KEEP_ROWS", "", false}, {"TC_MEM_LIMIT_MB", "", false}, {"TC_OVERLAP", "", false},
    {"TC_PERSIST", "", false}, {"TC_ITEM_WGS", "", false}, {"SORT_CHUNK", "", false}, {"UPLOAD_STAGED", "", false}, {"INIT_LAZY", "", false},
    {"KC_SLAB_MB", "", false}, {"KC_MAXD", "", false}, {"KC_STREAMS", "", false}, {"KC_PIPE_ALL", "", false}, {"KC_STREAM_BUILD", "", false},
    {"KC_REVERSE", "", false}, {"KC_REV_MIN", "", false}, {"KC_REV_FACTOR", "", false}, {"KC_REV_TAIL", "", false}, {"KC_REV_TAIL_MIN", "", false}, {"KC_REV_GW", "", false}, {"KC_TRI", "", false}, {"KC_MFMA", "", false}, {"KC_POOL_MB", "", false},
    {"BK_MAXC", "", false}, {"BK_ARENA_MB", "", false}, {"BK_GROUPS", "", false}, {"BK_SMALL_P", "", false}, {"BK_SMALL_P_GROUPS", "", false},
    {"BK_BUDGET", "", false}, {"BK_BUDGET0", "", false}, {"BK_RESUME_GRAB", "", false}, {"BK_SPLIT_BUILD", "", false}, {"BK_TINY_ROOTS", "", false},
    {"BK_TINY_BESIDE", "", false},
    {"BK_LIST_ARENA_MB", "", false},
    {"KCSTAR_SLAB_MB", "", false},
    {"CORE_WG_FRONTIER", "", false},
    {"COLOR_WG_FRONTIER", "", false},
    {"LP_LDS_MAXN", "", false}, {"LP_SLAB_MB", "", false},
};
Option *find_option(const char *name) {
    if (!name) return nullptr;
    for (Option &o : g_options)
        if (std::strcmp(o.name, name) == 0) return &o;
    return nullptr;
}
}

const char *opt(const char *name) {
    const Option *o = find_option(name);
    return o && o->set ? o->value : nullptr;
}

}

using namespace gmsx;

extern "C" {

int gmsx_csr_generate(int generator, int scale, int degree, int relabel, int threads, gmsx_csr **out) {
    return gmsx::guard([&]() -> int {
        if (!out || scale < 1 || degree < 1 || relabel < 0 || relabel > 2) return GMSX_ERR_INVALID;
        if (scale > 30) return GMSX_ERR_OVERFLOW;
        if (generator != GMSX_GEN_KRONECKER && generator != GMSX_GEN_UNIFORM) return GMSX_ERR_INVALID;
    #ifdef _OPENMP
        struct Threads {
            int saved, set;
            ~Threads() { if (set > 0) omp_set_num_threads(saved); }
        } threads_guard{omp_get_max_threads(), threads};
        if (threads > 0) omp_set_num_threads(threads);
    #else
        (void)threads;
    #endif
        int rc;
        {
            Csr g;
            {
                PhaseTimer pt;
                EdgeList el;
                rc = generator == GMSX_GEN_UNIFORM ? make_uniform(scale, degree, el) : make_rmat(scale, degree, el);
                pt.lap("generate edge list");
                if (!rc) rc = build_from_el(el, -1, true, g);
            }
            PhaseTimer pf;
            if (!rc) rc = finish(std::move(g), relabel, out);
            pf.lap("relabel decision + relabel");
        }
        return rc;
    });
}

int gmsx_csr_generate_rmat(int scale, int degree, double a, double b, double c, int relabel, int threads, gmsx_csr **out) {
    return gmsx::guard([&]() -> int {
        if (!out || scale < 1 || degree < 1 || relabel < 0 || relabel > 2) return GMSX_ERR_INVALID;
        if (!(a > 0 && b >= 0 && c >= 0 && a + b + c < 1.0)) return GMSX_ERR_INVALID;
        if (scale > 30) return GMSX_ERR_OVERFLOW;
    #ifdef _OPENMP
        struct Threads {
            int saved, set;
            ~Threads() { if (set > 0) omp_set_num_threads(saved); }
        } threads_guard{omp_get_max_threads(), threads};
        if (threads > 0) omp_set_num_threads(threads);
    #else
        (void)threads;
    #endif
        int rc;
        {
            Csr g;
            {
                EdgeList el;
                rc = make_rmat(scale, degree, el, float(a), float(b), float(c));
                if (!rc) rc = build_from_el(el, -1, true, g);
            }
            if (!rc) rc = finish(std::move(g), relabel, out);
        }
        return rc;
    });
}

int gmsx_csr_from_edges(int64_t num_nodes, int64_t num_edges, const int32_t *src, const int32_t *dst,
                        int symmetrize, int relabel, gmsx_csr **out) {
    return gmsx::guard([&]() -> int {
        if (!out || num_edges < 0 || (num_edges && (!src || !dst)) || relabel < 0 || relabel > 2) return GMSX_ERR_INVALID;
        EdgeList el;
        if (int rc = el.alloc(num_edges)) return rc;
        if (num_edges) {
            std::memcpy(el.u.get(), src, size_t(num_edges) * 4);
            std::memcpy(el.v.get(), dst, size_t(num_edges) * 4);
        }
        Csr g;
        if (int rc = build_from_el(el, num_nodes, symmetrize != 0, g)) return rc;
        return finish(std::move(g), relabel, out);
    });
}

int gmsx_csr_load(const char *path, int symmetrize, int relabel, gmsx_csr **out) {
    return gmsx::guard([&]() -> int {
        if (!path || !out || relabel < 0 || relabel > 2) return GMSX_ERR_INVALID;
        const std::string p(path), suf = suffix_of(p);
        Csr g;
        if (suf == ".sg") {
            if (int rc = read_sg(p, g)) return rc;
        } else if (suf == ".sgx") {
            if (int rc = read_sgx(p, g)) return rc;
        } else if (suf == ".el" || suf == ".wel" || suf == ".gr" || suf == ".graph" || suf == ".mtx") {
            EdgeList el;
            const int rc = suf == ".el" ? read_el(p, el) : suf == ".wel" ? read_wel(p, el) : suf == ".gr" ? read_gr(p, el)
                         : suf == ".graph" ? read_metis(p, el) : read_mtx(p, el);
            if (rc) return rc;
            if (int rc2 = build_from_el(el, -1, symmetrize != 0, g)) return rc2;
        } else {
            return GMSX_ERR_FORMAT;
        }
        return finish(std::move(g), relabel, out);
    });
}

int gmsx_csr_save_sg(const gmsx_csr *h, const char *path) {
    return gmsx::guard([&]() -> int {
        if (!h || !path) return GMSX_ERR_INVALID;
        std::FILE *f = std::fopen(path, "wb");
        if (!f) return GMSX_ERR_IO;
        const Csr &g = h->g;
        const unsigned char directed = g.directed ? 1 : 0;
        bool ok = std::fwrite(&directed, 1, 1, f) == 1 && std::fwrite(&g.nnz, 8, 1, f) == 1 &&
                  std::fwrite(&g.n, 8, 1, f) == 1 && std::fwrite(g.off.get(), 8, size_t(g.n + 1), f) == size_t(g.n + 1) &&
                  (g.nnz == 0 || std::fwrite(g.neigh.get(), 4, size_t(g.nnz), f) == size_t(g.nnz));
        ok = (std::fclose(f) == 0) && ok;
        return ok ? GMSX_OK : GMSX_ERR_IO;
    });
}

int gmsx_csr_save_sgx(const gmsx_csr *h, const char *path) {
    return gmsx::guard([&]() -> int {
        if (!h || !path) return GMSX_ERR_INVALID;
        return write_sgx(h->g, path);
    });
}
int gmsx_csr_is_mapped(const gmsx_csr *h) { return h ? int(h->g.mapped) : GMSX_ERR_INVALID; }

int gmsx_csr_from_arrays(int64_t n, const int64_t *offsets, const int32_t *neigh, gmsx_csr **out) {
    return gmsx::guard([&]() -> int {
// ... 111 lines not shown
```

Before: 15.74 billion.

## Count triangles among top hub core via dense bitmatrix MFMA kernel

Adds a dense adjacency bit-matrix for the first K (highest-degree) vertices and a new k_tc_core kernel that counts triangles inside this core with MFMA-style bit matrix products. Rows in the core are then skipped by the inline, light-edge and task-list builders. K is picked at prepare time by a cost model that weighs the streamed bytes saved against K^3 bit-MAC work plus launch overhead. The aim is to move dense hub intersections off the bandwidth-bound list path, at the cost of extra device memory, another kernel, and a host sync during setup.

```diff
diff --git a/gms_amd/capi.py b/gms_amd/capi.py
--- a/gms_amd/capi.py
+++ b/gms_amd/capi.py
@@ -424,9 +424,9 @@
     BREAKDOWN = ["hub_rows_list", "hub_rows_bitset", "hub_rows_delta", "tail_rows_list", "tail_rows_delta", "entries", "pivot_containers",
                  "of_which_inline_rows", "light_streamed_hub_rows", "light_streamed_tail_rows", "light_pivot_lists_and_descriptors",
                  "count_entries", "count_inline_entries", "count_work_items", "count_light_streamed_members",
-                 "reserved15", "reserved16", "reserved17", "reserved18", "reserved19", "reserved20"]
+                 "core_matrix", "core_k", "reserved17", "reserved18", "reserved19", "reserved20"]
     BREAKDOWN_BYTES = ("hub_rows_list", "hub_rows_bitset", "hub_rows_delta", "tail_rows_list", "tail_rows_delta", "entries", "pivot_containers",
-                       "light_streamed_hub_rows", "light_streamed_tail_rows", "light_pivot_lists_and_descriptors")
+                       "light_streamed_hub_rows", "light_streamed_tail_rows", "light_pivot_lists_and_descriptors", "core_matrix")
 
     def tc_stream_breakdown(self):
         out = np.zeros(21, dtype=np.uint64)
diff --git a/gms_amd/csrc/hip/device_graph.hip b/gms_amd/csrc/hip/device_graph.hip
--- a/gms_amd/csrc/hip/device_graph.hip
+++ b/gms_amd/csrc/hip/device_graph.hip
@@ -17,6 +17,8 @@
 #include <rocprim/iterator/transform_iterator.hpp>
 
 #include "../host/gmsx_internal.hpp"
+#include "../host/tc_core_plan.hpp"
+#include "kc4_mfma.hpp"
 
 namespace gmsx {
 
@@ -409,6 +411,36 @@
         }
     }
 }
+__global__ __launch_bounds__(256) void k_core_fill(int32_t K, int WS, const int64_t *__restrict__ hoff, const uint16_t *__restrict__ hadj,
+                                                   uint32_t *__restrict__ bits) {
+    const int lane = threadIdx.x & 63;
+    const int32_t wave0 = int32_t((int64_t(blockIdx.x) * blockDim.x + threadIdx.x) >> 6);
+    const int32_t nwaves = int32_t((int64_t(gridDim.x) * blockDim.x) >> 6);
+    for (int32_t i = wave0; i < K; i += nwaves)
+        for (int64_t j = hoff[i] + lane; j < hoff[i + 1]; j += 64) {
+            const uint32_t id = hadj[j];
+            if (id < uint32_t(i)) atomicOr(&bits[size_t(i) * size_t(WS) + (id >> 5)], 1u << (id & 31u));
+        }
+}
+__global__ __launch_bounds__(256) void k_core_units(int32_t cap, const int64_t *__restrict__ hoff, const uint16_t *__restrict__ hadj,
+                                                    const int32_t *__restrict__ dplus, unsigned long long *__restrict__ bucket) {
+    const int lane = threadIdx.x & 63;
+    const int32_t wave0 = int32_t((int64_t(blockIdx.x) * blockDim.x + threadIdx.x) >> 6);
+    const int32_t nwaves = int32_t((int64_t(gridDim.x) * blockDim.x) >> 6);
+    for (int32_t u = wave0; u < cap; u += nwaves) {
+        const int64_t hb = hoff[u];
+        const int hl = int(hoff[u + 1] - hb);
+        unsigned long long units = 0;
+        for (int i = lane; i < hl; i += 64) {
+            const uint32_t v = hadj[hb + i];
+            if (v >= uint32_t(u)) continue;
+            const uint32_t ids = uint32_t(min(i, dplus[v]));
+            units += min((ids + 7u) / 8u, (v + 127u) / 128u);
+        }
+        for (int s = 32; s > 0; s >>= 1) units += __shfl_down(units, s);
+        if (lane == 0 && units) atomicAdd(&bucket[u / kTcCoreBucket], units);
+    }
+}
 __global__ __launch_bounds__(256) void k_tail_split(int64_t n, const int64_t *__restrict__ toff, const int32_t *__restrict__ tadj, int32_t limit,
                                                     int32_t *__restrict__ tsplit) {
     const int lane = threadIdx.x & 63;
@@ -457,7 +489,7 @@
 template <bool FILL>
 __global__ __launch_bounds__(256) void k_inline_rows(int64_t first, int64_t end, const int32_t *__restrict__ order, const int64_t *__restrict__ hoff,
                                                      const uint16_t *__restrict__ hadj, const int64_t *__restrict__ toff, const int32_t *__restrict__ tadj,
-                                                     const int32_t *__restrict__ dplus, int32_t inline_limit, int inline_first, const int32_t *__restrict__ opos, int nparts, int part,
+                                                     const int32_t *__restrict__ dplus, int32_t inline_limit, int inline_first, int32_t core, const int32_t *__restrict__ opos, int nparts, int part,
                                                      unsigned long long *__restrict__ cnt_h,
                                                      unsigned long long *__restrict__ cnt_t, const int64_t *__restrict__ ihoff,
                                                      const int64_t *__restrict__ itoff, int64_t base_h, uint16_t *__restrict__ pool_h, int64_t base_t,
@@ -467,6 +499,7 @@
     const int64_t nwaves = (int64_t(gridDim.x) * blockDim.x) >> 6;
     for (int64_t pos = first + wave0; pos < end; pos += nwaves) {
         const int32_t u = order[pos];
+        if (u < core) continue;
         const int64_t hb = hoff[u], tb = toff[u];
         const int first_u = dplus[u] >= kHeavy ? inline_first : kInlineFirstMax;
         const int hl = min(int(hoff[u + 1] - hb), first_u), tl = min(int(toff[u + 1] - tb), first_u - hl);
@@ -576,7 +609,7 @@
 }
 
 __global__ void k_ledge_count(int64_t first, int64_t end, const int32_t *__restrict__ order, const int64_t *__restrict__ toff, const int32_t *__restrict__ tadj,
-                              const int32_t *__restrict__ tsplit, const int32_t *__restrict__ dplus, int64_t *__restrict__ cnt) {
+                              const int32_t *__restrict__ tsplit, const int32_t *__restrict__ dplus, int32_t core, int64_t *__restrict__ cnt) {
     const int64_t pos = first + int64_t(blockIdx.x) * blockDim.x + threadIdx.x;
     if (pos > end) return;
     int64_t c = 0;
@@ -584,16 +617,18 @@
         const int32_t u = order[pos];
         const int64_t tb = toff[u];
         const int tl = int(toff[u + 1] - tb);
-        for (int i = tsplit[u]; i < tl; ++i) c += dplus[tadj[tb + i]] < kHeavy ? 1 : 0;
+        if (u >= core)
+            for (int i = tsplit[u]; i < tl; ++i) c += dplus[tadj[tb + i]] < kHeavy ? 1 : 0;
     }
     cnt[pos - first] = c;
 }
 __global__ void k_ledge_fill(int64_t first, int64_t end, const int32_t *__restrict__ order, const int64_t *__restrict__ hoff, const int64_t *__restrict__ toff,
                              const int32_t *__restrict__ tadj, const int32_t *__restrict__ tsplit, const int32_t *__restrict__ dplus,
-                             const int64_t *__restrict__ ebeg, int nparts, int part, uint4 *__restrict__ ledge) {
+                             int32_t core, const int64_t *__restrict__ ebeg, int nparts, int part, uint4 *__restrict__ ledge) {
     const int64_t pos = first + int64_t(blockIdx.x) * blockDim.x + threadIdx.x;
     if (pos >= end) return;
     const int32_t u = order[pos];
+    if (u < core) return;
     const int64_t hb = hoff[u], tb = toff[u];
     const int tl = int(toff[u + 1] - tb);
     const unsigned long long hu = (unsigned long long)hb | ((unsigned long long)(hoff[u + 1] - hb) << 40);
@@ -660,7 +695,7 @@
                                                     uint32_t *__restrict__ cnt, uint32_t *__restrict__ cur, const int64_t *__restrict__ hbeg,
                                                     const int64_t *__restrict__ tbeg, TaskList htask, TaskList ttask,
                                                     int32_t *__restrict__ tunits, unsigned long long *__restrict__ reversed, const uint32_t *__restrict__ spool,
-                                                    const uint32_t *__restrict__ tpool, int32_t inline_limit, int inline_first, int nparts, int part, TcClasses cc) {
+                                                    const uint32_t *__restrict__ tpool, int32_t inline_limit, int inline_first, int32_t core, int nparts, int part, TcClasses cc) {
     const int kClasses = cc.count();
     const int lane = threadIdx.x & 63;
     const int64_t wave0 = (int64_t(blockIdx.x) * blockDim.x + threadIdx.x) >> 6;
@@ -668,6 +703,7 @@
     unsigned long long rev = 0;
     for (int64_t pos = wave0; pos < n_heavy; pos += nwaves) {
         const int32_t u = order[pos];
+        if (u < core) continue;
         const int64_t hb = hoff[u], tb = toff[u];
         const int hl = int(hoff[u + 1] - hb), tl = int(toff[u + 1] - tb);
         const unsigned long long du_s = srow[u], du_s2 = srow2[u], du_t = trow[u];
@@ -815,7 +851,8 @@
         p = nullptr;
     };
     drop(g->tsplit); drop(g->srow); drop(g->srow2); drop(g->ksplit); drop(g->spool); drop(g->trow); drop(g->htask.lo); drop(g->htask.hi); drop(g->ttask.lo); drop(g->ttask.hi); drop(g->hitem); drop(g->titem); drop(g->tunits);
-    drop(g->ledge); drop(g->tpool); drop(g->shard_hitem); drop(g->shard_titem);
+    drop(g->ledge); drop(g->tpool); drop(g->shard_hitem); drop(g->shard_titem); drop(g->core_bits);
+    g->tc_core = 0;
     g->shard_idx_part = g->shard_idx_nparts = -1;
     g->device_bytes -= g->tc_bytes;
     g->tc_bytes = 0;
@@ -854,6 +891,7 @@
     (void)hipFree(g->shard_hitem);
     (void)hipFree(g->shard_titem);
     (void)hipFree(g->ledge);
+    (void)hipFree(g->core_bits);
     (void)hipFree(g->tpool);
     (void)hipFree(g->dplus);
     (void)hipFree(g->order);
@@ -1201,6 +1239,37 @@
     if (int rc = dmalloc(&opos, n + 1, nullptr)) return rc;
     DevGuard g_opos{opos};
     if (n > 0) hipLaunchKernelGGL(k_opos, dim3(tb), dim3(256), 0, s, n, g->order, opos);
+    {
+        long long want = kTcCoreDefault;
+        if (const char *e = opt("TC_CORE")) want = std::atoll(e);
+        g->tc_core = 0;
+        if (want > 0) g->tc_core = tc_core_clamp(want, hub_limit, n);
+        else if (want < 0) {
+            const int cap = tc_core_clamp(kTcCoreCap, hub_limit, n) / kTcCoreBucket * kTcCoreBucket;
+            if (cap > 0) {
+                const int nbk = cap / kTcCoreBucket;
+                unsigned long long *bucket = nullptr;
+                if (int rc = dmalloc(&bucket, nbk, nullptr)) return rc;
+                DevGuard g_b{bucket};
+                GMSX_HIP(hipMemsetAsync(bucket, 0, size_t(nbk) * sizeof(unsigned long long), s));
+                hipLaunchKernelGGL(k_core_units, dim3(grid_for_waves(cap)), dim3(256), 0, s, cap, g->hoff, g->hadj, g->dplus, bucket);
+                std::vector<uint64_t> h(size_t(nbk), 0);
+                static_assert(sizeof(uint64_t) == sizeof(unsigned long long), "bucket words");
+                GMSX_HIP(hipMemcpyAsync(h.data(), bucket, size_t(nbk) * sizeof(uint64_t), hipMemcpyDeviceToHost, s));
+                GMSX_HIP(hipStreamSynchronize(s));
+                g->tc_core = choose_tc_core(h, cap);
+            }
+        }
+        if (g->tc_core > 0) {
+            const int32_t K = g->tc_core;
+            const int WS = kc4m_stride(K);
+            const int64_t words = int64_t(K) * WS + 8;
+            if (int rc = dmalloc(&g->core_bits, words, g)) return rc;
+            GMSX_HIP(hipMemsetAsync(g->core_bits, 0, size_t(words) * sizeof(uint32_t), s));
+            hipLaunchKernelGGL(k_core_fill, dim3(grid_for_waves(K)), dim3(256), 0, s, K, WS, g->hoff, g->hadj, g->core_bits);
+        }
+    }
+    pt.mark("core matrix");
     {
         int64_t want = std::min<int64_t>(524288, n / 256);
         bool forced = false;
@@ -1246,7 +1315,7 @@
         GMSX_HIP(hipMemsetAsync(inl_t, 0, size_t(n + 1) * sizeof(unsigned long long), s));
         if (n_work > 0)
             hipLaunchKernelGGL(k_inline_rows<false>, dim3(grid_for_waves(n_work)), dim3(256), 0, s, int64_t(0), n_work, g->order, g->hoff, g->hadj,
-                               g->toff, g->tadj, g->dplus, g->inline_limit, g->inline_first, opos, g->shard_nparts, g->shard_part, inl_h, inl_t, ihoff, itoff, int64_t(0), static_cast<uint16_t *>(nullptr),
+                               g->toff, g->tadj, g->dplus, g->inline_limit, g->inline_first, g->tc_core, opos, g->shard_nparts, g->shard_part, inl_h, inl_t, ihoff, itoff, int64_t(0), static_cast<uint16_t *>(nullptr),
                                int64_t(0), static_cast<int32_t *>(nullptr));
         int64_t *uh = nullptr, *ut = nullptr;
         if (int rc = dmalloc(&uh, n + 1, nullptr)) return rc;
@@ -1364,7 +1433,7 @@
         GMSX_HIP(hipMemsetAsync(inl_h, 0, size_t(n + 1) * sizeof(unsigned long long), s));
         GMSX_HIP(hipMemsetAsync(inl_t, 0, size_t(n + 1) * sizeof(unsigned long long), s));
         hipLaunchKernelGGL(k_inline_rows<true>, dim3(grid_for_waves(n_work)), dim3(256), 0, s, int64_t(0), n_work, g->order, g->hoff, g->hadj, g->toff,
-                           g->tadj, g->dplus, g->inline_limit, g->inline_first, opos, g->shard_nparts, g->shard_part, inl_h, inl_t, ihoff, itoff, inline_h_base, reinterpret_cast<uint16_t *>(g->spool),
+                           g->tadj, g->dplus, g->inline_limit, g->inline_first, g->tc_core, opos, g->shard_nparts, g->shard_part, inl_h, inl_t, ihoff, itoff, inline_h_base, reinterpret_cast<uint16_t *>(g->spool),
                            inline_t_base, reinterpret_cast<int32_t *>(g->tpool));
     }
     pt.mark("inline rows fill");
@@ -1377,7 +1446,7 @@
             DevGuard g_ec{ecnt};
             if (int rc = dmalloc(&ebeg, nl + 1, nullptr)) return rc;
             DevGuard g_eb{ebeg};
-            hipLaunchKernelGGL(k_ledge_count, dim3(unsigned(nl / 256 + 1)), dim3(256), 0, s, n_heavy, n_work, g->order, g->toff, g->tadj, g->tsplit, g->dplus, ecnt);
+            hipLaunchKernelGGL(k_ledge_count, dim3(unsigned(nl / 256 + 1)), dim3(256), 0, s, n_heavy, n_work, g->order, g->toff, g->tadj, g->tsplit, g->dplus, g->tc_core, ecnt);
             if (int rc = exclusive_scan_i64(ecnt, ebeg, nl + 1, s)) return rc;
             GMSX_HIP(hipMemcpy(&g->ledge_total, ebeg + nl, sizeof(int64_t), hipMemcpyDeviceToHost));
             const int np = g->shard_nparts > 1 ? g->shard_nparts : 1, pp = g->shard_nparts > 1 ? g->shard_part : 0;
@@ -1386,7 +1455,7 @@
                 g->n_ledge = np <= 1 ? g->ledge_total : full + (((full & 1) ? np - 1 - pp : pp) < rem ? 1 : 0);
             }
             if (int rc = dmalloc(&g->ledge, 2 * g->n_ledge + 2, g)) return rc;
-            hipLaunchKernelGGL(k_ledge_fill, dim3(unsigned(nl / 256 + 1)), dim3(256), 0, s, n_heavy, n_work, g->order, g->hoff, g->toff, g->tadj, g->tsplit, g->dplus, ebeg,
+            hipLaunchKernelGGL(k_ledge_fill, dim3(unsigned(nl / 256 + 1)), dim3(256), 0, s, n_heavy, n_work, g->order, g->hoff, g->toff, g->tadj, g->tsplit, g->dplus, g->tc_core, ebeg,
                                np, pp, g->ledge);
             GMSX_HIP(hipStreamSynchronize(s));
         }
@@ -1455,7 +1524,7 @@
         if (n_heavy > 0)
             hipLaunchKernelGGL(k_task_lists<false>, dim3(grid), dim3(256), 0, s, n_heavy, g->order, g->hoff, g->hadj, g->toff, g->tadj, g->dplus, g->srow, g->srow2, g->ksplit, g->trow,
                                two_sided, opos, cnt, cur, hbeg, tbeg, TaskList{}, TaskList{}, g->tunits,
-                               totals + 2, g->spool, g->tpool, g->inline_limit, g->inline_first, g->shard_nparts, g->shard_part, cc);
+                               totals + 2, g->spool, g->tpool, g->inline_limit, g->inline_first, g->tc_core, g->shard_nparts, g->shard_part, cc);
         pt.mark("task lists count");
         hipLaunchKernelGGL(k_list_sizes, dim3(unsigned(n_recv / 256 + 1)), dim3(256), 0, s, n_recv, cnt, hcnt, tcnt, cc);
         if (int rc = exclusive_scan_i64(hcnt, hbeg, n_recv + 1, s)) return rc;
@@ -1478,7 +1547,7 @@
                                inline_t_base, cnt, cur, hbeg, tbeg, g->htask, g->ttask, totals, cc);
         if (n_heavy > 0)
             hipLaunchKernelGGL(k_task_lists<true>, dim3(grid), dim3(256), 0, s, n_heavy, g->order, g->hoff, g->hadj, g->toff, g->tadj, g->dplus, g->srow, g->srow2, g->ksplit, g->trow,
-                               two_sided, opos, cnt, cur, hbeg, tbeg, g->htask, g->ttask, g->tunits, totals + 2, g->spool, g->tpool, g->inline_limit, g->inline_first, g->shard_nparts, g->shard_part, cc);
+                               two_sided, opos, cnt, cur, hbeg, tbeg, g->htask, g->ttask, g->tunits, totals + 2, g->spool, g->tpool, g->inline_limit, g->inline_first, g->tc_core, g->shard_nparts, g->shard_part, cc);
         pt.mark("task lists fill");
         const int hub_phases = cc.hub_phases();
         const int64_t slots = int64_t(hub_phases) * n_recv;
diff --git a/gms_amd/csrc/hip/device_graph.hpp b/gms_amd/csrc/hip/device_graph.hpp
--- a/gms_amd/csrc/hip/device_graph.hpp
+++ b/gms_amd/csrc/hip/device_graph.hpp
@@ -73,6 +73,10 @@
     int64_t task_reverse = 0;
     uint4 *ledge = nullptr;
     int64_t n_ledge = 0, ledge_total = 0;
+    uint32_t *core_bits = nullptr;
+    int32_t tc_core = 0;
+    mutable int core_bytes_k = -1, core_bytes_part = -1, core_bytes_nparts = -1;
+    mutable uint64_t core_bytes = 0;
     int tc_hot_windows = 0;
     uint32_t tc_window_units = 1;
     int tc_hot_min = 0;
diff --git a/gms_amd/csrc/hip/tc.hip b/gms_amd/csrc/hip/tc.hip
--- a/gms_amd/csrc/hip/tc.hip
+++ b/gms_amd/csrc/hip/tc.hip
@@ -1,4 +1,6 @@
 #include "device_graph.hpp"
+#include "kc4_mfma.hpp"
+#include "../host/tc_core_plan.hpp"
 
 #include <algorithm>
 #include <type_traits>
@@ -658,10 +660,43 @@
     block_add(total, red, lane, wave, tid, acc);
 }
 
+__global__ __launch_bounds__(1024) void k_tc_core(const uint32_t *__restrict__ bits, int WS, int K, int nb, int nblk, int part, int nparts,
+                                                  unsigned long long *__restrict__ acc) {
+    __shared__ unsigned long long red[16];
+    auto lane_id = [] { return int(__builtin_amdgcn_mbcnt_hi(~0u, __builtin_amdgcn_mbcnt_lo(~0u, 0u))); };
+    const int wave = uni32(int(threadIdx.x) >> 6);
+    const int x = blockIdx.x & 7, y = blockIdx.x >> 3, Y = int(gridDim.x) >> 3;
+    const int Q = 16 * Y, q = y * 16 + wave;
+    const int ns = (nblk - part + nparts - 1) / nparts;
+    uint32_t cnt = 0;
+    for (int j = 0;; ++j) {
+        const int sidx = (8 * j + ((j & 1) ? 7 - x : x)) * Q + q;
+        if (sidx >= ns) break;
+        const int t = sidx * nparts + part;
+        int c = int((__builtin_sqrtf(8.0f * float(t) + 1.0f) - 1.0f) * 0.5f);
+        while (c * (c + 1) / 2 > t) --c;
+        while ((c + 1) * (c + 2) / 2 <= t) ++c;
+        const int bj = nb - 1 - c, bi = bj + (t - c * (c + 1) / 2);
+        int lane = lane_id();
+        asm volatile("" : "+v"(lane));
+        cnt += Kc4mBlock<2>::run(bits, WS, K, bi, bj, lane);
+    }
+    const int lane = lane_id();
+    unsigned long long total = cnt;
+    for (int sft = 32; sft > 0; sft >>= 1) total += __shfl_down(total, sft);
+    if (lane == 0) red[wave] = total;
+    __syncthreads();
+    if (wave == 0 && lane == 0) {
+        unsigned long long t = 0;
+        for (int w = 0; w < 16; ++w) t += red[w];
+        if (t) atomicAdd(&acc[(blockIdx.x & (kAccSlots - 1)) * kAccStride], t);
+    }
+}
+
 __global__ __launch_bounds__(256) void k_tc_stats(const int64_t *__restrict__ hoff, const uint16_t *__restrict__ hadj,
                                                   const int64_t *__restrict__ toff, const int32_t *__restrict__ tadj,
                                                   const int32_t *__restrict__ dplus, const int32_t *__restrict__ order,
-                                                  const int32_t *__restrict__ tunits, int32_t inline_limit, int inline_first, int64_t end, int nparts, int part,
+                                                  const int32_t *__restrict__ tunits, int32_t inline_limit, int inline_first, int32_t core, int64_t end, int nparts, int part,
                                                   unsigned long long *__restrict__ out) {
     const int lane = threadIdx.x & 63;
     const int64_t wave0 = (int64_t(blockIdx.x) * blockDim.x + threadIdx.x) >> 6;
@@ -673,6 +708,10 @@
         const int du = dplus[u];
         if (du >= kHeavy) {
             if (lane == 0) units += (unsigned long long)tunits[pos];
+            if (u < core) {
+                if (lane == 0) units += (unsigned long long)du;
+                continue;
+            }
             const int hl = min(int(hoff[u + 1] - hoff[u]), inline_first), tl = min(int(toff[u + 1] - toff[u]), inline_first - hl);
             int32_t v = -1;
             if (lane < hl) {
@@ -684,7 +723,7 @@
         }
         const int hl = int(hoff[u + 1] - hoff[u]);
         if (lane == 0) units += (unsigned long long)du;
-        if (du < 2) continue;
+        if (du < 2 || u < core) continue;
         for (int64_t j = toff[u] + lane; j < toff[u + 1]; j += 64) {
             const int32_t v = tadj[j];
             if (v < inline_limit || dplus[v] >= kHeavy) continue;
@@ -741,7 +780,7 @@
                                                       const int32_t *__restrict__ dplus, const int32_t *__restrict__ order,
                                                       const TaskList htask, const gmsx_tc_item *__restrict__ hitem, int64_t hitems,
                                                       const TaskList ttask, const gmsx_tc_item *__restrict__ titem, int64_t titems,
-                                                      int32_t inline_limit, int64_t first_light, int64_t end_light,
+                                                      int32_t inline_limit, int32_t core, int64_t first_light, int64_t end_light,
                                                       unsigned long long *__restrict__ out) {
     const int lane = threadIdx.x & 63;
     const int64_t wave0 = (int64_t(blockIdx.x) * blockDim.x + threadIdx.x) >> 6;
@@ -769,6 +808,7 @@
     }
     for (int64_t pos = first_light + wave0; pos < end_light; pos += nwaves) {
         const int32_t u = order[pos];
+        if (u < core) continue;
         const int64_t tb0 = toff[u], te = toff[u + 1];
         const unsigned long long hl = (unsigned long long)(hoff[u + 1] - hoff[u]);
         for (int64_t j = tb0 + lane; j < te; j += 64) {
@@ -890,11 +930,21 @@
         if (h[i]) atomicAdd(&out[i], h[i]);
 }
 
-static int tc_one(const gmsx_graph *g, int part, int nparts, uint64_t *partial, gmsx_stats *st);
+static int tc_one(const gmsx_graph *g, int part, int nparts, int cpart, int cnparts, uint64_t *partial, gmsx_stats *st);
+static uint64_t core_bytes_of(const gmsx_graph *g, int part, int nparts) {
+    if (g->tc_core <= 0 || nparts < 1) return 0;
+    if (!(g->core_bytes_k == g->tc_core && g->core_bytes_part == part && g->core_bytes_nparts == nparts)) {
+        g->core_bytes = tc_core_bytes(g->tc_core, part, nparts);
+        g->core_bytes_k = g->tc_core;
+        g->core_bytes_part = part;
+        g->core_bytes_nparts = nparts;
+    }
+    return g->core_bytes;
+}
 
 static int tc_oriented(const gmsx_graph *g, int part, int nparts, uint64_t *partial, gmsx_stats *st) {
     if (int rc = ensure_tc(g)) return rc;
-    if (g->tc_passes == 1) return tc_one(g, part, nparts, partial, st);
+    if (g->tc_passes == 1) return tc_one(g, part, nparts, part, nparts, partial, st);
     if (nparts > 1) {
         auto restore = [&](int rc) {
             gmsx_graph *m = const_cast<gmsx_graph *>(g);
@@ -914,7 +964,7 @@
                 if (rc) break;
                 uint64_t pp = 0;
                 gmsx_stats sp{};
-                rc = tc_one(g, sub, nparts * J, &pp, st ? &sp : nullptr);
+                rc = tc_one(g, sub, nparts * J, part, a == 0 ? nparts : 0, &pp, st ? &sp : nullptr);
                 total += pp;
                 sum.kernel_ms += sp.kernel_ms;
                 sum.setup_ms += sp.setup_ms;
@@ -936,7 +986,7 @@
         if (int rc = ensure_tc_shard(g, p, g->tc_passes)) return rc;
         uint64_t pp = 0;
         gmsx_stats sp{};
-        if (int rc = tc_one(g, p, g->tc_passes, &pp, st ? &sp : nullptr)) return rc;
+        if (int rc = tc_one(g, p, g->tc_passes, 0, p == 0 ? 1 : 0, &pp, st ? &sp : nullptr)) return rc;
         total += pp;
         sum.kernel_ms += sp.kernel_ms;
         sum.setup_ms += sp.setup_ms;
@@ -953,7 +1003,7 @@
     return GMSX_OK;
 }
 
-static int tc_one(const gmsx_graph *g, int part, int nparts, uint64_t *partial, gmsx_stats *st) {
+static int tc_one(const gmsx_graph *g, int part, int nparts, int cpart, int cnparts, uint64_t *partial, gmsx_stats *st) {
     const bool use_idx = nparts > 1 && g->shard_nparts == 1;
     if (use_idx)
         if (int rc = tc_shard_items(g, part, nparts)) return rc;
@@ -1012,6 +1062,16 @@
         GMSX_HIP(hipStreamWaitEvent(c.side[1], c.ev_fork, 0));
         join.armed[1] = true;
     }
+    const bool run_core = g->tc_core > 0 && cnparts > 0 && !only;
+    if (run_core) {
+        const int K = g->tc_core, nb = (K + 63) / 64, nblk = int(tc_core_blocks(K));
+        const int64_t ns = (int64_t(nblk) - cpart + cnparts - 1) / cnparts;
+        if (ns > 0) {
+            const int64_t wgs = std::max<int64_t>(8, std::min<int64_t>(cus / 8 * 8, ((ns + 15) / 16 + 7) / 8 * 8));
+            hipLaunchKernelGGL(k_tc_core, dim3(unsigned(wgs)), dim3(1024), 0, s, g->core_bits, kc4m_stride(K), K, nb, nblk, cpart, cnparts, acc);
+            ++launches;
+        }
+    }
     if (persist) {
         const int wgs_env = [] { const char *e = opt("TC_ITEM_WGS"); return e ? std::atoi(e) : 0; }();
         auto grid = [&](int64_t n, int wgs) {
@@ -1056,7 +1116,7 @@
         if (g->n > 0) {
             const int64_t blocks = std::min<int64_t>((g->n + 3) / 4, cap_blocks);
             hipLaunchKernelGGL(k_tc_stats, dim3(unsigned(blocks)), dim3(256), 0, s, g->hoff, g->hadj, g->toff, g->tadj, g->dplus, g->order,
-                               g->tunits, g->inline_limit, g->inline_first, g->n, nparts, part, acc + kAccSlots * kAccStride);
+                               g->tunits, g->inline_limit, g->inline_first, g->tc_core, g->n, nparts, part, acc + kAccSlots * kAccStride);
         }
         if (g->hitems > 0)
             hipLaunchKernelGGL(k_tc_item_stats, dim3(unsigned(std::min<int64_t>((g->hitems + 3) / 4, cap_blocks))), dim3(256), 0, s, g->hoff, 2, 0, g->htask, g->hitem,
@@ -1089,7 +1149,7 @@
         st->alg_elements = nparts == 1 ? g->alg_elements : 0;
         st->launches = launches;
         st->reserved = 0;
-        st->stream_bytes = g->stats_bytes;
+        st->stream_bytes = g->stats_bytes + (run_core ? core_bytes_of(g, cpart, cnparts) : 0);
     }
     return GMSX_OK;
 }
@@ -1119,12 +1179,14 @@
         GMSX_HIP(hipMemsetAsync(acc, 0, 21 * 8, s));
         const int cus = ctx().compute_units > 0 ? ctx().compute_units : 256;
         hipLaunchKernelGGL(k_tc_breakdown, dim3(unsigned(cus * 16)), dim3(256), 0, s, g->hoff, g->toff, g->tadj, g->dplus, g->order, g->htask,
-                           g->hitem, g->hitems, g->ttask, g->titem, g->titems, g->inline_limit, n_block, n_work, acc);
+                           g->hitem, g->hitems, g->ttask, g->titem, g->titems, g->inline_limit, g->tc_core, n_block, n_work, acc);
         GMSX_HIP(hipMemcpyAsync(out21, acc, 21 * 8, hipMemcpyDeviceToHost, s));
         GMSX_HIP(hipStreamSynchronize(s));
         GMSX_HIP(hipGetLastError());
         out21[7] = uint64_t(g->inline_units) * 16ull;
         out21[12] = uint64_t(g->inline_hentries + g->inline_tentries);
+        out21[15] = core_bytes_of(g, 0, 1);
+        out21[16] = uint64_t(g->tc_core);
         return GMSX_OK;
     });
 }
diff --git a/gms_amd/csrc/host/loader.cpp b/gms_amd/csrc/host/loader.cpp
--- a/gms_amd/csrc/host/loader.cpp
+++ b/gms_amd/csrc/host/loader.cpp
@@ -677,7 +677,7 @@
     {"INLINE_LIMIT", "", false}, {"TC_INLINE_FIRST", "", false}, {"TC_DELTA", "", false}, {"TC_DELTA_PCT", "", false}, {"TC_GAP12", "", false},
     {"TC_HYBRID", "", false}, {"TC_TAIL_DELTA", "", false}, {"TC_TWO_SIDED", "", false}, {"TC_HOT_WINDOWS", "", false}, {"TC_HOT_KB", "", false},
     {"TC_HOT_MIN", "", false}, {"TC_TEST_MAX_UNITS", "", false}, {"TC_KEEP_ROWS", "", false}, {"TC_MEM_LIMIT_MB", "", false}, {"TC_OVERLAP", "", false},
-    {"TC_PERSIST", "", false}, {"TC_ITEM_WGS", "", false}, {"SORT_CHUNK", "", false}, {"UPLOAD_STAGED", "", false}, {"INIT_LAZY", "", false},
+    {"TC_PERSIST", "", false}, {"TC_ITEM_WGS", "", false}, {"TC_CORE", "", false}, {"SORT_CHUNK", "", false}, {"UPLOAD_STAGED", "", false}, {"INIT_LAZY", "", false},
     {"KC_SLAB_MB", "", false}, {"KC_MAXD", "", false}, {"KC_STREAMS", "", false}, {"KC_PIPE_ALL", "", false}, {"KC_STREAM_BUILD", "", false},
     {"KC_REVERSE", "", false}, {"KC_REV_MIN", "", false}, {"KC_REV_FACTOR", "", false}, {"KC_REV_TAIL", "", false}, {"KC_REV_TAIL_MIN", "", false}, {"KC_REV_GW", "", false}, {"KC_TRI", "", false}, {"KC_MFMA", "", false}, {"KC_POOL_MB", "", false},
     {"BK_MAXC", "", false}, {"BK_ARENA_MB", "", false}, {"BK_GROUPS", "", false}, {"BK_SMALL_P", "", false}, {"BK_SMALL_P_GROUPS", "", false},
diff --git a/gms_amd/csrc/host/tc_core_plan.hpp b/gms_amd/csrc/host/tc_core_plan.hpp
--- /dev/null
+++ b/gms_amd/csrc/host/tc_core_plan.hpp
@@ -0,0 +1,52 @@
+#pragma once
+#include <algorithm>
+#include <cstdint>
+#include <vector>
+
+namespace gmsx {
+
+constexpr int kTcCoreBucket = 1024;
+constexpr int kTcCoreCap = 32768;
+constexpr double kTcCoreStreamBytesPerSec = 7.35e12;
+constexpr double kTcCoreBitMacsPerSec = 1.7e15;
+constexpr double kTcCoreLaunchSec = 20e-6;
+constexpr int kTcCoreDefault = -1;
+
+inline int tc_core_clamp(long long want, long long hub_limit, long long n) {
+    return int(std::max<long long>(0, std::min<long long>(std::min<long long>(want, kTcCoreCap), std::min<long long>(hub_limit, n))));
+}
+
+inline int choose_tc_core(const std::vector<uint64_t> &bucket_units, int cap, double b_stream = kTcCoreStreamBytesPerSec,
+                          double r_core = kTcCoreBitMacsPerSec, double launch_sec = kTcCoreLaunchSec) {
+    int best_k = 0;
+    double best = 0.0;
+    unsigned long long units = 0;
+    for (size_t b = 0; b < bucket_units.size(); ++b) {
+        const long long k = (long long)(b + 1) * kTcCoreBucket;
+        if (k > cap) break;
+        units += bucket_units[b];
+        const double gain = double(units) * 16.0 / b_stream - (double(k) * double(k) * double(k) / 6.0) / r_core - launch_sec;
+        if (gain > best) {
+            best = gain;
+            best_k = int(k);
+        }
+    }
+    return best_k;
+}
+
+inline long long tc_core_blocks(int k) {
+    const long long nb = (k + 63) / 64;
+    return nb * (nb + 1) / 2;
+}
+inline unsigned long long tc_core_block_bytes(int bj) { return 1024ull * (unsigned long long)(bj + 1) + 1024ull; }
+inline unsigned long long tc_core_bytes(int k, int part, int nparts) {
+    const long long nb = (k + 63) / 64;
+    unsigned long long bytes = 0;
+    long long t = 0;
+    for (long long c = 0; c < nb; ++c)
+        for (long long r = 0; r <= c; ++r, ++t)
+            if (nparts <= 1 || t % nparts == part) bytes += tc_core_block_bytes(int(nb - 1 - c));
+    return bytes;
+}
+
+}
```

New measurement: 16.07 billion, median of 6. +2.1%, better.
